# phymhan/pc-gan

Measured on AMD Instinct MI355X. Metric: images/sec (G+D step) 128x128 bs32 per GPU, higher is better.
Workload: dtype f32; 1 GPU; wsgan_emb UTKFace-shaped 128x128 bs32/GPU fp32: 9-block ResnetGenerator + 3-layer PatchGAN + ResNet-18 Elo encoder@224 + AlexNet IP@224, full optimize_parameters(); global_batch=32, parallelism=dp1

## Files before the change

### include/pcgan_hip.h

```cpp
#ifndef PCGAN_HIP_H
#define PCGAN_HIP_H

#include <stddef.h>
#include <stdint.h>

#ifdef __cplusplus
extern "C" {
#endif

typedef void* pcgan_stream_t;

const char* pcgan_last_error(void);
int pcgan_version(void);
int pcgan_device_info(int* cu_count, char* arch, int arch_len);

typedef struct {
    int N, C, H, W;
    int K, R, S;
    int stride, pad, pad_mode;
    int P, Q;
    int dtype;
} pcgan_conv_desc;

enum { PCGAN_ACT_NONE = 0, PCGAN_ACT_RELU = 1, PCGAN_ACT_LRELU = 2, PCGAN_ACT_TANH = 3, PCGAN_ACT_SIGMOID = 4 };
// ... 182 lines not shown
                       const float* const* b1, const void* const* pk2, const float* const* b2, float* const* rm1, float* const* rv1,
                       float* const* rm2, float* const* rv2, void* y1, void* h, void* y2, void* out, float* stats, float* amax,
                       pcgan_stream_t s);
int pcgan_restrunk_bwd(const pcgan_resblock_desc* d, int nblocks, const void* dout, const void* x, const float* x_amax, int n_xamax,
                       const void* y1, const void* h, const void* y2, const void* out, const float* stats, const float* amax,
                       const void* const* pk1b, const void* const* pk2b, float* const* dw1, float* const* db1, float* const* dw2,
                       float* const* db2, void* dy2, void* dh, void* dy1, void* dxs, void* dx, float* scratch, void* wgrad_ws,
                       size_t wgrad_ws_bytes, pcgan_stream_t s, pcgan_stream_t side, pcgan_event_t fork_event);

int pcgan_conv2d_wgrad_direct_supported(const pcgan_conv_desc* d);
int pcgan_conv2d_wgrad_rowring_supported(const pcgan_conv_desc* d);
size_t pcgan_conv2d_wgrad_rowring_workspace_bytes(const pcgan_conv_desc* d);
int pcgan_conv2d_bwd_weight_rowring(const pcgan_conv_desc* d, const void* x, const float* x_amax, int n_xamax, const void* dy, const float* dy_amax,
                                    int n_dyamax, float* dw, int accumulate, void* ws, size_t ws_bytes, pcgan_stream_t s);
size_t pcgan_conv2d_wgrad_direct_workspace_bytes(const pcgan_conv_desc* d);
int pcgan_conv2d_bwd_weight_direct(const pcgan_conv_desc* d, const void* x, const float* x_amax, int n_xamax, const void* dy,
                                   const float* dy_amax, int n_dyamax, float* dw, int accumulate, void* ws, size_t ws_bytes, pcgan_stream_t s);

typedef struct {
    int N, C, H, W;
    int K, R, S;
    int stride, pad_h, pad_w;
    int P, Q;
    int k_off, K_total;
    int dtype;
} pcgan_iconv_desc;
int pcgan_iconv_supported(const pcgan_iconv_desc* d);
size_t pcgan_iconv_packed_bytes(const pcgan_iconv_desc* d);
int pcgan_iconv_pack(const pcgan_iconv_desc* d, int pool_expand, const float* w, const float* gamma, const float* beta, const float* mean,
                     const float* var, float eps, void* packed, pcgan_stream_t s);
int pcgan_iconv_fwd(const pcgan_iconv_desc* d, const void* x, const void* packed, void* y, int relu, pcgan_stream_t s);
int pcgan_maxpool_slice_fwd(const void* x, void* y, int N, int C, int H, int W, int k, int stride, int P, int Q, int k_off, int K_total,
                            int dtype, pcgan_stream_t s);
int pcgan_inception_prep(const void* x, void* y, int N, int C, int H, int W, int OH, int OW, const float* scale, const float* shift,
                         int dtype, pcgan_stream_t s);

int pcgan_linear_softmax_fwd(const void* x, const float* w, const float* b, void* logits, void* probs, int N, int C, int K, int dtype,
                             pcgan_stream_t s);

size_t pcgan_linear_ce_workspace_bytes(int N);
int pcgan_linear_ce_fwd(const void* x, const float* w, const float* b, const int64_t* labels, const float* class_weight, void* logits,
                        void* dlogits, float* loss, int64_t* pred, int32_t* correct, void* workspace, size_t workspace_bytes, int N,
                        int C, int K, int dtype, pcgan_stream_t s);
int pcgan_linear_bwd(const void* dlogits, const void* x, const float* w, void* dx, float* dw, float* db, int N, int C, int K,
                     int accumulate, int dtype, pcgan_stream_t s);

size_t pcgan_pool_mse_workspace_bytes(int NF);
int pcgan_pool_mse_fwd(const void* x, const float* target, float* pred, int32_t* argmax, void* dx, float* loss, int32_t* hits, void* ws,
                       size_t ws_bytes, int N, int F, int HW, int is_max, float delta, float gscale, int dtype, pcgan_stream_t s);

int pcgan_proj_head_fwd(const void* p, const float* y, const float* psi_w, const float* psi_b, const float* ly_w, const float* ly_b,
                        void* out, float* h, int B, int C, int HW, int nz, int By, int sigmoid, int dtype, pcgan_stream_t s);
size_t pcgan_proj_head_bwd_workspace_bytes(int B, int nz);
int pcgan_proj_head_bwd(const void* g, const float* h, const float* y, const float* psi_w, const float* psi_b, const float* ly_w,
                        const float* ly_b, void* dp, float* dpsi_w, float* dpsi_b, float* dly_w, float* dly_b, float* dy, void* workspace,
                        size_t workspace_bytes, int B, int C, int HW, int nz, int By, int sigmoid, int accumulate, int dtype,
                        pcgan_stream_t s);

int pcgan_skip_join_fwd(const void* a, const void* b, void* out, int N, int Ca, int Cb, int HW, int act_a, int act_b, int dtype,
                        pcgan_stream_t s);
int pcgan_skip_join_bwd(const void* dout, const void* a, const void* b, void* da, void* db, int N, int Ca, int Cb, int HW, int act_a,
                        int act_b, int dtype, pcgan_stream_t s);

int pcgan_set_nonfinite_counter(unsigned int* dev_word);
int pcgan_set_option(const char* key, int value);
int pcgan_get_option(const char* key, int* value);
int pcgan_timer_enable(int capacity);
int pcgan_timer_read(int kind, float* ms, int cap);
#define PCGAN_IGEMM_LAUNCH_INFO 7
#define PCGAN_IGEMM_HGEMM_F16X2 1
#define PCGAN_IGEMM_HGEMM_BF16 2
#define PCGAN_IGEMM_IGEMM2_CG16 3
#define PCGAN_IGEMM_IGEMM2_CG4 4
#define PCGAN_IGEMM_GENERIC 5
#define PCGAN_IGEMM_SMALLM 6
int pcgan_igemm_last_launch(int* info, int n);
#define PCGAN_WGRAD_LAUNCH_INFO 9
#define PCGAN_WGRAD_TILE2 1
#define PCGAN_WGRAD_TILE 2
#define PCGAN_WGRAD_SMALLM 3
#define PCGAN_WGRAD_STRIP 4
int pcgan_wgrad_last_launch(int* info, int n);

#ifdef __cplusplus
}
#endif
#endif
```

### pc-gan_amd/csrc/amax.hip

```cpp
#include "common.h"

namespace pcgan {

template <typename TA>
__global__ void __launch_bounds__(256) absmax_kernel(const TA* __restrict__ x, size_t n, float* __restrict__ out) {
    float m = 0.f;
    size_t head = ((16 - (reinterpret_cast<uintptr_t>(x) & 15)) & 15) / sizeof(TA);
    head = head < n ? head : n;
    const TA* xb = x + head;
    const size_t nb = n - head, n4 = nb / 4, stride = (size_t)gridDim.x * blockDim.x;
    size_t i = blockIdx.x * (size_t)blockDim.x + threadIdx.x;
    for (; i + 3 * stride < n4; i += 4 * stride) {
        const float4 a = ld4(xb + 4 * i), b = ld4(xb + 4 * (i + stride)), c = ld4(xb + 4 * (i + 2 * stride)), d = ld4(xb + 4 * (i + 3 * stride));
        m = fmaxf(m, fmaxf(fmaxf(fmaxf(fabsf(a.x), fabsf(a.y)), fmaxf(fabsf(a.z), fabsf(a.w))), fmaxf(fmaxf(fabsf(b.x), fabsf(b.y)), fmaxf(fabsf(b.z), fabsf(b.w)))));
        m = fmaxf(m, fmaxf(fmaxf(fmaxf(fabsf(c.x), fabsf(c.y)), fmaxf(fabsf(c.z), fabsf(c.w))), fmaxf(fmaxf(fabsf(d.x), fabsf(d.y)), fmaxf(fabsf(d.z), fabsf(d.w)))));
    }
    for (; i < n4; i += stride) {
        const float4 v = ld4(xb + 4 * i);
        m = fmaxf(fmaxf(m, fmaxf(fabsf(v.x), fabsf(v.y))), fmaxf(fabsf(v.z), fabsf(v.w)));
    }
    if (blockIdx.x == 0) {
        if (threadIdx.x < head) m = fmaxf(m, fabsf(ld1(x + threadIdx.x)));
        if (threadIdx.x < (nb & 3)) m = fmaxf(m, fabsf(ld1(xb + 4 * n4 + threadIdx.x)));
    }
    __shared__ float red[16];
    m = block_max(m, red);
    if (threadIdx.x == 0) out[blockIdx.x] = m;
}

__global__ void __launch_bounds__(256) amax_audit_kernel(const float* __restrict__ claimed, int nc, const float* __restrict__ fresh, int nf,
                                                         unsigned* __restrict__ counts) {
    __shared__ float red[16];
    float c = 0.f, f = 0.f;
    for (int i = threadIdx.x; i < nc; i += 256) c = fmaxf(c, claimed[i]);
    for (int i = threadIdx.x; i < nf; i += 256) f = fmaxf(f, fresh[i]);
    c = block_max(c, red);
    __syncthreads();
    f = block_max(f, red);
    if (threadIdx.x == 0 && f != c) {
        if (!(f <= c)) atomicAdd(counts + 0, 1u);
        else if (f < c * 0.00390625f) atomicAdd(counts + 1, 1u);
        else atomicAdd(counts + 2, 1u);
    }
}

__global__ void __launch_bounds__(256) weight_row_absmax_kernel(const float* __restrict__ w, int K, int C, int T, int by_c, float* __restrict__ out) {
    const int row = blockIdx.x;
    float m = 0.f;
    if (!by_c) {
        const float* p = w + (size_t)row * C * T;
        for (int i = threadIdx.x; i < C * T; i += 256) m = fmaxf(m, fabsf(p[i]));
    } else {
        for (int i = threadIdx.x; i < K * T; i += 256) {
            const int k = i / T, t = i - k * T;
            m = fmaxf(m, fabsf(w[((size_t)k * C + row) * T + t]));
        }
    }
    __shared__ float red[16];
    m = block_max(m, red);
    if (threadIdx.x == 0) out[row] = m;
}

int launch_weight_row_absmax(const float* w, int K, int C, int T, int by_c, float* out, hipStream_t st) {
    hipLaunchKernelGGL(weight_row_absmax_kernel, dim3((unsigned)(by_c ? C : K)), dim3(256), 0, st, w, K, C, T, by_c, out);
    PCGAN_LAUNCH_CHECK();
    return 0;
}

}

extern "C" int pcgan_absmax_slots(size_t n) {
    const size_t want = (n / 4 + 1023) / 1024;
    return (int)(want < 1 ? 1 : (want > 1024 ? 1024 : want));
}

extern "C" int pcgan_absmax(const void* x, size_t n, int dtype, float* out, int slots, pcgan_stream_t s) {
    PCGAN_CHECK(x && out && n > 0 && slots > 0 && slots <= 1024, "absmax: null pointer, empty tensor or bad slot count");
    PCGAN_CHECK(dtype == PCGAN_F32 || dtype == PCGAN_BF16, "absmax: dtype %d", dtype);
    hipStream_t st = (hipStream_t)s;
    const dim3 grid((unsigned)slots);
    if (dtype == PCGAN_BF16) hipLaunchKernelGGL(pcgan::absmax_kernel<pcgan::bf16>, grid, dim3(256), 0, st, (const pcgan::bf16*)x, n, out);
    else hipLaunchKernelGGL(pcgan::absmax_kernel<float>, grid, dim3(256), 0, st, (const float*)x, n, out);
    PCGAN_LAUNCH_CHECK();
    return 0;
}

extern "C" int pcgan_amax_audit(const float* claimed, int n_claimed, const float* fresh, int n_fresh, unsigned int* counts, pcgan_stream_t s) {
    PCGAN_CHECK(claimed && fresh && counts && n_claimed > 0 && n_fresh > 0, "amax_audit: null pointer or empty maxima");
    hipLaunchKernelGGL(pcgan::amax_audit_kernel, dim3(1), dim3(256), 0, (hipStream_t)s, claimed, n_claimed, fresh, n_fresh, counts);
    PCGAN_LAUNCH_CHECK();
    return 0;
}
```

### pc-gan_amd/csrc/bsplit.h

```cpp
#pragma once
#include "common.h"

namespace pcgan {

typedef float f32x16 __attribute__((ext_vector_type(16)));
typedef __bf16 bf16x8 __attribute__((ext_vector_type(8)));
typedef _Float16 f16x8 __attribute__((ext_vector_type(8)));
typedef unsigned int u32x4 __attribute__((ext_vector_type(4)));
static constexpr unsigned BS_OOB = 0x80000000u;
static constexpr int BS_MAXTAP = 25;

__device__ __forceinline__ void split3(float x, __bf16& h, __bf16& m, __bf16& l) {
    h = (__bf16)x;
    const float r1 = x - (float)h;
    m = (__bf16)r1;
    l = (__bf16)(r1 - (float)m);
}

struct BsplitArgs {
    const void* X;
    const void* A;
    const float* bias;
    void* Y;
    int N, C, H, W, M, R, S, pad, reflect, P, Q;
    int nMt, nst, act;
    float slope;
    unsigned x_bytes, a_bytes;
    int tstart[4];
    unsigned phase_bytes;
    int nst_split;
};

enum { BS_FWD_ZERO = 0, BS_FWD_REFLECT = 1, BS_DGRAD_REFLECT = 2, BS_WGRAD = 3 };

__device__ __forceinline__ void pack_store8(__bf16* __restrict__ A, size_t e, size_t per_piece, int np, float wscale, const float (&v)[8]) {
    if (np == 2) {
        f16x8 h, l;
#pragma unroll
        for (int j = 0; j < 8; ++j) {
            _Float16 x, y;
            split2h(v[j] * wscale, x, y);
            h[j] = x;
            l[j] = y;
        }
        *reinterpret_cast<f16x8*>(reinterpret_cast<_Float16*>(A) + 8 * e) = h;
        *reinterpret_cast<f16x8*>(reinterpret_cast<_Float16*>(A) + per_piece + 8 * e) = l;
        return;
    }
    bf16x8 h, mm, l;
#pragma unroll
    for (int j = 0; j < 8; ++j) {
        __bf16 x, y, z;
        split3(v[j], x, y, z);
        h[j] = x;
        mm[j] = y;
        l[j] = z;
    }
    *reinterpret_cast<bf16x8*>(A + 8 * e) = h;
    if (np == 3) {
        *reinterpret_cast<bf16x8*>(A + per_piece + 8 * e) = mm;
        *reinterpret_cast<bf16x8*>(A + 2 * per_piece + 8 * e) = l;
    }
}

enum { BH_FWD = 0, BH_DGRAD = 1 };

struct HaloArgs {
    const void* X;
    const void* A;
    const float* bias;
    void* Y;
    int N, C, H, M, nMt, nch, act;
    float slope;
    unsigned x_bytes, a_bytes;
    const float* x_amax;
    const float* w_amax;
    int x_namax;
    unsigned* ovf;
    const void* R;
};

enum { PK_BF16X3 = 0,
       PK_BF16 = 1,
       PK_F16X2 = 2 };

struct HWgradArgs {
    const void* XP;
    const void* DY;
    float* part;
    int N, C, K, P, Q, Hp, Wp, R, S, nst, nst_split;
    unsigned xp_bytes, dy_bytes;
    const float* x_amax;
    const float* dy_amax;
    int x_namax, dy_namax;
    int ntile, nwg;
    unsigned* ovf;
    int reflect_inline;
    int splits, nmt;
    int Qs, pad;
};

static inline int np_of(const pcgan_conv_desc* d) { return d->dtype == PCGAN_BF16 ? 1 : 3; }
static inline size_t es_of(const pcgan_conv_desc* d) { return d->dtype == PCGAN_BF16 ? 2 : 4; }

int launch_pad(const void* x, void* xpad, int planes, int H, int W, int pad, int reflect, bool half, hipStream_t st);
int launch_bsplit_pack(const float* w, void* packed, int M, int C, int T, int nMt, int nst, int bm, int np, const float* rowmax, hipStream_t st);
int launch_bsplit_pack_dgrad(const float* w, void* packed, int K, int C, int nMt, int nst, int bm, int np, const float* rowmax, int nphase,
                             hipStream_t st);
int launch_pack_dy(const void* dy, void* packed, int K, int HW, int nst, int bm, int np, bool half, hipStream_t st);
int launch_wgrad_reduce(const float* part, float* dw, int splits, size_t total, int accumulate, hipStream_t st);
int launch_bsplit(int mode, int dtype, int bm, dim3 grid, const BsplitArgs& a, hipStream_t st);
int launch_halo(int mode, int pk, int W, const HaloArgs& a, hipStream_t st);
int launch_hsplit_wgrad(const HWgradArgs& a, int bm, int stride, int cw, bool gen, bool half, dim3 grid, hipStream_t st);

}
```

### pc-gan_amd/csrc/bsplit_pack.hip

```cpp
#include "bsplit.h"

namespace pcgan {

__global__ void bsplit_pack_kernel(const float* __restrict__ w, __bf16* __restrict__ A, int M, int C, int T, int nMt, int nst,
                                   int bm_shift, int np, const float* __restrict__ rowmax = nullptr) {
    const int BM = 128 << bm_shift;
    const size_t per_piece = (size_t)nMt * nst * 16 * BM;
    for (size_t e = blockIdx.x * (size_t)blockDim.x + threadIdx.x; e < per_piece / 8; e += (size_t)gridDim.x * blockDim.x) {
        const int row = (int)(e & (BM - 1)), half = (int)((e >> (7 + bm_shift)) & 1);
        const size_t q = e >> (8 + bm_shift);
        const int st = (int)(q % nst), mt = (int)(q / nst);
        const int m = mt * BM + row, c0 = (st / T) * 16 + half * 8, tap = st % T;
        float v[8];
#pragma unroll
        for (int j = 0; j < 8; ++j) v[j] = m < M ? w[((size_t)m * C + c0 + j) * T + tap] : 0.f;
        const float wscale = (np == 2 && m < M) ? pow2_scale(rowmax[m]) : 1.f;
        pack_store8(A, e, per_piece, np, wscale, v);
    }
}

int launch_bsplit_pack(const float* w, void* packed, int M, int C, int T, int nMt, int nst, int bm, int np, const float* rowmax, hipStream_t st) {
    const size_t per_piece = (size_t)nMt * nst * 16 * bm;
    hipLaunchKernelGGL(bsplit_pack_kernel, dim3(capped_blocks(per_piece / 8, 256, 4096)), dim3(256), 0, st, w, (__bf16*)packed, M, C, T, nMt, nst,
                       bm == 256 ? 1 : 0, np, rowmax);
    PCGAN_LAUNCH_CHECK();
    return 0;
}

__global__ void bsplit_pack_dgrad_kernel(const float* __restrict__ w, __bf16* __restrict__ A, int K, int C, int nMt, int nst, int bm_shift,
                                         int np, const float* __restrict__ rowmax = nullptr, int nphase = 3) {
    const int BM = 128 << bm_shift;
    const size_t per_piece = (size_t)nMt * nst * 16 * BM, per_phase = (size_t)np * per_piece;
    const size_t per_phase8 = per_piece / 8;
    for (size_t i = blockIdx.x * (size_t)blockDim.x + threadIdx.x; i < (size_t)nphase * per_phase8; i += (size_t)gridDim.x * blockDim.x) {
        const int phase = (int)(i / per_phase8);
        const size_t e = i - (size_t)phase * per_phase8;
        const int row = (int)(e & (BM - 1)), half = (int)((e >> (7 + bm_shift)) & 1);
        const size_t q = e >> (8 + bm_shift);
        const int st = (int)(q % nst), mt = (int)(q / nst);
        const int c = mt * BM + row, k0 = (st / 9) * 16 + half * 8, tap = st % 9;
        const int rp = tap / 3, sp = tap - rp * 3;
        const bool fold = (phase == 1 && rp == 0) || (phase == 2 && rp == 2);
        float v[8];
#pragma unroll
        for (int j = 0; j < 8; ++j) {
            v[j] = 0.f;
            if (c < C) {
                const float* wk = w + ((size_t)(k0 + j) * C + c) * 9;
                v[j] = wk[(2 - rp) * 3 + (2 - sp)];
                if (fold) v[j] += wk[rp * 3 + (2 - sp)];
            }
        }
        const float wscale = (np == 2 && c < C) ? pow2_scale(rowmax[c]) : 1.f;
        pack_store8(A + (size_t)phase * per_phase, e, per_piece, np, wscale, v);
    }
}

int launch_bsplit_pack_dgrad(const float* w, void* packed, int K, int C, int nMt, int nst, int bm, int np, const float* rowmax, int nphase,
                             hipStream_t st) {
    const size_t total = (size_t)nphase * nMt * nst * 2 * bm;
    hipLaunchKernelGGL(bsplit_pack_dgrad_kernel, dim3(capped_blocks(total, 256, 4096)), dim3(256), 0, st, w, (__bf16*)packed, K, C, nMt, nst,
                       bm == 256 ? 1 : 0, np, rowmax, nphase);
    PCGAN_LAUNCH_CHECK();
    return 0;
}

template <typename TA>
__global__ void bsplit_pad_reflect_kernel(const TA* __restrict__ x, TA* __restrict__ xp, int H, int W, int pad, int reflect = 1) {
    const int Hp = H + 2 * pad, Wp = W + 2 * pad;
    const TA* src = x + (size_t)blockIdx.y * H * W;
    TA* dst = xp + (size_t)blockIdx.y * Hp * Wp;
    for (int i = blockIdx.x * blockDim.x + threadIdx.x; i < Hp * Wp; i += gridDim.x * blockDim.x) {
        int y = i / Wp - pad, xx = i % Wp - pad;
        if (!reflect) {
            const bool in = (unsigned)y < (unsigned)H && (unsigned)xx < (unsigned)W;
            TA v;
            st1(&v, 0.f);
            dst[i] = in ? src[y * W + xx] : v;
            continue;
        }
        y = y < 0 ? -y : (y >= H ? 2 * (H - 1) - y : y);
        xx = xx < 0 ? -xx : (xx >= W ? 2 * (W - 1) - xx : xx);
        dst[i] = src[y * W + xx];
    }
}

template <typename TA>
__global__ void __launch_bounds__(256) bsplit_pad_wave_kernel(const TA* __restrict__ x, TA* __restrict__ xp, int planes, int H, int W, int pad, int reflect) {
    const int lane = threadIdx.x & 63;
    const int plane = blockIdx.x * 4 + (threadIdx.x >> 6);
    if (plane >= planes) return;
    const int Hp = H + 2 * pad, Wp = W + 2 * pad, half = Wp >> 1;
    const TA* src = x + (size_t)plane * H * W;
    TA* dst = xp + (size_t)plane * Hp * Wp;
    int row = lane / half, cp = lane - row * half;
    const int drow = 64 / half, dcp = 64 - drow * half;
    typedef TA pair_t __attribute__((ext_vector_type(2)));
    while (row < Hp) {
        int y = row - pad, x0 = 2 * cp - pad, x1 = x0 + 1;
        bool in0 = (unsigned)y < (unsigned)H, in1 = in0;
        if (reflect) {
            y = y < 0 ? -y : (y >= H ? 2 * (H - 1) - y : y);
            x0 = x0 < 0 ? -x0 : (x0 >= W ? 2 * (W - 1) - x0 : x0);
            x1 = x1 < 0 ? -x1 : (x1 >= W ? 2 * (W - 1) - x1 : x1);
            in0 = in1 = true;
        } else {
            in0 = in0 && (unsigned)x0 < (unsigned)W;
            in1 = in1 && (unsigned)x1 < (unsigned)W;
        }
        TA zero;
        st1(&zero, 0.f);
        pair_t v;
        v.x = in0 ? src[y * W + x0] : zero;
        v.y = in1 ? src[y * W + x1] : zero;
        *reinterpret_cast<pair_t*>(dst + row * Wp + 2 * cp) = v;
        cp += dcp;
        row += drow;
        if (cp >= half) {
            cp -= half;
            ++row;
        }
    }
}

int launch_pad(const void* x, void* xpad, int planes, int H, int W, int pad, int reflect, bool half, hipStream_t st) {
    const int Hp = H + 2 * pad, Wp = W + 2 * pad;
    if (Wp % 2 == 0 && Wp <= 128 && Hp * Wp <= 8192 && planes >= 1024) {
        const dim3 grid((planes + 3) / 4);
        if (half) hipLaunchKernelGGL(bsplit_pad_wave_kernel<bf16>, grid, dim3(256), 0, st, (const bf16*)x, (bf16*)xpad, planes, H, W, pad, reflect);
        else hipLaunchKernelGGL(bsplit_pad_wave_kernel<float>, grid, dim3(256), 0, st, (const float*)x, (float*)xpad, planes, H, W, pad, reflect);
        PCGAN_LAUNCH_CHECK();
        return 0;
    }
    const dim3 pgrid((Hp * Wp + 255) / 256, planes);
    if (half) hipLaunchKernelGGL(bsplit_pad_reflect_kernel<bf16>, pgrid, dim3(256), 0, st, (const bf16*)x, (bf16*)xpad, H, W, pad, reflect);
    else hipLaunchKernelGGL(bsplit_pad_reflect_kernel<float>, pgrid, dim3(256), 0, st, (const float*)x, (float*)xpad, H, W, pad, reflect);
    PCGAN_LAUNCH_CHECK();
    return 0;
}

template <typename TA>
__global__ void bsplit_pack_dy_kernel(const TA* __restrict__ dy, __bf16* __restrict__ A, int K, int HW, int nst, int bm_shift, int np) {
    const int BM = 128 << bm_shift;
    const size_t per_piece = (size_t)nst * 16 * BM;
    for (size_t i = blockIdx.x * (size_t)blockDim.x + threadIdx.x; i < per_piece; i += (size_t)gridDim.x * blockDim.x) {
// ... 46 lines not shown
```

### pc-gan_amd/csrc/hgemm.hip

```cpp
#include "igemm.h"

namespace pcgan {

typedef _Float16 f16x8 __attribute__((ext_vector_type(8)));
typedef _Float16 f16x4 __attribute__((ext_vector_type(4)));

typedef __bf16 bf16x8v __attribute__((ext_vector_type(8)));
typedef __bf16 bf16x4v __attribute__((ext_vector_type(4)));

template <int MODE, int BM, int BP, typename TA>
__global__ void __launch_bounds__(256) hgemm_kernel(IgemmArgs a) {
    static_assert(MODE == MODE_FWD_ZERO || MODE == MODE_FWD_REFLECT || MODE == MODE_BWD, "forward and plain data gradient");
    constexpr bool HALF = sizeof(TA) == 2;
    constexpr int NP = HALF ? 1 : 2;
    constexpr unsigned ES = sizeof(TA);
    constexpr int WM = (BM == 128 || (BM == 64 && BP == 64)) ? 2 : 1;
    constexpr int WP = 4 / WM;
    constexpr int WMT = BM / WM, WPT = BP / WP;
    constexpr int MI = WMT / 32, PJ = WPT / 32;
    constexpr int KPT = BP / 16;
    constexpr int ACH = BM * 4 / 256;
    constexpr int TROWS = NTAP_FWD + 1;
    constexpr int AH = BM + 8;
    __shared__ __attribute__((aligned(16))) f16x8 As[2][NP][2 * AH];
    __shared__ __attribute__((aligned(16))) f16x8 Bs[2][NP][2 * BP];
    __shared__ unsigned offT[TROWS][BP];
    __shared__ __attribute__((aligned(16))) float biasS[BM];
    __shared__ __attribute__((aligned(16))) float iswS[BM];

    const int nMt = (a.M + BM - 1) / BM;
    const int mt = blockIdx.x % nMt;
    int pt = blockIdx.x / nMt;
    int phase = 0;
    while (phase + 1 < a.nphase && pt >= a.tstart[phase + 1]) ++phase;
    pt -= a.tstart[phase];
    const PhaseArgs& P = a.ph[phase];
    const int tid = threadIdx.x;
    const int lane = tid & 63, lo = lane & 31, hi = lane >> 5;
    const int wave = __builtin_amdgcn_readfirstlane(tid >> 6);
    const int wm = wave / WP, wp = wave % WP;
    const int Ptot = P.Ptot, Kp = P.Kp;
    const int m0 = mt * BM, p0 = pt * BP;
    const int ph_nS = P.nS;
    const int T = P.nR * ph_nS;
    const int HgWg4 = a.Hg * a.Wg * (int)ES;
    const __amdgpu_buffer_rsrc_t rX = make_rsrc(a.X, a.x_bytes);
    const __amdgpu_buffer_rsrc_t rA = make_rsrc(P.A, (unsigned)a.M * (unsigned)Kp * 4u);

    float sx = 1.f;
    const int pl = tid % BP;
    {
        const int pg = p0 + pl;
        const bool pvalid = pg < Ptot;
        int gn = 0, py = 0, px = 0;
        if (pvalid) pix_coord(a, P, pg, gn, py, px);
        const unsigned vbase = (unsigned)gn * (unsigned)a.Cg * (unsigned)(a.Hg * a.Wg);
        for (int t = tid / BP; t <= T; t += 256 / BP) {
            const int ri = t / ph_nS, sj = t - ri * ph_nS;
            const int r = P.r0 + ri * a.tstep, sxx = P.s0 + sj * a.tstep;
            const bool live = pvalid && t < T;
            const unsigned y = axis_entry<MODE>(py, py + a.pad, true, r, a.Hg, a.sl, a.pad);
            const unsigned x = axis_entry<MODE>(px, px + a.pad, true, sxx, a.Wg, a.sl, a.pad);
            offT[t][pl] = (live && y != 0xffffffffu && x != 0xffffffffu) ? (vbase + y * (unsigned)a.Wg + x) * ES : OOB;
        }
    }
    const int ksub = __builtin_amdgcn_readfirstlane(tid / BP);
    __syncthreads();

    const int nst_all = Kp >> 4;
    const int nst_per = a.ksplit > 1 ? (nst_all + a.ksplit - 1) / a.ksplit : nst_all;
    const int st_begin = a.ksplit > 1 ? (int)blockIdx.z * nst_per : 0;
    const int st_end = st_begin + nst_per < nst_all ? st_begin + nst_per : nst_all;
    const int nst_here = st_end > st_begin ? st_end - st_begin : 0;

    int it_tap, it_c, it_k0, it_left = nst_here;
    {
        const int cc0 = st_begin / T;
        it_tap = st_begin - cc0 * T;
        it_c = cc0 * 16;
        it_k0 = st_begin * 16;
    }
    unsigned a_base[ACH];
#pragma unroll
    for (int j = 0; j < ACH; ++j) {
        const int q = tid + 256 * j;
        const int row = q >> 2, kc = (q & 3) * 4;
        a_base[j] = (m0 + row < a.M) ? (unsigned)((m0 + row) * Kp + kc) * 4u : OOB;
    }
// ... 147 lines not shown
        fetch(op[0], 0);
        stash(rg[1], 1);
        __syncthreads();
        load(rg[1]);
        const int nst2 = (nst_here + 1) & ~1;
        for (int s = 0; s < nst2; s += 2) {
#pragma unroll
            for (int t = 0; t < 2; ++t) {
                fetch(op[t ^ 1], t ^ 1);
                mma(op[t]);
                stash(rg[t], t);
                load(rg[t]);
                interleave();
                __builtin_amdgcn_sched_barrier(0);
                __syncthreads();
                __builtin_amdgcn_sched_barrier(0);
            }
        }
    }

    const float isx = 1.f / sx;
    const int YhYw = a.Yh * a.Yw;
    bool bad = false;
    if constexpr (!HALF) {
#pragma unroll
        for (int j = 0; j < PJ; ++j)
#pragma unroll
            for (int i = 0; i < MI; ++i)
#pragma unroll
                for (int r = 0; r < 16; ++r) bad |= is_nonfinite(acc[i][j][r]);
        report_nonfinite(a.ovf, bad);
    }
#pragma unroll
    for (int j = 0; j < PJ; ++j) {
        const int pix = p0 + wp * WPT + j * 32 + lo;
        if (pix >= Ptot) continue;
        int n, oy, ox;
        pix_coord(a, P, pix, n, oy, ox);
        if (a.ksplit > 1) {
            float* Yp = a.Ypart + ((size_t)blockIdx.z * a.N + n) * a.M * YhYw + oy * a.Yw + ox;
#pragma unroll
            for (int i = 0; i < MI; ++i)
#pragma unroll
                for (int r = 0; r < 16; ++r) {
                    const int ml = wm * WMT + i * 32 + (r & 3) + 8 * (r >> 2) + 4 * hi;
                    const int m = m0 + ml;
                    if (m < a.M) Yp[(size_t)m * YhYw] = (acc[i][j][r] * isx) * (HALF ? 1.f : iswS[ml]);
                }
            continue;
        }
        TA* Yp = (TA*)a.Y + (size_t)n * a.M * YhYw + oy * a.Yw + ox;
#pragma unroll
        for (int i = 0; i < MI; ++i)
#pragma unroll
            for (int r = 0; r < 16; ++r) {
                const int ml = wm * WMT + i * 32 + (r & 3) + 8 * (r >> 2) + 4 * hi;
                if (m0 + ml < a.M) st1(Yp + (size_t)(m0 + ml) * YhYw, act_apply((acc[i][j][r] * isx) * (HALF ? 1.f : iswS[ml]) + biasS[ml], a.act, a.slope));
            }
    }
}

template <int MODE>
static void launch_mode(const IgemmArgs& a, int bm, int bp, dim3 grid2, hipStream_t st) {
    if (bm == 128 && bp == 128) LAUNCH_TA(a.dtype, hgemm_kernel, grid2, a, MODE, 128, 128);
    else if (bm == 128) LAUNCH_TA(a.dtype, hgemm_kernel, grid2, a, MODE, 128, 64);
    else if (bp == 128) LAUNCH_TA(a.dtype, hgemm_kernel, grid2, a, MODE, 64, 128);
    else LAUNCH_TA(a.dtype, hgemm_kernel, grid2, a, MODE, 64, 64);
}
int launch_hgemm(int mode, const IgemmArgs& a, int bm, int bp, dim3 grid2, hipStream_t st) {
    switch (mode) {
        case MODE_FWD_ZERO: launch_mode<MODE_FWD_ZERO>(a, bm, bp, grid2, st); break;
        case MODE_FWD_REFLECT: launch_mode<MODE_FWD_REFLECT>(a, bm, bp, grid2, st); break;
        case MODE_BWD: launch_mode<MODE_BWD>(a, bm, bp, grid2, st); break;
        default: PCGAN_CHECK(false, "hgemm: no kernel for mode %d", mode);
    }
    PCGAN_LAUNCH_CHECK();
    return 0;
}

}

using namespace pcgan;

__global__ void __launch_bounds__(256) hgemm_presplit_kernel(float* __restrict__ A, int M, int Kp4, const float* __restrict__ rowmax) {
    const size_t n4 = (size_t)M * Kp4;
    for (size_t i = (size_t)blockIdx.x * 256 + threadIdx.x; i < n4; i += (size_t)gridDim.x * 256) {
        const float s = pow2_scale(rowmax[i / Kp4]);
        const float4 v = reinterpret_cast<const float4*>(A)[i];
        f16x4 h, l;
        _Float16 x, y;
        split2h(v.x * s, x, y); h[0] = x; l[0] = y;
        split2h(v.y * s, x, y); h[1] = x; l[1] = y;
        split2h(v.z * s, x, y); h[2] = x; l[2] = y;
        split2h(v.w * s, x, y); h[3] = x; l[3] = y;
        reinterpret_cast<f16x4*>(A)[2 * i] = h;
        reinterpret_cast<f16x4*>(A)[2 * i + 1] = l;
    }
}

int pcgan::launch_hgemm_presplit(float* A, int M, int Kp4, const float* rowmax, hipStream_t st) {
    hipLaunchKernelGGL(hgemm_presplit_kernel, dim3(capped_blocks((size_t)M * Kp4, 256, 2048)), dim3(256), 0, st, A, M, Kp4, rowmax);
    PCGAN_LAUNCH_CHECK();
    return 0;
}
```

### pc-gan_amd/csrc/igemm_conv.hip

```cpp
#include "igemm.h"
#include <stdlib.h>
#include <mutex>

namespace pcgan {

template <typename TA>
__global__ void splitk_reduce_kernel(const float* __restrict__ part, TA* __restrict__ y, const float* __restrict__ bias,
                                     int ks, size_t n, int M, int HW, int act, float slope) {
    const size_t n4 = (n & 3) ? 0 : (n >> 2);
    const size_t stride = (size_t)gridDim.x * blockDim.x;
    for (size_t i = blockIdx.x * (size_t)blockDim.x + threadIdx.x; i < n4; i += stride) {
        float4 acc = reinterpret_cast<const float4*>(part)[i];
        for (int s = 1; s < ks; ++s) {
            const float4 v = reinterpret_cast<const float4*>(part + (size_t)s * n)[i];
            acc.x += v.x; acc.y += v.y; acc.z += v.z; acc.w += v.w;
        }
        float o[4] = {acc.x, acc.y, acc.z, acc.w};
#pragma unroll
        for (int u = 0; u < 4; ++u) {
            const size_t e = i * 4 + u;
            if (bias) o[u] += bias[(e / HW) % M];
            o[u] = act_apply(o[u], act, slope);
        }
        st4(y + 4 * i, make_float4(o[0], o[1], o[2], o[3]));
    }
    for (size_t e = (n4 << 2) + blockIdx.x * (size_t)blockDim.x + threadIdx.x; e < n; e += stride) {
        float acc = 0.f;
        for (int s = 0; s < ks; ++s) acc += part[(size_t)s * n + e];
        if (bias) acc += bias[(e / HW) % M];
        st1(y + e, act_apply(acc, act, slope));
    }
}

__global__ void repack_fwd_kernel(const float* __restrict__ w, float* __restrict__ A, int K, int C, int Cgp,
                                  int RS, int chunked) {
    const int Kp = RS * Cgp;
    const size_t total = (size_t)K * Kp;
    for (size_t i = blockIdx.x * (size_t)blockDim.x + threadIdx.x; i < total; i += (size_t)gridDim.x * blockDim.x) {
        const int k = (int)(i / Kp);
        const int j = (int)(i - (size_t)k * Kp);
        int tap, c;
        if (chunked) {
            const int t2 = j >> 4;
            const int cc = t2 / RS;
            tap = t2 - cc * RS;
            c = cc * 16 + (j & 15);
        } else {
            tap = j / Cgp;
            c = j - tap * Cgp;
        }
        A[i] = (c < C) ? w[((size_t)k * C + c) * RS + tap] : 0.f;
    }
}
__global__ void repack_bwd_kernel(const float* __restrict__ w, float* __restrict__ A, int K, int C, int Kgp,
                                  int R, int S, int r0, int s0, int tstep, int nR, int nS, int chunked, int fold) {
    const int Kp = nR * nS * Kgp;
    const size_t total = (size_t)C * Kp;
    for (size_t i = blockIdx.x * (size_t)blockDim.x + threadIdx.x; i < total; i += (size_t)gridDim.x * blockDim.x) {
        const int c = (int)(i / Kp);
        const int j = (int)(i - (size_t)c * Kp);
        int t, k;
        if (chunked) {
            const int t2 = j >> 4;
            const int kc = t2 / (nR * nS);
            t = t2 - kc * (nR * nS);
            k = kc * 16 + (j & 15);
        } else {
            t = j / Kgp;
            k = j - t * Kgp;
        }
        const int ri = t / nS, sj = t - ri * nS;
        const int r = r0 + ri * tstep, s = s0 + sj * tstep;
        float v = (k < K) ? w[(((size_t)k * C + c) * R + r) * S + s] : 0.f;
        if (k < K && fold == 1 && r == R - 1) v += w[(((size_t)k * C + c) * R + 0) * S + s];
        if (k < K && fold == 2 && r == 0) v += w[(((size_t)k * C + c) * R + (R - 1)) * S + s];
        A[i] = v;
    }
}

struct PackBwdArgs {
    const float* w;
    int K, C, Kgp, R, S, tstep, chunked, n;
    struct Entry {
        float* A;
        int r0, s0, nR, nS, fold;
    } e[16];
};
__global__ void repack_bwd_multi_kernel(PackBwdArgs a) {
    const PackBwdArgs::Entry& E = a.e[blockIdx.y];
    const int RS = E.nR * E.nS;
    const int Kp = RS * a.Kgp;
    const size_t total = (size_t)a.C * Kp;
    for (size_t i = blockIdx.x * (size_t)blockDim.x + threadIdx.x; i < total; i += (size_t)gridDim.x * blockDim.x) {
        const int c = (int)(i / Kp);
        const int j = (int)(i - (size_t)c * Kp);
        int t, k;
        if (a.chunked) {
            const int t2 = j >> 4;
            const int kc = t2 / RS;
            t = t2 - kc * RS;
            k = kc * 16 + (j & 15);
        } else {
            t = j / a.Kgp;
            k = j - t * a.Kgp;
        }
        const int ri = t / E.nS, sj = t - ri * E.nS;
        const int r = E.r0 + ri * a.tstep, sx = E.s0 + sj * a.tstep;
        float v = 0.f;
        if (k < a.K) {
            const float* wk = a.w + ((size_t)k * a.C + c) * a.R * a.S;
            v = wk[r * a.S + sx];
            if (E.fold == 1 && r == a.R - 1) v += wk[sx];
            if (E.fold == 2 && r == 0) v += wk[(a.R - 1) * a.S + sx];
        }
        E.A[i] = v;
    }
}

template <typename TA>
__global__ void reflect_fold_kernel(const TA* __restrict__ t, TA* __restrict__ dx, int NC, int H, int W,
                                    int pad) {
    const int Hp = H + 2 * pad, Wp = W + 2 * pad;
    const int W4 = (W + 3) >> 2;
    const TA* tp = t + (size_t)blockIdx.y * Hp * Wp;
    TA* dp = dx + (size_t)blockIdx.y * H * W;
    for (int i = blockIdx.x * blockDim.x + threadIdx.x; i < H * W4; i += gridDim.x * blockDim.x) {
        const int y = i / W4, x0 = (i - y * W4) * 4;
        int ys[3], ny = 0;
        ys[ny++] = y + pad;
        if (y >= 1 && y <= pad) ys[ny++] = pad - y;
        if (y >= H - 1 - pad && y <= H - 2) ys[ny++] = pad + 2 * (H - 1) - y;
        float acc[4] = {0.f, 0.f, 0.f, 0.f};
        for (int a = 0; a < ny; ++a) {
            const TA* row = tp + ys[a] * Wp;
#pragma unroll
            for (int j = 0; j < 4; ++j) {
                const int x = x0 + j;
                if (x >= W) continue;
                float v = ld1(row + x + pad);
                if (x >= 1 && x <= pad) v += ld1(row + pad - x);
                if (x >= W - 1 - pad && x <= W - 2) v += ld1(row + pad + 2 * (W - 1) - x);
                acc[j] += v;
            }
        }
        if ((W & 3) == 0) {
            st4(dp + y * W + x0, make_float4(acc[0], acc[1], acc[2], acc[3]));
        } else {
            for (int j = 0; j < 4 && x0 + j < W; ++j) st1(dp + y * W + x0 + j, acc[j]);
        }
    }
}

int launch_splitk_reduce(int dtype, hipStream_t st, const float* part, void* y, const float* bias, int ks, size_t out_elems, int M,
                         int HW, int act, float slope) {
    const dim3 b(capped_blocks(out_elems / 4, 256, 4096));
    if (dtype == PCGAN_BF16)
        hipLaunchKernelGGL(splitk_reduce_kernel<bf16>, b, dim3(256), 0, st, part, (bf16*)y, bias, ks, out_elems, M, HW, act, slope);
    else
        hipLaunchKernelGGL(splitk_reduce_kernel<float>, b, dim3(256), 0, st, part, (float*)y, bias, ks, out_elems, M, HW, act, slope);
    PCGAN_LAUNCH_CHECK();
    return 0;
}

static int check_desc(const pcgan_conv_desc* d) {
    PCGAN_CHECK(d != nullptr, "conv: null descriptor");
    PCGAN_CHECK(d->N > 0 && d->C > 0 && d->H > 0 && d->W > 0 && d->K > 0 && d->R > 0 && d->S > 0,
                "conv: non-positive dimension");
    PCGAN_CHECK(ilog2_exact(d->stride) >= 0 && d->stride <= 4, "conv: stride %d unsupported (1,2,4)", d->stride);
    PCGAN_CHECK(d->pad_mode == 0 || d->pad_mode == 1, "conv: pad_mode %d", d->pad_mode);
    PCGAN_CHECK(d->dtype == PCGAN_F32 || d->dtype == PCGAN_BF16, "conv: dtype %d (PCGAN_F32 / PCGAN_BF16)", d->dtype);
    const int P = (d->H + 2 * d->pad - d->R) / d->stride + 1, Q = (d->W + 2 * d->pad - d->S) / d->stride + 1;
    PCGAN_CHECK(P == d->P && Q == d->Q, "conv: output dims %dx%d do not match geometry %dx%d", d->P, d->Q, P, Q);
    if (d->pad_mode == 1)
        PCGAN_CHECK(d->pad < d->H && d->pad < d->W, "conv: reflection pad %d >= input size", d->pad);
    const size_t xin = (size_t)d->N * d->C * (d->H + 2 * d->pad) * (d->W + 2 * d->pad) * 4;
    const size_t yout = (size_t)d->N * d->K * d->P * d->Q * 4;
    PCGAN_CHECK(xin < (1ull << 31) && yout < (1ull << 31),
                "conv: tensor of %zu bytes exceeds the 2 GiB addressing limit of one launch (split the batch)",
                xin > yout ? xin : yout);
    PCGAN_CHECK((size_t)d->K * round4(d->C) * d->R * d->S * 4 < (1ull << 31) &&
                    (size_t)d->C * round4(d->K) * d->R * d->S * 4 < (1ull << 31), "conv: weight tensor too large");
    PCGAN_CHECK(d->R * d->S <= 512, "conv: filter too large");
    return 0;
}

static inline bool chunked_k(int Cg, int M, int R, int S) { return (Cg % 16) == 0 && M > 4 && R * S <= NTAP_FWD; }
static inline bool cg4_k(int Cg, int M, int R, int S) { return round4(Cg) == 4 && M > 4 && R * S <= NTAP_CG4; }
static inline long tile_blocks(int M, int ptot_max, int nphase, int mm, int pp) {
    return (long)((M + mm - 1) / mm) * ((ptot_max + pp - 1) / pp) * nphase;
}
static inline long split_below() { return 192; }
static inline bool may_split(int M, int ptot_max, int nphase) {
    if (option(OPT_HGEMM_KS) > 1) return M > 4;
    const int m = M > 64 ? 128 : (M > 32 ? 64 : 32);
    return M > 4 && tile_blocks(M, ptot_max, nphase, m, 128) < split_below();
}
static void choose_tile(int M, int ptot_max, int nphase, int nst, bool allow_split, int* bm, int* bp, int* ks) {
    int m = M > 64 ? 128 : (M > 32 ? 64 : 32);
    int p = 128;
// ... 52 lines not shown
    int nst_min = 1 << 30;
    for (int i = 0; i < a.nphase; ++i) nst_min = (a.ph[i].Kp + 15) / 16 < nst_min ? (a.ph[i].Kp + 15) / 16 : nst_min;
    const size_t out_elems = (size_t)a.N * a.M * a.Yh * a.Yw;
    choose_tile(a.M, pmax, a.nphase, nst_min, part_ws != nullptr, &bm, &bp, &ks);
    if (ks > 1 && (size_t)ks * out_elems * 4 > part_bytes) ks = 1;
    a.ksplit = ks;
    a.Ypart = part_ws;
    const dim3 grid((unsigned)(((a.M + bm - 1) / bm) * ((pmax + bp - 1) / bp)), (unsigned)a.nphase, (unsigned)ks);
    a.tstart[0] = 0;
    for (int i = 0; i < a.nphase; ++i) a.tstart[i + 1] = a.tstart[i] + (a.ph[i].Ptot + bp - 1) / bp;
    const dim3 grid2((unsigned)(((a.M + bm - 1) / bm) * a.tstart[a.nphase]), 1u, (unsigned)ks);
    const bool cg16 = a.chunked == 1, cg4 = a.chunked == 2;
    PCGAN_CHECK(cg16 || mode != MODE_BWD_REFLECT, "igemm: fused reflect data-gradient needs K %% 16 == 0");
    if (cg4) {
        PCGAN_CHECK(a.Cgp == 4, "igemm: 4-channel stages need a 3-/4-channel tensor");
        for (int i = 0; i < a.nphase; ++i)
            PCGAN_CHECK(a.ph[i].nR * a.ph[i].nS <= NTAP_CG4, "igemm: 4-channel stages: more than %d taps", NTAP_CG4);
    }
    if (cg16) {
        PCGAN_CHECK((a.Cg % 16) == 0, "igemm: chunked K order needs a multiple of 16 channels");
        for (int i = 0; i < a.nphase; ++i)
            PCGAN_CHECK(a.ph[i].nR * a.ph[i].nS <= (mode == MODE_BWD_REFLECT ? NTAP_MIR : NTAP_FWD) && (a.ph[i].Kp % 16) == 0,
                        "igemm: chunked K order: bad phase");
    }
    const bool half = a.dtype == PCGAN_BF16 && option(OPT_HGEMM_BF16) != 0;
    if ((half || (a.hsplit && a.dtype == PCGAN_F32)) && cg16 && mode != MODE_BWD_REFLECT && bm >= 64) {
        record_launch(half ? PCGAN_IGEMM_HGEMM_BF16 : PCGAN_IGEMM_HGEMM_F16X2, mode, bm, bp, ks, a.nphase);
        if (int e = launch_hgemm(mode, a, bm, bp, grid2, st)) return e;
    } else {
        record_launch(cg16 ? PCGAN_IGEMM_IGEMM2_CG16 : (cg4 ? PCGAN_IGEMM_IGEMM2_CG4 : PCGAN_IGEMM_GENERIC), mode, bm, bp, ks, a.nphase);
        if (int e = launch_igemm_f32(mode, a, bm, bp, grid, grid2, st)) return e;
    }
    if (ks > 1 && launch_splitk_reduce(a.dtype, st, part_ws, a.Y, a.bias, ks, out_elems, a.M, a.Yh * a.Yw, a.act, a.slope)) return 2;
    return 0;
}

}

using namespace pcgan;

static size_t fwd_part_bytes(const pcgan_conv_desc* d) {
    const int ptot = d->N * d->P * d->Q;
    if (d->K <= 4) return (ptot <= 65536 && d->C >= 64) ? align_up((size_t)8 * d->K * ptot * 4, 256) : 0;
    return may_split(d->K, ptot, 1) ? align_up((size_t)8 * d->N * d->K * d->P * d->Q * 4, 256) : 0;
}
static size_t bwd_part_bytes(const pcgan_conv_desc* d) {
    const int s = d->stride;
    const int pmax = d->N * ((d->H + s - 1) / s) * ((d->W + s - 1) / s);
    return may_split(d->C, pmax, s * s) ? align_up((size_t)8 * d->N * d->C * d->H * d->W * 4, 256) : 0;
}
static size_t fwd_base_bytes(const pcgan_conv_desc* d) {
    return align_up((size_t)d->K * d->R * d->S * round4(d->C) * 4 + (size_t)d->R * d->S * round4(d->C) * 16 +
                    (d->K <= 4 ? (size_t)d->S * d->C * 128 : 0), 256);
}
static bool bwd_fused_reflect(const pcgan_conv_desc* d) {
    return d->pad_mode == 1 && chunked_k(d->K, d->C, d->R, d->S) && d->R * d->S <= NTAP_MIR && d->H >= 2 * d->pad + 2 &&
           d->W >= 2 * d->pad + 2;
}
static bool bwd_rowfold(const pcgan_conv_desc* d) { return bwd_fused_reflect(d) && d->pad == 1 && d->R == 3 && d->stride == 1; }
static size_t bwd_base_bytes(const pcgan_conv_desc* d) {
    const size_t a = (size_t)d->C * d->R * d->S * round4(d->K) * 4;
    return align_up((bwd_rowfold(d) ? 3 * a : a) + (size_t)d->R * d->S * round4(d->K) * 16 +
                    (d->C <= 4 ? (size_t)d->stride * d->S * d->K * 128 : 0), 256);
}

extern "C" size_t pcgan_conv2d_workspace_bytes(const pcgan_conv_desc* d, int pass) {
    if (!d) return 0;
    const size_t RS = (size_t)d->R * d->S;
    if (pass == PCGAN_PASS_FWD) return fwd_base_bytes(d) + fwd_part_bytes(d);
    if (pass == PCGAN_PASS_BWD_DATA) {
        size_t b = bwd_base_bytes(d) + bwd_part_bytes(d);
        if (d->pad_mode == 1)
            b += align_up((size_t)d->N * d->C * (d->H + 2 * d->pad) * (d->W + 2 * d->pad) * 4, 256);
        return b;
    }
    int cps;
    const int splits = wgrad_splits(d, &cps);
    return align_up((size_t)splits * d->K * RS * round4(d->C) * 4, 256);
}

static int pack_fwd(const pcgan_conv_desc* d, const float* w, float* A, hipStream_t st) {
    const int Cgp = round4(d->C), RS = d->R * d->S;
    const size_t total = (size_t)d->K * RS * Cgp;
    hipLaunchKernelGGL(repack_fwd_kernel, dim3(capped_blocks(total, 256, 4096)), dim3(256), 0, st, w, A, d->K, d->C, Cgp, RS,
                       (int)chunked_k(d->C, d->K, d->R, d->S));
    PCGAN_LAUNCH_CHECK();
    if (d->K <= 4) {
        if (int e = launch_transpose4(A, A + total, d->K, RS * Cgp, st)) return e;
        if (int e = launch_pack_strip(A, A + total + (size_t)RS * Cgp * 4, d->K, d->C, Cgp, d->R, d->S, st)) return e;
    }
    return 0;
}

struct HsplitOpt {
    const float* x_amax;
    int n_amax;
    const float* w_amax;
};
static void apply_hsplit(IgemmArgs& a, const HsplitOpt* hs) {
    if (!hs) return;
    a.hsplit = 1; a.x_amax = hs->x_amax; a.x_namax = hs->n_amax; a.w_amax = hs->w_amax;
    a.ovf = pcgan::nonfinite_counter();
}

static int conv2d_fwd_impl(const pcgan_conv_desc* d, const void* x, const float* w, const float* packed,
                           const float* bias, void* y, int act, float slope, void* ws, size_t ws_bytes,
                           pcgan_stream_t s, const HsplitOpt* hs = nullptr) {
    if (check_desc(d)) return 1;
    PCGAN_CHECK(x && (w || packed) && y, "conv2d_fwd: null pointer");
    PCGAN_CHECK(ws && ws_bytes >= pcgan_conv2d_workspace_bytes(d, PCGAN_PASS_FWD),
                "conv2d_fwd: workspace too small (%zu)", ws_bytes);
    hipStream_t st = (hipStream_t)s;
    const int Cgp = round4(d->C), RS = d->R * d->S;
    float* A = packed ? const_cast<float*>(packed) : (float*)ws;
    if (!packed && pack_fwd(d, w, A, st)) return 2;
    IgemmArgs a;
    memset(&a, 0, sizeof(a));
    a.X = x; a.Y = y; a.bias = bias; a.dtype = d->dtype;
    a.M = d->K; a.N = d->N; a.Cg = d->C; a.Cgp = Cgp; a.Hg = d->H; a.Wg = d->W;
    a.Yh = d->P; a.Yw = d->Q;
    a.ostep = 1; a.sl = ilog2_exact(d->stride); a.pad = d->pad; a.tstep = 1;
    a.act = act; a.slope = slope;
    a.x_bytes = (unsigned)((size_t)d->N * d->C * d->H * d->W * esz(d));
    a.nphase = 1;
    a.chunked = chunked_k(d->C, d->K, d->R, d->S) ? 1 : (cg4_k(d->C, d->K, d->R, d->S) ? 2 : 0);
    apply_hsplit(a, hs);
    PhaseArgs& p = a.ph[0];
    p.A = A; p.Kp = RS * Cgp; p.Hs = d->P; p.Ws = d->Q; p.fy = 0; p.fx = 0;
    if (d->K <= 4) {
        p.A = A + (size_t)d->K * RS * Cgp;
        p.As = p.A + (size_t)RS * Cgp * 4;
    }
    p.r0 = 0; p.s0 = 0; p.nR = d->R; p.nS = d->S; p.Ptot = d->N * d->P * d->Q;
    float* part = fwd_part_bytes(d) ? (float*)((char*)ws + fwd_base_bytes(d)) : nullptr;
    return launch_igemm(d->pad_mode == 1 ? MODE_FWD_REFLECT : MODE_FWD_ZERO, a, st, part, fwd_part_bytes(d));
}

extern "C" int pcgan_conv2d_fwd(const pcgan_conv_desc* d, const void* x, const float* w, const float* bias,
                                void* y, int act, float slope, void* ws, size_t ws_bytes, pcgan_stream_t s) {
    if (check_desc(d)) return 1;
    PCGAN_CHECK(w, "conv2d_fwd: null weight pointer");
    return conv2d_fwd_impl(d, x, w, nullptr, bias, y, act, slope, ws, ws_bytes, s);
}
extern "C" int pcgan_conv2d_fwd_packed(const pcgan_conv_desc* d, const void* x, const float* packed,
                                       const float* bias, void* y, int act, float slope, void* ws, size_t ws_bytes,
                                       pcgan_stream_t s) {
    if (check_desc(d)) return 1;
    PCGAN_CHECK(packed, "conv2d_fwd_packed: null packed-weight pointer");
    pcgan::TimerScope timer(pcgan::timer_kind_res(d, pcgan::TIMER_RES_FWD), (hipStream_t)s);
    return conv2d_fwd_impl(d, x, nullptr, packed, bias, y, act, slope, ws, ws_bytes, s);
}

namespace pcgan {
int launch_reflect_fold(const void* padded, void* dx, int NC, int H, int W, int pad, int dtype, hipStream_t st) {
    PCGAN_CHECK(NC <= 65535, "conv2d_bwd_data: more than 65535 planes in the reflect fold");
    const dim3 grid((H * ((W + 3) / 4) + 255) / 256, NC);
    if (dtype == PCGAN_BF16)
        hipLaunchKernelGGL(reflect_fold_kernel<bf16>, grid, dim3(256), 0, st, (const bf16*)padded, (bf16*)dx, NC, H, W, pad);
    else
        hipLaunchKernelGGL(reflect_fold_kernel<float>, grid, dim3(256), 0, st, (const float*)padded, (float*)dx, NC, H, W, pad);
    PCGAN_LAUNCH_CHECK();
    return 0;
}
}

struct BwdPhase {
    int fy, fx, r0, s0, nR, nS, Hs, Ws;
    int fold;
    size_t a_off, at_off, as_off;
};
struct BwdPlan {
    bool fused, rowfold, padded;
    int H, W, pad;
    bool need_zero;
    int n;
    BwdPhase ph[16];
};
static void bwd_plan(const pcgan_conv_desc* d, BwdPlan& pl) {
    memset(&pl, 0, sizeof(pl));
    pl.fused = bwd_fused_reflect(d);
    pl.rowfold = bwd_rowfold(d);
    pl.padded = d->pad_mode == 1 && !pl.fused;
    const int H = pl.H = pl.padded ? d->H + 2 * d->pad : d->H;
    const int W = pl.W = pl.padded ? d->W + 2 * d->pad : d->W;
    const int pad = pl.pad = pl.padded ? 0 : d->pad;
    const int stv = d->stride, Kgp = round4(d->K), RS = d->R * d->S;
    if (pl.rowfold) {
        for (int f = 0; f < 3; ++f) {
            BwdPhase& p = pl.ph[pl.n++];
            p.nR = d->R; p.nS = d->S; p.Ws = W; p.fold = f;
            p.Hs = f == 0 ? H - 2 : 1;
            p.fy = f == 0 ? 0 : (f == 1 ? 1 : H - 2);
            p.a_off = (size_t)f * d->C * RS * Kgp;
        }
        return;
    }
    size_t a_off = 0;
    size_t at_off = (size_t)d->C * RS * Kgp;
    size_t as_off = at_off + (size_t)RS * Kgp * 4;
    for (int fy = 0; fy < stv; ++fy) {
        for (int fx = 0; fx < stv; ++fx) {
            const int r0 = (fy + pad) % stv, s0 = (fx + pad) % stv;
            const int nR = r0 < d->R ? (d->R - r0 + stv - 1) / stv : 0;
            const int nS = s0 < d->S ? (d->S - s0 + stv - 1) / stv : 0;
            const int Hs = fy < H ? (H - fy + stv - 1) / stv : 0;
            const int Ws = fx < W ? (W - fx + stv - 1) / stv : 0;
            if (Hs * Ws == 0) continue;
            if (nR * nS == 0) {
                pl.need_zero = true;
                continue;
            }
            const BwdPhase p = {fy, fx, r0, s0, nR, nS, Hs, Ws, 0, a_off, at_off, as_off};
            pl.ph[pl.n++] = p;
            a_off += (size_t)d->C * nR * nS * Kgp;
            at_off += (size_t)nR * nS * Kgp * 4;
            as_off += (size_t)d->K * nS * 32;
        }
    }
}

static int pack_bwd(const pcgan_conv_desc* d, const BwdPlan& pl, const float* w, float* packed, hipStream_t st) {
    const int Kgp = round4(d->K);
    const int chunked = (int)chunked_k(d->K, d->C, d->R, d->S);
    if (d->C <= 4) {
        for (int i = 0; i < pl.n; ++i) {
            const BwdPhase& p = pl.ph[i];
            float* A = packed + p.a_off;
            const size_t total = (size_t)d->C * p.nR * p.nS * Kgp;
            hipLaunchKernelGGL(repack_bwd_kernel, dim3(capped_blocks(total, 256, 4096)), dim3(256), 0, st, w, A, d->K, d->C, Kgp, d->R,
                               d->S, p.r0, p.s0, d->stride, p.nR, p.nS, chunked, 0);
            PCGAN_LAUNCH_CHECK();
            if (int e = launch_transpose4(A, packed + p.at_off, d->C, p.nR * p.nS * Kgp, st)) return e;
            if (int e = launch_pack_strip(A, packed + p.as_off, d->C, d->K, Kgp, p.nR, p.nS, st)) return e;
        }
        return 0;
    }
    if (pl.n == 0) return 0;
    size_t max_total = 0;
    PackBwdArgs pk;
    memset(&pk, 0, sizeof(pk));
    pk.w = w; pk.K = d->K; pk.C = d->C; pk.Kgp = Kgp; pk.R = d->R; pk.S = d->S; pk.tstep = d->stride; pk.chunked = chunked; pk.n = pl.n;
    for (int i = 0; i < pl.n; ++i) {
        const BwdPhase& p = pl.ph[i];
        const size_t total = (size_t)d->C * p.nR * p.nS * Kgp;
        max_total = total > max_total ? total : max_total;
        PackBwdArgs::Entry& pe = pk.e[i];
        pe.A = packed + p.a_off; pe.r0 = p.r0; pe.s0 = p.s0; pe.nR = p.nR; pe.nS = p.nS; pe.fold = p.fold;
    }
    hipLaunchKernelGGL(repack_bwd_multi_kernel, dim3(capped_blocks(max_total, 256, 2048), pk.n), dim3(256), 0, st, pk);
    PCGAN_LAUNCH_CHECK();
    return 0;
}

static int conv2d_bwd_data_impl(const pcgan_conv_desc* d, const void* dy, const float* w, const float* packed,
                                const float* bias, void* dx, void* ws, size_t ws_bytes, pcgan_stream_t s, const HsplitOpt* hs = nullptr) {
    if (check_desc(d)) return 1;
    PCGAN_CHECK(dy && (w || packed), "conv2d_bwd_data: null pointer");
    PCGAN_CHECK(ws && ws_bytes >= pcgan_conv2d_workspace_bytes(d, PCGAN_PASS_BWD_DATA),
                "conv2d_bwd_data: workspace too small (%zu)", ws_bytes);
    PCGAN_CHECK(d->pad_mode == 0 || d->stride == 1, "conv2d_bwd_data: reflection padding needs stride 1");
    hipStream_t st = (hipStream_t)s;
    const int Kgp = round4(d->K), stv = d->stride;
    BwdPlan pl;
    bwd_plan(d, pl);
    float* Abase = packed ? const_cast<float*>(packed) : (float*)ws;
    if (!packed && pack_bwd(d, pl, w, Abase, st)) return 2;
    const size_t a_bytes = bwd_base_bytes(d);
    const int H = pl.H, W = pl.W;
    void* out = pl.padded ? (void*)((char*)ws + a_bytes) : dx;

    IgemmArgs a;
    memset(&a, 0, sizeof(a));
    a.X = dy; a.Y = out; a.bias = bias; a.dtype = d->dtype;
    a.M = d->C; a.N = d->N; a.Cg = d->K; a.Cgp = Kgp; a.Hg = d->P; a.Wg = d->Q;
    a.Yh = H; a.Yw = W;
    a.ostep = stv; a.sl = ilog2_exact(stv); a.pad = pl.pad; a.tstep = stv;
    a.act = PCGAN_ACT_NONE; a.slope = 0.f;
    a.chunked = chunked_k(d->K, d->C, d->R, d->S) ? 1 : (cg4_k(d->K, d->C, d->R, d->S) ? 2 : 0);
    a.rowfold = pl.rowfold;
    apply_hsplit(a, hs);
    a.x_bytes = (unsigned)((size_t)d->N * d->K * d->P * d->Q * esz(d));
    a.nphase = pl.n;
    for (int i = 0; i < pl.n; ++i) {
        const BwdPhase& q = pl.ph[i];
        PhaseArgs& p = a.ph[i];
        p.A = Abase + q.a_off; p.Kp = q.nR * q.nS * Kgp; p.Hs = q.Hs; p.Ws = q.Ws; p.fy = q.fy; p.fx = q.fx;
        if (d->C <= 4) {
            p.A = Abase + q.at_off;
            p.As = Abase + q.as_off;
        }
        p.r0 = q.r0; p.s0 = q.s0; p.nR = q.nR; p.nS = q.nS; p.Ptot = d->N * q.Hs * q.Ws;
        p.ymap = pl.rowfold && q.fold == 0;
    }
    if (pl.rowfold) return launch_igemm(MODE_BWD_REFLECT, a, st, nullptr, 0);
    if (pl.need_zero) {
        PCGAN_CHECK(!bias, "conv2d_bwd_data: bias with uncovered phases is unsupported");
        hipError_t e = hipMemsetAsync(out, 0, (size_t)d->N * d->C * H * W * esz(d), st);
        PCGAN_CHECK(e == hipSuccess, "memset failed: %s", hipGetErrorString(e));
    }
    float* part = (bwd_part_bytes(d) && !pl.padded && !pl.need_zero) ? (float*)((char*)ws + a_bytes) : nullptr;
    if (launch_igemm(pl.fused ? MODE_BWD_REFLECT : MODE_BWD, a, st, part, bwd_part_bytes(d))) return 2;
    if (pl.padded) return pcgan::launch_reflect_fold(out, dx, d->N * d->C, d->H, d->W, d->pad, d->dtype, st);
    return 0;
}

extern "C" int pcgan_conv2d_bwd_data(const pcgan_conv_desc* d, const void* dy, const float* w,
                                     const float* bias, void* dx, void* ws, size_t ws_bytes,
                                     pcgan_stream_t s) {
    if (check_desc(d)) return 1;
    PCGAN_CHECK(w && dx, "conv2d_bwd_data: null pointer");
    return conv2d_bwd_data_impl(d, dy, w, nullptr, bias, dx, ws, ws_bytes, s);
}
extern "C" int pcgan_conv2d_bwd_data_packed(const pcgan_conv_desc* d, const void* dy, const float* packed,
                                            const float* bias, void* dx, void* ws, size_t ws_bytes,
                                            pcgan_stream_t s) {
    if (check_desc(d)) return 1;
    PCGAN_CHECK(packed && dx, "conv2d_bwd_data_packed: null pointer");
    pcgan::TimerScope timer(pcgan::timer_kind_res(d, pcgan::TIMER_RES_DGRAD), (hipStream_t)s);
    return conv2d_bwd_data_impl(d, dy, nullptr, packed, bias, dx, ws, ws_bytes, s);
}

extern "C" int pcgan_conv2d_hgemm_supported(const pcgan_conv_desc* d, int pass) {
    if (!d || d->dtype != PCGAN_F32) return 0;
    if (pass == PCGAN_PASS_FWD) return chunked_k(d->C, d->K, d->R, d->S) && d->K > 32;
    if (pass == PCGAN_PASS_BWD_DATA) return d->pad_mode == 0 && chunked_k(d->K, d->C, d->R, d->S) && d->C > 32;
    return 0;
}
extern "C" int pcgan_conv2d_fwd_packed_hsplit(const pcgan_conv_desc* d, const void* x, const float* x_amax, int n_amax, const float* packed,
                                              const float* w_amax, const float* bias, void* y, int act, float slope, void* ws,
                                              size_t ws_bytes, pcgan_stream_t s) {
    if (check_desc(d)) return 1;
    PCGAN_CHECK(pcgan_conv2d_hgemm_supported(d, PCGAN_PASS_FWD), "conv2d_fwd_packed_hsplit: unsupported shape");
    PCGAN_CHECK(packed && x_amax && n_amax > 0 && w_amax, "conv2d_fwd_packed_hsplit: null pointer");
    const HsplitOpt hs = {x_amax, n_amax, w_amax};
// ... 78 lines not shown
```

### pc-gan_amd/csrc/smallm_conv.hip

```cpp
#include "igemm.h"

namespace pcgan {

__global__ void transpose4_kernel(const float* __restrict__ A, float* __restrict__ At, int M, int Kp) {
    const int total = Kp * 4;
    for (int i = blockIdx.x * blockDim.x + threadIdx.x; i < total; i += gridDim.x * blockDim.x) {
        const int k = i >> 2, m = i & 3;
        At[i] = m < M ? A[(size_t)m * Kp + k] : 0.f;
    }
}

__global__ void pack_strip_kernel(const float* __restrict__ A, float* __restrict__ Ws, int M, int Cg, int Cgp, int nR, int nS) {
    const int total = Cg * nS * 32;
    const int Kp = nR * nS * Cgp;
    for (int i = blockIdx.x * blockDim.x + threadIdx.x; i < total; i += gridDim.x * blockDim.x) {
        const int m = i & 3, ri = (i >> 2) & 7, cs = i >> 5;
        const int c = cs / nS, sj = cs - c * nS;
        Ws[i] = (m < M && ri < nR) ? A[(size_t)m * Kp + (ri * nS + sj) * Cgp + c] : 0.f;
    }
}

template <int MODE, typename TA>
__global__ void __launch_bounds__(256) smallm_conv_kernel(IgemmArgs a) {
    constexpr unsigned ES = sizeof(TA);
    __shared__ unsigned rowoff[12][64], coloff[12][64];
    __shared__ float red[3][4][64];
    const PhaseArgs& P = a.ph[blockIdx.y];
    const int Ptot = P.Ptot;
    const int p0 = blockIdx.x * 64;
    if (p0 >= Ptot) return;
    const int tid = threadIdx.x;
    const int pl = tid & 63;
    const int wave = __builtin_amdgcn_readfirstlane(tid >> 6);
    const int pg = p0 + pl;
    const bool pvalid = pg < Ptot;
    const int HsWs = P.Hs * P.Ws, HgWg = a.Hg * a.Wg;
    int n = 0, py = 0, px = 0;
    if (pvalid) {
        n = pg / HsWs;
        const int rem = pg - n * HsWs;
        const int sy = rem / P.Ws;
        py = sy * a.ostep + P.fy;
        px = (rem - sy * P.Ws) * a.ostep + P.fx;
    }
    for (int i = wave; i < P.nR; i += 4) {
        const int r = P.r0 + i * a.tstep;
        int iy;
        bool ok = true;
        if (MODE == MODE_BWD) {
            const int ty = py + a.pad - r;
            iy = ty >> a.sl;
            ok = ty >= 0 && iy < a.Hg;
        } else {
            iy = (py << a.sl) - a.pad + r;
            if (MODE == MODE_FWD_REFLECT) {
                iy = iy < 0 ? -iy : iy;
                iy = iy >= a.Hg ? 2 * (a.Hg - 1) - iy : iy;
            } else {
                ok = (unsigned)iy < (unsigned)a.Hg;
            }
        }
        rowoff[i][pl] = ok ? (unsigned)(iy * a.Wg) * ES : SM_INV;
    }
    for (int j = wave; j < P.nS; j += 4) {
        const int s = P.s0 + j * a.tstep;
        int ix;
        bool ok = true;
        if (MODE == MODE_BWD) {
            const int tx = px + a.pad - s;
            ix = tx >> a.sl;
            ok = tx >= 0 && ix < a.Wg;
        } else {
            ix = (px << a.sl) - a.pad + s;
            if (MODE == MODE_FWD_REFLECT) {
                ix = ix < 0 ? -ix : ix;
                ix = ix >= a.Wg ? 2 * (a.Wg - 1) - ix : ix;
            } else {
                ok = (unsigned)ix < (unsigned)a.Wg;
            }
        }
        coloff[j][pl] = ok ? (unsigned)ix * ES : SM_INV;
    }
    __syncthreads();
    const unsigned vbase = pvalid ? (unsigned)(n * a.Cg * HgWg) * ES : SM_INV;
    const __amdgpu_buffer_rsrc_t rX = make_rsrc(a.X, a.x_bytes);
    const float4* __restrict__ At = reinterpret_cast<const float4*>(P.A);
    const int cpw = (a.Cg + 3) >> 2;
    const int c_lo = wave * cpw;
    const int c_hi = (c_lo + cpw < a.Cg) ? c_lo + cpw : a.Cg;
    float acc0 = 0.f, acc1 = 0.f, acc2 = 0.f, acc3 = 0.f;
    for (int c = c_lo; c < c_hi; ++c) {
        const unsigned soff = (unsigned)(c * HgWg) * ES;
        for (int ri = 0; ri < P.nR; ++ri) {
            const unsigned ro = vbase + rowoff[ri][pl];
            const float4* __restrict__ wrow = At + (ri * P.nS) * a.Cgp + c;
#pragma unroll 4
            for (int sj = 0; sj < P.nS; ++sj) {
                const float x = ldx<TA>(rX, ro + coloff[sj][pl], soff);
                const float4 w = wrow[sj * a.Cgp];
                acc0 += x * w.x; acc1 += x * w.y; acc2 += x * w.z; acc3 += x * w.w;
            }
        }
    }
// ... 150 lines not shown
    if (wave > 0 || !svalid) return;
    const int YhYw = a.Yh * a.Yw;
#pragma unroll
    for (int j = 0; j < PX; ++j) {
        if (sy0 + j >= P.Hs) break;
        const int py = (sy0 + j) * a.ostep + P.fy;
        const size_t yo = (size_t)n * a.M * YhYw + py * a.Yw + px;
#pragma unroll
        for (int m = 0; m < MO; ++m) {
            if (m < a.M) {
                float v = acc[m][j] + (red[0][m * PX + j][pl] + red[1][m * PX + j][pl]) + red[2][m * PX + j][pl];
                if (a.ksplit > 1) {
                    a.Ypart[(size_t)blockIdx.z * a.N * a.M * YhYw + yo + (size_t)m * YhYw] = v;
                    continue;
                }
                if (a.bias) v += a.bias[m];
                st1((TA*)a.Y + yo + (size_t)m * YhYw, act_apply(v, a.act, a.slope));
            }
        }
    }
}

template <int MODE, typename TA>
__global__ void __launch_bounds__(256) smallm_conv_fewtaps_kernel(IgemmArgs a) {
    constexpr unsigned ES = sizeof(TA);
    const PhaseArgs& P = a.ph[blockIdx.y];
    const int Ptot = P.Ptot;
    if ((int)(blockIdx.x * 256) >= Ptot) return;
    const int pg = blockIdx.x * 256 + threadIdx.x;
    const bool pvalid = pg < Ptot;
    const Geom g{a.Hg, a.Wg, a.sl, a.pad};
    const int HsWs = P.Hs * P.Ws, HgWg = a.Hg * a.Wg;
    int n = 0, py = 0, px = 0;
    if (pvalid) {
        n = pg / HsWs;
        const int rem = pg - n * HsWs;
        const int sy = rem / P.Ws;
        py = sy * a.ostep + P.fy;
        px = (rem - sy * P.Ws) * a.ostep + P.fx;
    }
    const int vbase = n * a.Cg * HgWg;
    const __amdgpu_buffer_rsrc_t rX = make_rsrc(a.X, a.x_bytes);
    const float4* __restrict__ At = reinterpret_cast<const float4*>(P.A);
    float acc0 = 0.f, acc1 = 0.f, acc2 = 0.f, acc3 = 0.f;
    for (int ri = 0; ri < P.nR; ++ri) {
        for (int sj = 0; sj < P.nS; ++sj) {
            int off;
            const bool ok = tap_offset<MODE>(g, py, px, P.r0 + ri * a.tstep, P.s0 + sj * a.tstep, off) && pvalid;
            const unsigned voff = ok ? (unsigned)(vbase + off) * ES : OOB;
            const int kbase = (ri * P.nS + sj) * a.Cgp;
            int c = 0;
            for (; c + 8 <= a.Cg; c += 8) {
                float x[8];
#pragma unroll
                for (int u = 0; u < 8; ++u) x[u] = ldx<TA>(rX, voff, (unsigned)((c + u) * HgWg) * ES);
#pragma unroll
                for (int u = 0; u < 8; ++u) {
                    const float4 w = At[kbase + c + u];
                    acc0 += x[u] * w.x; acc1 += x[u] * w.y; acc2 += x[u] * w.z; acc3 += x[u] * w.w;
                }
            }
            for (; c < a.Cg; ++c) {
                const float x = ldx<TA>(rX, voff, (unsigned)(c * HgWg) * ES);
                const float4 w = At[kbase + c];
                acc0 += x * w.x; acc1 += x * w.y; acc2 += x * w.z; acc3 += x * w.w;
            }
        }
    }
    if (!pvalid) return;
    const int YhYw = a.Yh * a.Yw;
    TA* Yp = (TA*)a.Y + (size_t)n * a.M * YhYw + py * a.Yw + px;
    const float out[4] = {acc0, acc1, acc2, acc3};
#pragma unroll
    for (int m = 0; m < 4; ++m) {
        if (m < a.M) {
            float v = out[m];
            if (a.bias) v += a.bias[m];
            st1(Yp + (size_t)m * YhYw, act_apply(v, a.act, a.slope));
        }
    }
}

int launch_transpose4(const float* A, float* At, int M, int Kp, hipStream_t st) {
    hipLaunchKernelGGL(transpose4_kernel, dim3((Kp * 4 + 255) / 256), dim3(256), 0, st, A, At, M, Kp);
    PCGAN_LAUNCH_CHECK();
    return 0;
}
int launch_pack_strip(const float* A, float* Ws, int M, int Cg, int Cgp, int nR, int nS, hipStream_t st) {
    hipLaunchKernelGGL(pack_strip_kernel, dim3((Cg * nS * 32 + 255) / 256), dim3(256), 0, st, A, Ws, M, Cg, Cgp, nR, nS);
    PCGAN_LAUNCH_CHECK();
    return 0;
}

enum { SM_STRIP, SM_FEWTAPS, SM_GENERIC };
template <int MODE>
static void launch_mode(int kernel, const IgemmArgs& a, dim3 grid, int maxR, hipStream_t st) {
    if (kernel == SM_FEWTAPS) LAUNCH_TA(a.dtype, smallm_conv_fewtaps_kernel, grid, a, MODE);
    else if (kernel == SM_GENERIC) LAUNCH_TA(a.dtype, smallm_conv_kernel, grid, a, MODE);
    else if (maxR <= 4 && a.M <= 3) LAUNCH_TA(a.dtype, smallm_strip_kernel, grid, a, MODE, 4, 3);
    else if (maxR <= 4) LAUNCH_TA(a.dtype, smallm_strip_kernel, grid, a, MODE, 4, 4);
    else if (a.M <= 3) LAUNCH_TA(a.dtype, smallm_strip_kernel, grid, a, MODE, 7, 3);
    else LAUNCH_TA(a.dtype, smallm_strip_kernel, grid, a, MODE, 7, 4);
}
static int launch_kernel(int mode, int kernel, const IgemmArgs& a, dim3 grid, int maxR, hipStream_t st) {
    switch (mode == MODE_BWD_REFLECT ? MODE_BWD : mode) {
        case MODE_FWD_ZERO: launch_mode<MODE_FWD_ZERO>(kernel, a, grid, maxR, st); break;
        case MODE_FWD_REFLECT: launch_mode<MODE_FWD_REFLECT>(kernel, a, grid, maxR, st); break;
        default: launch_mode<MODE_BWD>(kernel, a, grid, maxR, st); break;
    }
    PCGAN_LAUNCH_CHECK();
    return 0;
}

int launch_smallm(int mode, IgemmArgs& a, int pmax, hipStream_t st, float* part_ws, size_t part_bytes) {
    PCGAN_CHECK(a.x_bytes < SM_INV, "small-M conv: gathered tensor must be < 1 GiB");
    for (int i = 0; i < a.nphase; ++i)
        PCGAN_CHECK(a.ph[i].nR <= 12 && a.ph[i].nS <= 12, "small-M conv: more than 12 taps per axis");
    int maxR = 0, minH = 1 << 30, maxstrips = 0, maxtaps = 0;
    for (int i = 0; i < a.nphase; ++i) {
        maxR = a.ph[i].nR > maxR ? a.ph[i].nR : maxR;
        minH = a.ph[i].Hs < minH ? a.ph[i].Hs : minH;
        const int ns = a.N * ((a.ph[i].Hs + 7) / 8) * a.ph[i].Ws;
        maxstrips = ns > maxstrips ? ns : maxstrips;
        maxtaps = a.ph[i].nR * a.ph[i].nS > maxtaps ? a.ph[i].nR * a.ph[i].nS : maxtaps;
    }
    const bool unit = mode == MODE_BWD || mode == MODE_BWD_REFLECT || (a.sl == 0 && a.ostep == 1);
    if (unit && maxR >= 3 && maxR <= 7 && minH >= 8) {
        const int wgs = ((maxstrips + 63) / 64) * a.nphase;
        int ks = 1;
        const size_t out_elems = (size_t)a.N * a.M * a.Yh * a.Yw;
        if (part_ws != nullptr && a.nphase == 1 && wgs < 128 && a.Cg >= 64) {
            ks = 256 / wgs;
            if (ks > 8) ks = 8;
            if (ks > a.Cg / 16) ks = a.Cg / 16;
            if ((size_t)ks * out_elems * 4 > part_bytes) ks = 1;
        }
        a.ksplit = ks;
        a.Ypart = part_ws;
        record_launch(PCGAN_IGEMM_SMALLM, mode, 0, 0, ks, a.nphase);
        const dim3 gs((unsigned)((maxstrips + 63) / 64), (unsigned)a.nphase, (unsigned)ks);
        if (int e = launch_kernel(mode, SM_STRIP, a, gs, maxR, st)) return e;
        if (ks > 1 && launch_splitk_reduce(a.dtype, st, part_ws, a.Y, a.bias, ks, out_elems, a.M, a.Yh * a.Yw, a.act, a.slope)) return 2;
        return 0;
    }
    record_launch(PCGAN_IGEMM_SMALLM, mode, 0, 0, 1, a.nphase);
    if (maxtaps <= 9) return launch_kernel(mode, SM_FEWTAPS, a, dim3((unsigned)((pmax + 255) / 256), (unsigned)a.nphase), maxR, st);
    return launch_kernel(mode, SM_GENERIC, a, dim3((unsigned)((pmax + 63) / 64), (unsigned)a.nphase), maxR, st);
}

}
```

### pc-gan_amd/csrc/thin_conv.hip

```cpp
#include "common.h"

namespace pcgan {
namespace {

typedef _Float16 f16x8 __attribute__((ext_vector_type(8)));
typedef _Float16 f16x4 __attribute__((ext_vector_type(4)));
typedef float f32x16 __attribute__((ext_vector_type(16)));
typedef unsigned u32x4 __attribute__((ext_vector_type(4)));
typedef unsigned u32x2 __attribute__((ext_vector_type(2)));

constexpr unsigned THIN_OOB = 0x80000000u;

struct ThinArgs {
    const float* X;
    float* Y;
    const u32x4* A;
    const float* rowmax;
    const float* bias;
    const float* x_amax;
    int x_namax;
    int N, Cin, H, W, M, P, Q, pad, reflect, tilesX, tilesY, act;
    float slope;
    unsigned x_bytes;
    unsigned* ovf;
};

__device__ __forceinline__ constexpr int tap_off(int t, int T, int S, int WC) { return t < T ? (t / S) * WC + (t % S) : 0; }

template <int R, int S, int ST>
__global__ void __launch_bounds__(256) thin_conv_kernel(ThinArgs a) {
    constexpr int TH = 8, TW = 32, T = R * S;
    constexpr int WR = (TH - 1) * ST + R, WC = (TW - 1) * ST + S, NPOS = WR * WC;
    constexpr int NST = (T * 4 + 15) / 16;
    constexpr int PER = (NPOS + 255) / 256;
    __shared__ __attribute__((aligned(16))) u32x2 Wh[NPOS], Wl[NPOS];
    __shared__ float isw[64];
    __shared__ float red[8];
    const int tid = threadIdx.x, lane = tid & 63, lo = lane & 31, hi = lane >> 5;
    const int wave = __builtin_amdgcn_readfirstlane(tid >> 6);
    const int wm = wave & 1, ph = wave >> 1;
    const int bid = blockIdx.x, mt = blockIdx.y;
    const int tx = bid % a.tilesX, ty = (bid / a.tilesX) % a.tilesY, n = bid / (a.tilesX * a.tilesY);
    const int oy0 = ty * TH, ox0 = tx * TW;

#ifndef THIN_AHEAD
#define THIN_AHEAD 2
#endif
    constexpr int AHEAD = THIN_AHEAD < NST ? THIN_AHEAD : NST, NH = AHEAD;
    f16x8 Ah[NST], Al[NST];
    const u32x4* Ap = a.A + ((size_t)(mt * 2 + wm) * NST * 2) * 64 + lane;
#pragma unroll
    for (int st = 0; st < NH; ++st) {
        Ah[st] = __builtin_bit_cast(f16x8, Ap[(st * 2 + 0) * 64]);
        Al[st] = __builtin_bit_cast(f16x8, Ap[(st * 2 + 1) * 64]);
    }

    const __amdgpu_buffer_rsrc_t rX = __builtin_amdgcn_make_buffer_rsrc(const_cast<float*>(a.X), 0, (int)a.x_bytes, 0x00020000);
    const int HW = a.H * a.W;
    float xv[PER][4];
#pragma unroll
    for (int i = 0; i < PER; ++i) {
        const int p = tid + i * 256;
        const int wy = p / WC, wx = p - wy * WC;
        int iy = oy0 * ST - a.pad + wy, ix = ox0 * ST - a.pad + wx;
        bool ok = p < NPOS;
        if (a.reflect) {
            iy = iy < 0 ? -iy : (iy >= a.H ? 2 * a.H - 2 - iy : iy);
            ix = ix < 0 ? -ix : (ix >= a.W ? 2 * a.W - 2 - ix : ix);
            iy = min(max(iy, 0), a.H - 1);
            ix = min(max(ix, 0), a.W - 1);
        } else {
            ok = ok && iy >= 0 && iy < a.H && ix >= 0 && ix < a.W;
        }
        const unsigned vo = ok ? (unsigned)(iy * a.W + ix) * 4u : THIN_OOB;
#pragma unroll
        for (int c = 0; c < 4; ++c)
            xv[i][c] = c < a.Cin ? __uint_as_float(__builtin_amdgcn_raw_buffer_load_b32(rX, vo, (unsigned)((n * a.Cin + c) * HW) * 4u, 0)) : 0.f;
    }

    const float sx = pow2_scale(block_max(thread_max_of_partials(a.x_amax, a.x_namax, tid, 256), red));
    if (tid < 64) isw[tid] = 1.f / (pow2_scale(a.rowmax[mt * 64 + tid]) * sx);

#pragma unroll
    for (int i = 0; i < PER; ++i) {
        const int p = tid + i * 256;
        f16x4 h, l;
#pragma unroll
        for (int c = 0; c < 4; ++c) {
            _Float16 x, y;
            split2h(xv[i][c] * sx, x, y);
            h[c] = x;
            l[c] = y;
        }
        if (p < NPOS) {
            Wh[p] = __builtin_bit_cast(u32x2, h);
            Wl[p] = __builtin_bit_cast(u32x2, l);
        }
    }
    __syncthreads();

    f32x16 acc[4];
#pragma unroll
    for (int j = 0; j < 4; ++j)
#pragma unroll
        for (int r = 0; r < 16; ++r) acc[j][r] = 0.f;
    const int base = (ph * 4 * ST) * WC + lo * ST;
#pragma unroll
    for (int st = 0; st < NST; ++st) {
        if (st + AHEAD < NST) {
            Ah[st + AHEAD] = __builtin_bit_cast(f16x8, Ap[((st + AHEAD) * 2 + 0) * 64]);
            Al[st + AHEAD] = __builtin_bit_cast(f16x8, Ap[((st + AHEAD) * 2 + 1) * 64]);
            __builtin_amdgcn_sched_barrier(0);
        }
        const int o0 = hi ? tap_off(st * 4 + 2, T, S, WC) : tap_off(st * 4 + 0, T, S, WC);
        const int o1 = hi ? tap_off(st * 4 + 3, T, S, WC) : tap_off(st * 4 + 1, T, S, WC);
#pragma unroll
        for (int j = 0; j < 4; ++j) {
            const int q = base + j * ST * WC;
            u32x4 bh, bl;
            const u32x2 h0 = Wh[q + o0], h1 = Wh[q + o1], l0 = Wl[q + o0], l1 = Wl[q + o1];
            bh.x = h0.x; bh.y = h0.y; bh.z = h1.x; bh.w = h1.y;
            bl.x = l0.x; bl.y = l0.y; bl.z = l1.x; bl.w = l1.y;
            const f16x8 Bh = __builtin_bit_cast(f16x8, bh), Bl = __builtin_bit_cast(f16x8, bl);
            acc[j] = __builtin_amdgcn_mfma_f32_32x32x16_f16(Al[st], Bh, acc[j], 0, 0, 0);
            acc[j] = __builtin_amdgcn_mfma_f32_32x32x16_f16(Ah[st], Bl, acc[j], 0, 0, 0);
            acc[j] = __builtin_amdgcn_mfma_f32_32x32x16_f16(Ah[st], Bh, acc[j], 0, 0, 0);
        }
    }

    bool bad = false;
    const int ox = ox0 + lo;
    const size_t PQ = (size_t)a.P * a.Q;
#pragma unroll
    for (int j = 0; j < 4; ++j) {
        const int oy = oy0 + ph * 4 + j;
        if (oy >= a.P || ox >= a.Q) continue;
#pragma unroll
        for (int r = 0; r < 16; ++r) {
            const int ml = wm * 32 + (r >> 2) * 8 + hi * 4 + (r & 3), m = mt * 64 + ml;
            const float av = acc[j][r] * isw[ml];
            bad |= is_nonfinite(av);
            a.Y[((size_t)n * a.M + m) * PQ + (size_t)oy * a.Q + ox] = act_apply(av + (a.bias ? a.bias[m] : 0.f), a.act, a.slope);
        }
    }
    report_nonfinite(a.ovf, bad);
}

__global__ void thin_pack_kernel(const float* __restrict__ w, const float* __restrict__ rowmax, u32x4* __restrict__ out, int M, int G, int T,
                                 int nst, int transposed, int Kout, int Cin, int total) {
    const int e = blockIdx.x * blockDim.x + threadIdx.x;
    if (e >= total) return;
    const int ln = e & 63, piece = (e >> 6) & 1, st = (e >> 7) % nst, mb = (e >> 7) / nst;
    const int lo = ln & 31, hi = ln >> 5, m = mb * 32 + lo;
    const float s = m < M ? pow2_scale(rowmax[m]) : 1.f;
    f16x8 v;
#pragma unroll
    for (int i = 0; i < 8; ++i) {
        const int k = st * 16 + hi * 8 + i, tap = k >> 2, g = k & 3;
        float x = 0.f;
        if (m < M && tap < T && g < G) x = transposed ? w[((size_t)g * Cin + m) * T + (T - 1 - tap)] : w[((size_t)m * Cin + g) * T + tap];
        _Float16 h, l;
        split2h(x * s, h, l);
        v[i] = piece ? l : h;
    }
    (void)Kout;
    out[e] = __builtin_bit_cast(u32x4, v);
}

struct Geo {
    int G, M, Hin, Win, Hout, Wout, pad, reflect, R, S, ST, nst, transposed;
    bool fold;
};

bool thin_geometry(const pcgan_conv_desc* d, int pass, Geo* g) {
    if (!d || d->dtype != PCGAN_F32) return false;
    const bool k77 = d->R == 7 && d->S == 7, k44 = d->R == 4 && d->S == 4;
    if (pass == PCGAN_PASS_FWD) {
        if (d->C > 4 || d->K % 64 != 0 || d->K > 256) return false;
        if (!((k77 && (d->stride == 1 || d->stride == 2)) || (k44 && d->stride == 2))) return false;
        if (d->pad_mode == 1 && (d->stride != 1 || d->pad >= d->H || d->pad >= d->W)) return false;
        *g = Geo{d->C, d->K, d->H, d->W, d->P, d->Q, d->pad, d->pad_mode == 1, d->R, d->S, d->stride, (d->R * d->S * 4 + 15) / 16, 0, false};
        return true;
    }
    if (pass == PCGAN_PASS_BWD_DATA) {
        if (d->K > 4 || d->C % 64 != 0 || d->C > 256 || !k77 || d->stride != 1) return false;
        const bool refl = d->pad_mode == 1;
        const int pad = refl ? d->R - 1 : d->R - 1 - d->pad;
        if (pad < 0) return false;
        *g = Geo{d->K, d->C, d->P, d->Q, refl ? d->H + 2 * d->pad : d->H, refl ? d->W + 2 * d->pad : d->W, pad, false, d->R, d->S, 1,
                 (d->R * d->S * 4 + 15) / 16, 1, refl};
        return true;
    }
    return false;
}

size_t thin_body_bytes(const Geo& g) { return (size_t)(g.M / 32) * g.nst * 2 * 64 * 16; }

template <int R, int S, int ST>
int launch_thin(const ThinArgs& a, int mtiles, hipStream_t st) {
    hipLaunchKernelGGL((thin_conv_kernel<R, S, ST>), dim3((unsigned)(a.N * a.tilesX * a.tilesY), (unsigned)mtiles), dim3(256), 0, st, a);
    PCGAN_LAUNCH_CHECK();
    return 0;
}

int run_thin(const Geo& g, int N, const void* x, const float* x_amax, int n_amax, const void* packed, const float* bias, void* y, int act,
             float slope, hipStream_t st) {
    ThinArgs a;
    memset(&a, 0, sizeof(a));
    a.X = (const float*)x; a.Y = (float*)y; a.A = (const u32x4*)packed;
    a.rowmax = (const float*)((const char*)packed + thin_body_bytes(g));
    a.bias = bias; a.x_amax = x_amax; a.x_namax = n_amax;
    a.N = N; a.Cin = g.G; a.H = g.Hin; a.W = g.Win; a.M = g.M; a.P = g.Hout; a.Q = g.Wout; a.pad = g.pad; a.reflect = g.reflect;
    a.tilesX = (g.Wout + 31) / 32; a.tilesY = (g.Hout + 7) / 8; a.act = act; a.slope = slope;
    const size_t xb = (size_t)N * g.G * g.Hin * g.Win * 4;
    PCGAN_CHECK(xb < 0x7fffffffull, "conv2d thin: input of %zu bytes exceeds the 31-bit buffer range", xb);
    PCGAN_CHECK((size_t)N * a.tilesX * a.tilesY < 0x7fffffffull, "conv2d thin: too many tiles");
    a.x_bytes = (unsigned)xb;
    a.ovf = nonfinite_counter();
    const int mt = g.M / 64;
    if (g.R == 7 && g.ST == 1) return launch_thin<7, 7, 1>(a, mt, st);
    if (g.R == 7 && g.ST == 2) return launch_thin<7, 7, 2>(a, mt, st);
    if (g.R == 4 && g.ST == 2) return launch_thin<4, 4, 2>(a, mt, st);
    set_error("conv2d thin: no kernel for %dx%d stride %d", g.R, g.S, g.ST);
    return 1;
}

}
}

using namespace pcgan;

extern "C" int pcgan_conv2d_thin_supported(const pcgan_conv_desc* d, int pass) {
    Geo g;
    return thin_geometry(d, pass, &g) ? 1 : 0;
}

extern "C" size_t pcgan_conv2d_thin_packed_bytes(const pcgan_conv_desc* d, int pass) {
    Geo g;
    if (!thin_geometry(d, pass, &g)) return 0;
    return thin_body_bytes(g) + (size_t)g.M * sizeof(float);
}

extern "C" size_t pcgan_conv2d_thin_workspace_bytes(const pcgan_conv_desc* d, int pass) {
    Geo g;
    if (!thin_geometry(d, pass, &g) || !g.fold) return 0;
    return (size_t)d->N * g.M * g.Hout * g.Wout * sizeof(float);
}

extern "C" int pcgan_conv2d_thin_pack(const pcgan_conv_desc* d, int pass, const float* w, void* packed, pcgan_stream_t s) {
    Geo g;
    PCGAN_CHECK(thin_geometry(d, pass, &g), "conv2d_thin_pack: unsupported shape (pcgan_conv2d_thin_supported)");
    PCGAN_CHECK(w && packed, "conv2d_thin_pack: null pointer");
    hipStream_t st = (hipStream_t)s;
    float* rowmax = (float*)((char*)packed + thin_body_bytes(g));
    if (launch_weight_row_absmax(w, d->K, d->C, d->R * d->S, g.transposed, rowmax, st)) return 2;
    const int total = (g.M / 32) * g.nst * 2 * 64;
    hipLaunchKernelGGL(thin_pack_kernel, dim3((unsigned)((total + 255) / 256)), dim3(256), 0, st, w, (const float*)rowmax, (u32x4*)packed, g.M,
                       g.G, g.R * g.S, g.nst, g.transposed, d->K, d->C, total);
    PCGAN_LAUNCH_CHECK();
    return 0;
}

extern "C" int pcgan_conv2d_fwd_thin(const pcgan_conv_desc* d, const void* x, const float* x_amax, int n_amax, const void* packed,
                                     const float* bias, void* y, int act, float slope, pcgan_stream_t s) {
    Geo g;
    PCGAN_CHECK(thin_geometry(d, PCGAN_PASS_FWD, &g), "conv2d_fwd_thin: unsupported shape (pcgan_conv2d_thin_supported)");
    PCGAN_CHECK(x && x_amax && n_amax > 0 && packed && y, "conv2d_fwd_thin: null pointer");
    return run_thin(g, d->N, x, x_amax, n_amax, packed, bias, y, act, slope, (hipStream_t)s);
}

extern "C" int pcgan_conv2d_bwd_data_thin(const pcgan_conv_desc* d, const void* dy, const float* dy_amax, int n_amax, const void* packed,
                                          void* dx, void* ws, size_t ws_bytes, pcgan_stream_t s) {
    Geo g;
    PCGAN_CHECK(thin_geometry(d, PCGAN_PASS_BWD_DATA, &g), "conv2d_bwd_data_thin: unsupported shape (pcgan_conv2d_thin_supported)");
    PCGAN_CHECK(dy && dy_amax && n_amax > 0 && packed && dx, "conv2d_bwd_data_thin: null pointer");
    if (!g.fold) return run_thin(g, d->N, dy, dy_amax, n_amax, packed, nullptr, dx, PCGAN_ACT_NONE, 0.f, (hipStream_t)s);
    PCGAN_CHECK(ws && ws_bytes >= pcgan_conv2d_thin_workspace_bytes(d, PCGAN_PASS_BWD_DATA), "conv2d_bwd_data_thin: workspace too small (%zu)",
                ws_bytes);
    if (int e = run_thin(g, d->N, dy, dy_amax, n_amax, packed, nullptr, ws, PCGAN_ACT_NONE, 0.f, (hipStream_t)s)) return e;
    return launch_reflect_fold(ws, dx, d->N * d->C, d->H, d->W, d->pad, PCGAN_F32, (hipStream_t)s);
}
```

### pc-gan_amd/hip/lib.py

```python
import ctypes
import os

_HERE = os.path.dirname(os.path.abspath(__file__))
LIB_PATH = os.environ.get('PCGAN_LIB') or os.path.join(os.path.dirname(_HERE), 'lib', 'libpcgan_hip.so')

ACT_NONE, ACT_RELU, ACT_LRELU, ACT_TANH, ACT_SIGMOID = 0, 1, 2, 3, 4
PASS_FWD, PASS_BWD_DATA, PASS_BWD_WEIGHT = 0, 1, 2
F32, BF16 = 0, 1


class ImageDesc(ctypes.Structure):
    _fields_ = [(n, ctypes.c_int) for n in ('H', 'W', 'RH', 'RW', 'FH', 'FW', 'ksize_h', 'ksize_v', 'out_channels')]


class ResBlockDesc(ctypes.Structure):
    _fields_ = [('N', ctypes.c_int), ('C', ctypes.c_int), ('H', ctypes.c_int), ('W', ctypes.c_int), ('eps', ctypes.c_float),
                ('momentum', ctypes.c_float), ('dtype', ctypes.c_int)]


class ConvDesc(ctypes.Structure):
    _fields_ = [(n, ctypes.c_int) for n in
                ('N', 'C', 'H', 'W', 'K', 'R', 'S', 'stride', 'pad', 'pad_mode', 'P', 'Q', 'dtype')]


class IconvDesc(ctypes.Structure):
    _fields_ = [(n, ctypes.c_int) for n in
                ('N', 'C', 'H', 'W', 'K', 'R', 'S', 'stride', 'pad_h', 'pad_w', 'P', 'Q', 'k_off', 'K_total', 'dtype')]


_vp, _i, _f, _sz = ctypes.c_void_p, ctypes.c_int, ctypes.c_float, ctypes.c_size_t
_dp = ctypes.POINTER(ConvDesc)
_icp = ctypes.POINTER(IconvDesc)
_ip = ctypes.POINTER(ImageDesc)
_rp = ctypes.POINTER(ResBlockDesc)

SIGNATURES = {
    'pcgan_last_error': (ctypes.c_char_p, []),
    'pcgan_version': (_i, []),
    'pcgan_device_info': (_i, [ctypes.POINTER(_i), ctypes.c_char_p, _i]),
    'pcgan_conv2d_workspace_bytes': (_sz, [_dp, _i]),
    'pcgan_conv2d_fwd': (_i, [_dp, _vp, _vp, _vp, _vp, _i, _f, _vp, _sz, _vp]),
    'pcgan_conv2d_bwd_data': (_i, [_dp, _vp, _vp, _vp, _vp, _vp, _sz, _vp]),
    'pcgan_conv2d_packed_bytes': (_sz, [_dp, _i]),
    'pcgan_conv2d_pack_weights': (_i, [_dp, _i, _vp, _vp, _vp]),
    'pcgan_conv2d_fwd_packed': (_i, [_dp, _vp, _vp, _vp, _vp, _i, _f, _vp, _sz, _vp]),
    'pcgan_conv2d_bwd_data_packed': (_i, [_dp, _vp, _vp, _vp, _vp, _vp, _sz, _vp]),
    'pcgan_conv2d_bwd_weight': (_i, [_dp, _vp, _vp, _vp, _i, _vp, _sz, _vp]),
    'pcgan_channel_sum': (_i, [_vp, _vp, _vp, _i, _i, _i, _i, _i, _vp]),
    'pcgan_act_bwd': (_i, [_vp, _vp, _vp, _sz, _i, _f, _i, _vp]),
    'pcgan_act_fwd': (_i, [_vp, _vp, _sz, _i, _f, _i, _vp]),
    'pcgan_concat_z': (_i, [_vp, _vp, _vp, _i, _i, _i, _i, _i, _i, _vp]),
    'pcgan_add': (_i, [_vp, _vp, _vp, _sz, _i, _vp]),
    'pcgan_scale': (_i, [_vp, _vp, _f, _vp, _sz, _i, _vp]),
    'pcgan_cast': (_i, [_vp, _i, _vp, _i, _sz, _vp]),
    'pcgan_channel_scale': (_i, [_vp, _vp, _vp, _i, _i, _f, _i, _vp]),
    'pcgan_plane_stats': (_i, [_vp, _vp, _vp, _i, _i, _i, _vp]),
    'pcgan_bn_merge': (_i, [_vp, _vp, _vp, _vp, _vp, _vp, _i, _i, _i, _f, _vp]),
    'pcgan_in_running_update': (_i, [_vp, _vp, _vp, _vp, _i, _i, _i, _f, _vp]),
    'pcgan_norm_act_fwd': (_i, [_vp, _vp, _vp, _vp, _vp, _vp, _vp, _vp, _i, _i, _i, _i, _f, _i, _f, _i, _vp]),
    'pcgan_norm_bwd_stats': (_i, [_vp, _vp, _vp, _vp, _vp, _vp, _vp, _i, _i, _i, _i, _f, _i, _f, _i, _vp]),
    'pcgan_norm_bwd_apply': (_i, [_vp, _vp, _vp, _vp, _vp, _vp, _vp, _vp, _vp, _vp, _vp, _i, _i, _i, _i, _f, _i, _f, _i, _vp]),
    'pcgan_bn_bwd_reduce': (_i, [_vp, _vp, _vp, _vp, _i, _i, _vp]),
    'pcgan_bn_stats_merged': (_i, [_vp, _vp, _vp, _vp, _vp, _vp, _vp, _vp, _vp, _i, _i, _i, _f, _i, _vp]),
    'pcgan_bn_bwd_stats_reduced': (_i, [_vp, _vp, _vp, _vp, _vp, _vp, _vp, _vp, _vp, _vp, _i, _i, _i, _f, _i, _f, _i, _vp]),
    'pcgan_bn_fwd_fused': (_i, [_vp, _vp, _vp, _vp, _vp, _vp, _vp, _vp, _vp, _vp, _vp, _i, _i, _i, _f, _f, _i, _f, _i, _vp]),
    'pcgan_bn_bwd_fused': (_i, [_vp, _vp, _vp, _vp, _vp, _vp, _vp, _vp, _vp, _vp, _vp, _i, _i, _i, _f, _i, _f, _i, _vp]),
    'pcgan_instnorm_fwd': (_i, [_vp, _vp, _vp, _vp, _vp, _vp, _i, _i, _i, _f, _i, _f, _i, _vp]),
    'pcgan_instnorm_bwd': (_i, [_vp, _vp, _vp, _vp, _vp, _vp, _vp, _vp, _vp, _i, _i, _i, _f, _i, _f, _i, _vp]),
    'pcgan_instnorm_fused': (_i, [_i]),
    'pcgan_sum_planes': (_i, [_vp, _vp, _i, _i, _i, _vp]),
    'pcgan_maxpool_fwd': (_i, [_vp, _vp, _vp, _i, _i, _i, _i, _i, _i, _i, _i, _i, _vp]),
    'pcgan_maxpool_bwd': (_i, [_vp, _vp, _vp, _i, _i, _i, _i, _i, _i, _i, _i, _i, _vp]),
    'pcgan_global_pool_fwd': (_i, [_vp, _vp, _vp, _i, _i, _i, _i, _vp]),
    'pcgan_global_pool_bwd': (_i, [_vp, _vp, _vp, _i, _i, _i, _i, _vp]),
    'pcgan_bilinear_fwd': (_i, [_vp, _vp, _i, _i, _i, _i, _i, _i, _vp]),
    'pcgan_bilinear_bwd': (_i, [_vp, _vp, _i, _i, _i, _i, _i, _i, _vp]),
    'pcgan_bce_loss': (_i, [_vp, _vp, _vp, _vp, _i, _i, _f, _vp, _sz, _i, _vp]),
    'pcgan_l1_loss': (_i, [_vp, _vp, _vp, _vp, _sz, _f, _vp, _sz, _i, _vp]),
    'pcgan_mse_loss': (_i, [_vp, _vp, _vp, _vp, _sz, _f, _vp, _sz, _i, _vp]),
    'pcgan_loss_workspace_bytes': (_sz, [_sz]),
    'pcgan_adam_step': (_i, [_vp, _vp, _vp, _vp, _sz, _f, _f, _f, _f, _i, _vp]),
    'pcgan_adam_step_dev': (_i, [_vp, _vp, _vp, _vp, _sz, _vp, _vp, _f, _f, _f, _vp]),
    'pcgan_conv2d_bsplit_supported': (_i, [_dp]),
    'pcgan_conv2d_bsplit_packed_bytes': (_sz, [_dp]),
    'pcgan_conv2d_bsplit_pack': (_i, [_dp, _vp, _vp, _vp]),
    'pcgan_conv2d_fwd_bsplit': (_i, [_dp, _vp, _vp, _vp, _vp, _i, _f, _vp]),
    'pcgan_conv2d_bsplit_dgrad_supported': (_i, [_dp]),
    'pcgan_conv2d_bsplit_dgrad_packed_bytes': (_sz, [_dp]),
    'pcgan_conv2d_bsplit_dgrad_pack': (_i, [_dp, _vp, _vp, _vp]),
    'pcgan_conv2d_bwd_data_bsplit': (_i, [_dp, _vp, _vp, _vp, _vp]),
    'pcgan_conv2d_bsplit_wgrad_supported': (_i, [_dp]),
    'pcgan_conv2d_bsplit_wgrad_workspace_bytes': (_sz, [_dp]),
    'pcgan_conv2d_bwd_weight_bsplit': (_i, [_dp, _vp, _vp, _vp, _i, _vp, _sz, _vp]),
    'pcgan_absmax_slots': (_i, [_sz]),
    'pcgan_absmax': (_i, [_vp, _sz, _i, _vp, _i, _vp]),
    'pcgan_amax_audit': (_i, [_vp, _i, _vp, _i, _vp, _vp]),
    'pcgan_conv2d_hsplit_supported': (_i, [_dp, _i]),
    'pcgan_conv2d_hsplit_packed_bytes': (_sz, [_dp, _i]),
    'pcgan_conv2d_hsplit_pack': (_i, [_dp, _i, _vp, _vp, _vp]),
    'pcgan_conv2d_fwd_hsplit': (_i, [_dp, _vp, _vp, _i, _vp, _vp, _vp, _i, _f, _vp]),
    'pcgan_conv2d_bwd_data_hsplit': (_i, [_dp, _vp, _vp, _i, _vp, _vp, _vp]),
    'pcgan_conv2d_bwd_data_hsplit_add': (_i, [_dp, _vp, _vp, _i, _vp, _vp, _vp, _vp]),
    'pcgan_event_create': (_i, [ctypes.POINTER(_vp)]),
    'pcgan_event_destroy': (_i, [_vp]),
    'pcgan_resblock_supported': (_i, [_rp]),
    'pcgan_resblock_wgrad_workspace_bytes': (_sz, [_rp]),
    'pcgan_resblock_fwd': (_i, [_rp, _vp, _vp, _i, _vp, _vp, _vp, _vp, _vp, _vp, _vp, _vp, _vp, _vp, _vp, _vp, _vp, _vp, _vp]),
    'pcgan_resblock_bwd': (_i, [_rp, _vp, _vp, _vp, _i, _vp, _vp, _vp, _vp, _vp, _vp, _vp, _vp, _vp, _vp, _vp, _vp, _vp, _vp, _vp, _vp,
                                _vp, _sz, _vp, _vp, _vp]),
    'pcgan_set_nonfinite_counter': (_i, [_vp]),
    'pcgan_set_option': (_i, [ctypes.c_char_p, _i]),
    'pcgan_get_option': (_i, [ctypes.c_char_p, _vp]),
    'pcgan_timer_enable': (_i, [_i]),
    'pcgan_timer_read': (_i, [_i, _vp, _i]),
    'pcgan_igemm_last_launch': (_i, [ctypes.POINTER(_i), _i]),
    'pcgan_wgrad_last_launch': (_i, [ctypes.POINTER(_i), _i]),
    'pcgan_conv2d_hgemm_supported': (_i, [_dp, _i]),
    'pcgan_conv2d_hgemm_pack': (_i, [_dp, _i, _vp, _vp, _vp, _vp]),
    'pcgan_conv2d_fwd_packed_hsplit': (_i, [_dp, _vp, _vp, _i, _vp, _vp, _vp, _vp, _i, _f, _vp, _sz, _vp]),
    'pcgan_conv2d_bwd_data_packed_hsplit': (_i, [_dp, _vp, _vp, _i, _vp, _vp, _vp, _vp, _vp, _sz, _vp]),
    'pcgan_conv2d_thin_supported': (_i, [_dp, _i]),
    'pcgan_conv2d_thin_packed_bytes': (_sz, [_dp, _i]),
    'pcgan_conv2d_thin_workspace_bytes': (_sz, [_dp, _i]),
    'pcgan_conv2d_thin_pack': (_i, [_dp, _i, _vp, _vp, _vp]),
    'pcgan_conv2d_fwd_thin': (_i, [_dp, _vp, _vp, _i, _vp, _vp, _vp, _i, _f, _vp]),
    'pcgan_conv2d_bwd_data_thin': (_i, [_dp, _vp, _vp, _i, _vp, _vp, _vp, _sz, _vp]),
    'pcgan_conv2d_hsplit_wgrad_supported': (_i, [_dp]),
    'pcgan_conv2d_hsplit_wgrad_inline': (_i, [_dp]),
    'pcgan_conv2d_hsplit_wgrad_workspace_bytes': (_sz, [_dp]),
    'pcgan_conv2d_bwd_weight_hsplit': (_i, [_dp, _vp, _vp, _i, _vp, _vp, _i, _vp, _i, _vp, _sz, _vp]),
    'pcgan_restrunk_fwd': (_i, [_rp, _i, _vp, _vp, _i] + [_vp] * 8 + [_vp] * 6 + [_vp]),
    'pcgan_restrunk_bwd': (_i, [_rp, _i, _vp, _vp, _vp, _i] + [_vp] * 6 + [_vp] * 6 + [_vp] * 6 + [_vp, _sz, _vp, _vp, _vp]),
    'pcgan_conv2d_wgrad_direct_supported': (_i, [_dp]),
    'pcgan_conv2d_wgrad_rowring_supported': (_i, [_dp]),
    'pcgan_conv2d_wgrad_rowring_workspace_bytes': (_sz, [_dp]),
    'pcgan_conv2d_bwd_weight_rowring': (_i, [_dp, _vp, _vp, _i, _vp, _vp, _i, _vp, _i, _vp, _sz, _vp]),
    'pcgan_conv2d_wgrad_direct_workspace_bytes': (_sz, [_dp]),
    'pcgan_conv2d_bwd_weight_direct': (_i, [_dp, _vp, _vp, _i, _vp, _vp, _i, _vp, _i, _vp, _sz, _vp]),
    'pcgan_image_transform_band': (_i, [_ip, _vp, ctypes.POINTER(_i), ctypes.POINTER(_i)]),
    'pcgan_image_transform': (_i, [_ip, _vp, _vp, _vp, _vp, _vp, _vp, _vp, _i, _i, _i, _vp]),
    'pcgan_image_resize_u8': (_i, [_ip, _vp, _vp, _vp, _vp, _vp, _vp, _i, _i, _i, _vp]),
    'pcgan_image_affine': (_i, [_ip, _vp, _vp, _vp, _vp, _i, _vp]),
    'pcgan_iconv_supported': (_i, [_icp]),
    'pcgan_iconv_packed_bytes': (_sz, [_icp]),
    'pcgan_iconv_pack': (_i, [_icp, _i, _vp, _vp, _vp, _vp, _vp, _f, _vp, _vp]),
    'pcgan_iconv_fwd': (_i, [_icp, _vp, _vp, _vp, _i, _vp]),
    'pcgan_maxpool_slice_fwd': (_i, [_vp, _vp, _i, _i, _i, _i, _i, _i, _i, _i, _i, _i, _i, _vp]),
    'pcgan_inception_prep': (_i, [_vp, _vp, _i, _i, _i, _i, _i, _i, _vp, _vp, _i, _vp]),
    'pcgan_linear_softmax_fwd': (_i, [_vp, _vp, _vp, _vp, _vp, _i, _i, _i, _i, _vp]),
    'pcgan_linear_ce_workspace_bytes': (_sz, [_i]),
    'pcgan_linear_ce_fwd': (_i, [_vp, _vp, _vp, _vp, _vp, _vp, _vp, _vp, _vp, _vp, _vp, _sz, _i, _i, _i, _i, _vp]),
    'pcgan_linear_bwd': (_i, [_vp, _vp, _vp, _vp, _vp, _vp, _i, _i, _i, _i, _i, _vp]),
    'pcgan_proj_head_fwd': (_i, [_vp] * 8 + [_i] * 7 + [_vp]),
    'pcgan_proj_head_bwd_workspace_bytes': (_sz, [_i, _i]),
    'pcgan_proj_head_bwd': (_i, [_vp] * 14 + [_sz] + [_i] * 8 + [_vp]),
    'pcgan_pool_mse_workspace_bytes': (_sz, [_i]),
    'pcgan_pool_mse_fwd': (_i, [_vp] * 8 + [_sz] + [_i] * 4 + [_f, _f, _i, _vp]),
    'pcgan_skip_join_fwd': (_i, [_vp] * 3 + [_i] * 7 + [_vp]),
    'pcgan_skip_join_bwd': (_i, [_vp] * 5 + [_i] * 7 + [_vp]),
}

_lib = None


def load():
    global _lib
    if _lib is not None:
        return _lib
    if not os.path.exists(LIB_PATH):
        raise RuntimeError(
            'pcgan_amd: %s not found -- build it with `python -c "import __graft_entry__ as g; g.build()"` '
            '(or `make -C pc-gan_amd/csrc`). There is no fallback path.' % LIB_PATH)
    import torch
    bundled = os.path.join(os.path.dirname(torch.__file__), 'lib', 'libamdhip64.so')
    if os.path.exists(bundled):
        ctypes.CDLL(bundled, mode=ctypes.RTLD_GLOBAL)
    lib = ctypes.CDLL(LIB_PATH)
    for name, (res, args) in SIGNATURES.items():
        fn = getattr(lib, name)
        fn.restype = res
        fn.argtypes = args
    _lib = lib
    _options_from_environment(lib)
    return lib


_ENV_OPTIONS = (('PCGAN_BSPLIT_HALO', 'bsplit_halo', int), ('PCGAN_WGRAD_GEN', 'wgrad_gen', int), ('PCGAN_WGRAD_PADCOPY', 'wgrad_padcopy', int),
                ('PCGAN_WGRAD_CW', 'wgrad_cw', int), ('PCGAN_HGEMM', 'hgemm_bf16', int), ('PCGAN_WGRAD_DIRECT', 'wgrad_direct', int),
                ('PCGAN_WGD_LOOK', 'wgd_look', int), ('PCGAN_WGRAD_ROWRING', 'wgrad_rowring', int))


def _options_from_environment(lib):
    for env, key, conv in _ENV_OPTIONS:
        v = os.environ.get(env)
        if v not in (None, ''):
            set_option(key, conv(v), lib)


def set_option(key, value, lib=None):
    lib = lib or load()
    if lib.pcgan_set_option(key.encode(), int(value)) != 0:
        msg = lib.pcgan_last_error()
        raise RuntimeError('pcgan_hip set_option failed: %s' % (msg.decode() if msg else '?'))


def get_option(key):
    v = ctypes.c_int(0)
    if load().pcgan_get_option(key.encode(), ctypes.byref(v)) != 0:
        raise RuntimeError('pcgan_hip get_option: unknown option %r' % key)
    return v.value


def check(status, what):
    if status != 0:
        msg = load().pcgan_last_error()
        raise RuntimeError('pcgan_hip %s failed (status %d): %s' % (what, status, msg.decode() if msg else '?'))
```

### pc-gan_amd/hip/ops.py

```python
import collections
import ctypes
import os

import torch

from . import lib as _L
from .lib import ConvDesc, ResBlockDesc, ACT_NONE, F32, BF16

_vp = ctypes.c_void_p


def _p(t):
    return _vp(t.data_ptr()) if t is not None else _vp(0)


_DEVICE_INDEX = []


def _raw_stream():
    if not _DEVICE_INDEX:
        _DEVICE_INDEX.append(torch.cuda.current_device())
    return torch._C._cuda_getCurrentRawStream(_DEVICE_INDEX[0])


# ... 237 lines not shown
THIN = os.environ.get('PCGAN_THIN', '1') == '1'
THIN_WGRAD = os.environ.get('PCGAN_THIN_WGRAD', '1') == '1'
WGRAD_INLINE_BIG = os.environ.get('PCGAN_WGRAD_INLINE_BIG', '1') != '0'
THIN_MASK = int(os.environ.get('PCGAN_THIN_MASK', '7'))


AMAX_STATS = {'attached': 0, 'computed': 0}
ROUTE_STATS = {}


def _count_route(pass_, route, n=1):
    k = (pass_, route)
    ROUTE_STATS[k] = ROUTE_STATS.get(k, 0) + n


def _want_maxima(dt, C):
    return HSPLIT and dt == F32 and C % 16 == 0


def _attach_amax(t, pmax, event=None):
    t._pcgan_amax = (t._version, pmax, _raw_stream(), event)


def amax_of(x):
    ent = x.__dict__.get('_pcgan_amax')
    if ent is not None and ent[0] == x._version:
        AMAX_STATS['attached'] += 1
        if ent[2] != _raw_stream():
            cur = torch.cuda.current_stream()
            if len(ent) > 3 and ent[3] is not None:
                cur.wait_event(ent[3])
            ent[1].record_stream(cur)
        if AMAX_AUDIT_EVERY and AMAX_STATS['attached'] % AMAX_AUDIT_EVERY == 0:
            _audit_amax(x, ent[1])
        return ent[1]
    AMAX_STATS['computed'] += 1
    lib = _L.load()
    slots = int(lib.pcgan_absmax_slots(x.numel()))
    out = torch.empty(slots, dtype=torch.float32, device=x.device)
    _L.check(lib.pcgan_absmax(_p(x), x.numel(), _DTYPES[x.dtype], _p(out), slots, _stream()), 'absmax')
    ev = torch.cuda.Event()
    ev.record(torch.cuda.current_stream())
    _attach_amax(x, out, ev)
    return out


AMAX_AUDIT_EVERY = int(os.environ.get('PCGAN_AMAX_AUDIT', '64') or 0)
AMAX_STATS['audited'] = 0


def _audit_amax(x, claimed):
    _sentinel()
    cnt = _SENTINEL.get('audit')
    if cnt is None or x.dtype != torch.float32:
        return
    lib = _L.load()
    slots = int(lib.pcgan_absmax_slots(x.numel()))
    fresh = torch.empty(slots, dtype=torch.float32, device=x.device)
    _L.check(lib.pcgan_absmax(_p(x), x.numel(), F32, _p(fresh), slots, _stream()), 'absmax')
    _L.check(lib.pcgan_amax_audit(_p(claimed), claimed.numel(), _p(fresh), slots, _vp(cnt.data_ptr()), _stream()), 'amax_audit')
    AMAX_STATS['audited'] += 1


_PackForm = collections.namedtuple('_PackForm', 'query pack lib_pass rows')
_PACK_FORMS = {
    _L.PASS_FWD: _PackForm('pcgan_conv2d_packed_bytes', 'pcgan_conv2d_pack_weights', _L.PASS_FWD, None),
    _L.PASS_BWD_DATA: _PackForm('pcgan_conv2d_packed_bytes', 'pcgan_conv2d_pack_weights', _L.PASS_BWD_DATA, None),
    PASS_FWD_BSPLIT: _PackForm('pcgan_conv2d_bsplit_packed_bytes', 'pcgan_conv2d_bsplit_pack', None, None),
    PASS_BWD_BSPLIT: _PackForm('pcgan_conv2d_bsplit_dgrad_packed_bytes', 'pcgan_conv2d_bsplit_dgrad_pack', None, None),
    PASS_FWD_HSPLIT: _PackForm('pcgan_conv2d_hsplit_packed_bytes', 'pcgan_conv2d_hsplit_pack', _L.PASS_FWD, None),
    PASS_BWD_HSPLIT: _PackForm('pcgan_conv2d_hsplit_packed_bytes', 'pcgan_conv2d_hsplit_pack', _L.PASS_BWD_DATA, None),
    PASS_FWD_HGEMM: _PackForm('pcgan_conv2d_packed_bytes', 'pcgan_conv2d_hgemm_pack', _L.PASS_FWD, 'K'),
    PASS_BWD_HGEMM: _PackForm('pcgan_conv2d_packed_bytes', 'pcgan_conv2d_hgemm_pack', _L.PASS_BWD_DATA, 'C'),
    PASS_FWD_THIN: _PackForm('pcgan_conv2d_thin_packed_bytes', 'pcgan_conv2d_thin_pack', _L.PASS_FWD, None),
    PASS_BWD_THIN: _PackForm('pcgan_conv2d_thin_packed_bytes', 'pcgan_conv2d_thin_pack', _L.PASS_BWD_DATA, None),
}


def _packed_weights(lib, d, pass_, w, cache, want_rowmax=False):
    key = (pass_, d.stride, d.pad, d.pad_mode, d.dtype)
    stamp = _weight_stamp(w)
    ent = cache.get(key)
    if ent is not None and ent[0] == stamp:
        if ent[3] != _raw_stream():
            torch.cuda.current_stream().wait_event(ent[2])
        return (ent[1], ent[4]) if want_rowmax else ent[1]
    cur = torch.cuda.current_stream()
    form = _PACK_FORMS[pass_]
    head = (ctypes.byref(d),) if form.lib_pass is None else (ctypes.byref(d), form.lib_pass)
    nb = max(int(getattr(lib, form.query)(*head)), 256)
    if ent is not None and ent[1].numel() == nb and ent[1].device == w.device:
        buf = ent[1]
        if ent[3] != cur.cuda_stream:
            for st in list(_side.values()) + list(_branch.values()):
                cur.wait_stream(st)
    else:
        buf = _ws(nb, w.device)
    rowmax = None
    if form.rows is not None:
        rows = getattr(d, form.rows)
        rowmax = ent[4] if (ent is not None and len(ent) > 4 and ent[4] is not None and ent[4].numel() == rows and buf is ent[1]) else \
            torch.empty(rows, dtype=torch.float32, device=w.device)
    out = (_p(buf),) if rowmax is None else (_p(rowmax), _p(buf))
    _L.check(getattr(lib, form.pack)(*head, _p(w), *out, _stream()), form.pack[len('pcgan_'):])
    ev = torch.cuda.Event()
    ev.record(cur)
    cache[key] = (stamp, buf, ev, cur.cuda_stream, rowmax)
    return (buf, rowmax) if want_rowmax else buf


_PLANS = {}


def clear_plans():
    _PLANS.clear()
    _RB_PLANS.clear()


class _Plan(object):
    __slots__ = ('d', 'dref', 'P', 'Q', 'ws_bytes', 'route', 'pack_pass', 'amax', 'launch')


NONFINITE_CHECK = os.environ.get('PCGAN_NONFINITE_CHECK', '1') != '0'
_SENTINEL = {}


def _sentinel():
    if not NONFINITE_CHECK or 'word' in _SENTINEL or not torch.cuda.is_available():
        return
    _SENTINEL['word'] = torch.zeros(1, dtype=torch.int32, device='cuda')
    _SENTINEL['audit'] = torch.zeros(3, dtype=torch.int32, device='cuda')
    _L.check(_L.load().pcgan_set_nonfinite_counter(_vp(_SENTINEL['word'].data_ptr())), 'set_nonfinite_counter')


def nonfinite_count(reset=True):
    w = _SENTINEL.get('word')
    if w is None:
        return 0
    n = int(w.item())
    if n and reset:
        w.zero_()
    return n


def stale_maxima_count(reset=True):
    a = _SENTINEL.get('audit')
    if a is None:
        return (0, 0, 0)
    v = tuple(int(t) for t in a.tolist())
    if any(v) and reset:
        a.zero_()
    return v


def check_nonfinite(where=''):
    small, large, other = stale_maxima_count()
    if small or large or other:
        raise RuntimeError('pcgan_amd: stale operand maxima%s: %d audited tensor(s) held MORE than the maximum attached to them (fp16 overflow), '
                           '%d held less than 2^-8 of it (the fp16 route silently loses >= 8 bits of every product), %d differed otherwise -- '
                           'a tensor was rewritten through .data / a raw pointer after a kernel attached its maxima; rewrite it through an '
                           'op, or drop `_pcgan_amax`' % ((' (' + where + ')') if where else '', small, large, other))
    n = nonfinite_count()
    if n:
        raise RuntimeError('pcgan_amd: %d wave(s) of the fp16-route convolutions produced inf / NaN%s -- an operand exceeded the maximum its '
                           'scale was derived from (a tensor rewritten through .data / a raw pointer after its maxima were attached?) or the '
                           'inputs were already non-finite' % (n, (' (' + where + ')') if where else ''))


_Route = collections.namedtuple('_Route', 'name pack_pass cond ws_bytes amax launch')


def _n(t):
    return t.numel() if t is not None else 0


def _fwd_hsplit(lib, d, x, xmax, pk, wmax, bias, y, act, slope, ws):
    _L.check(lib.pcgan_conv2d_fwd_hsplit(d, _p(x), _p(xmax), _n(xmax), _p(pk), _p(bias), _p(y), act, slope, _stream()), 'conv2d_fwd_hsplit')


def _fwd_hgemm(lib, d, x, xmax, pk, wmax, bias, y, act, slope, ws):
    _L.check(lib.pcgan_conv2d_fwd_packed_hsplit(d, _p(x), _p(xmax), _n(xmax), _p(pk), _p(wmax), _p(bias), _p(y), act, slope, _p(ws), ws.numel(),
                                                _stream()), 'conv2d_fwd_packed_hsplit')


def _fwd_bsplit(lib, d, x, xmax, pk, wmax, bias, y, act, slope, ws):
    _L.check(lib.pcgan_conv2d_fwd_bsplit(d, _p(x), _p(pk), _p(bias), _p(y), act, slope, _stream()), 'conv2d_fwd_bsplit')


def _fwd_thin(lib, d, x, xmax, pk, wmax, bias, y, act, slope, ws):
    _L.check(lib.pcgan_conv2d_fwd_thin(d, _p(x), _p(xmax), _n(xmax), _p(pk), _p(bias), _p(y), act, slope, _stream()), 'conv2d_fwd_thin')


def _fwd_packed(lib, d, x, xmax, pk, wmax, bias, y, act, slope, ws):
    _L.check(lib.pcgan_conv2d_fwd_packed(d, _p(x), _p(pk), _p(bias), _p(y), act, slope, _p(ws), ws.numel(), _stream()), 'conv2d_fwd_packed')


def _dgrad_hsplit(lib, d, dy, dmax, pk, wmax, bias, dx, ws):
    _L.check(lib.pcgan_conv2d_bwd_data_hsplit(d, _p(dy), _p(dmax), _n(dmax), _p(pk), _p(dx), _stream()), 'conv2d_bwd_data_hsplit')

# ... 955 lines not shown
```

### pc-gan_amd/hip/optim.py

```python
import torch

from . import ops

_ALIGN = 64


class FusedAdam(torch.optim.Optimizer):
    def __init__(self, params, lr=1e-3, betas=(0.9, 0.999), eps=1e-8):
        params = list(params)
        if not params:
            raise ValueError('FusedAdam: empty parameter list')
        super().__init__(params, dict(lr=lr, betas=betas, eps=eps))
        ps = self.param_groups[0]['params']
        dev = ps[0].device
        for p in ps:
            if p.dtype != torch.float32 or p.device != dev:
                raise RuntimeError('FusedAdam: all parameters must be fp32 on one device')
        offs, total = [], 0
        for p in ps:
            offs.append(total)
            total += (p.numel() + _ALIGN - 1) // _ALIGN * _ALIGN
        self.flat = torch.zeros(total, dtype=torch.float32, device=dev)
        self.gflat = torch.zeros(total, dtype=torch.float32, device=dev)
        self.exp_avg = torch.zeros(total, dtype=torch.float32, device=dev)
        self.exp_avg_sq = torch.zeros(total, dtype=torch.float32, device=dev)
        self._views = []
        with torch.no_grad():
            for p, o in zip(ps, offs):
                n = p.numel()
                self.flat[o:o + n].copy_(p.data.reshape(-1))
                p.data = self.flat[o:o + n].view(p.shape)
                gv = self.gflat[o:o + n].view(p.shape)
                p.grad = gv
                p._pcgan_fused_grad = True
                self._views.append((p, gv))
        self.numel = sum(p.numel() for p in ps)
        self.step_dev = torch.zeros(1, dtype=torch.int32, device=dev)
        self.lr_dev = torch.full((1,), float(lr), dtype=torch.float32, device=dev)
        self._lr_host = float(lr)
        self._step_host = 0
        self.updated = None

    def zero_grad(self, set_to_none=False):
        if self.updated is not None and self.gflat.is_cuda:
            torch.cuda.current_stream(self.gflat.device).wait_event(self.updated)
        else:
            ops.join_side_stream()
        self.gflat.zero_()
        for p, gv in self._views:
            if p.grad is None or p.grad.data_ptr() != gv.data_ptr():
                p.grad = gv

    def rebind(self):
        with torch.no_grad():
            o = 0
            for p, gv in self._views:
                n = p.numel()
                view = self.flat[o:o + n].view(p.shape)
                if p.data.data_ptr() != view.data_ptr():
                    view.copy_(p.data)
                    p.data = view
                o += (n + _ALIGN - 1) // _ALIGN * _ALIGN

    def step_on_grad_stream(self, before=None):
        cur = torch.cuda.current_stream(self.flat.device)
        side = ops.side_stream_for(cur)
        side.wait_stream(cur)
        with torch.cuda.stream(side):
            if before is not None:
                before()
            self.step(_joined=True)
            ev = torch.cuda.Event()
            ev.record(side)
        self.updated = ev
        ops._side_state['dirty'] = True
        return ev

    @torch.no_grad()
    def step(self, closure=None, _joined=False):
        if not _joined:
            ops.join_side_stream(force=True)
            self.updated = None
        g = self.param_groups[0]
        lr = float(g['lr'])
        if lr != self._lr_host:
            self.lr_dev.fill_(lr)
            self._lr_host = lr
        for p, gv in self._views:
            if p.grad is not None and p.grad.data_ptr() != gv.data_ptr():
                gv.copy_(p.grad)
                p.grad = gv
        if self.flat.is_cuda:
            ops.adam_step_dev(self.flat, self.gflat, self.exp_avg, self.exp_avg_sq, self.lr_dev, self.step_dev,
                              g['betas'][0], g['betas'][1], g['eps'], params=[p for p, _ in self._views])
        else:
            raise RuntimeError('FusedAdam: parameters are on %s; the HIP path needs a GPU (no CPU fallback)'
                               % self.flat.device)
        self._step_host += 1
```

Baseline: 1199 images/sec.

## Batch all weight repacks into one recorded pack plan run after Adam step

```diff
diff --git a/include/pcgan_hip.h b/include/pcgan_hip.h
--- a/include/pcgan_hip.h
+++ b/include/pcgan_hip.h
@@ -288,6 +288,25 @@
 #define PCGAN_WGRAD_STRIP 4
 int pcgan_wgrad_last_launch(int* info, int n);
 
+#define PCGAN_PACK_WEIGHTS 0
+#define PCGAN_PACK_HGEMM 1
+#define PCGAN_PACK_BSPLIT 2
+#define PCGAN_PACK_BSPLIT_DGRAD 3
+#define PCGAN_PACK_HSPLIT 4
+#define PCGAN_PACK_THIN 5
+typedef struct {
+    pcgan_conv_desc desc;
+    int form, pass;
+    const float* w;
+    float* rowmax;
+    void* packed;
+} pcgan_pack_item;
+int pcgan_pack_plan_create(const pcgan_pack_item* items, int n, void** plan);
+int pcgan_pack_plan_run(void* plan, pcgan_stream_t s);
+int pcgan_pack_plan_launches(void* plan);
+int pcgan_pack_plan_jobs(void* plan, int level);
+int pcgan_pack_plan_destroy(void* plan);
+
 #ifdef __cplusplus
 }
 #endif
diff --git a/pc-gan_amd/csrc/amax.hip b/pc-gan_amd/csrc/amax.hip
--- a/pc-gan_amd/csrc/amax.hip
+++ b/pc-gan_amd/csrc/amax.hip
@@ -1,4 +1,5 @@
-#include "common.h"
+#include "pack_kernels.h"
+#include "pack_plan.h"
 
 namespace pcgan {
 
@@ -44,25 +45,13 @@
     }
 }
 
-__global__ void __launch_bounds__(256) weight_row_absmax_kernel(const float* __restrict__ w, int K, int C, int T, int by_c, float* __restrict__ out) {
-    const int row = blockIdx.x;
-    float m = 0.f;
-    if (!by_c) {
-        const float* p = w + (size_t)row * C * T;
-        for (int i = threadIdx.x; i < C * T; i += 256) m = fmaxf(m, fabsf(p[i]));
-    } else {
-        for (int i = threadIdx.x; i < K * T; i += 256) {
-            const int k = i / T, t = i - k * T;
-            m = fmaxf(m, fabsf(w[((size_t)k * C + row) * T + t]));
-        }
-    }
-    __shared__ float red[16];
-    m = block_max(m, red);
-    if (threadIdx.x == 0) out[row] = m;
-}
+__global__ void __launch_bounds__(256) weight_row_absmax_kernel(RowAbsmaxArgs a) { weight_row_absmax_body(a, blockIdx.x, gridDim.x); }
 
 int launch_weight_row_absmax(const float* w, int K, int C, int T, int by_c, float* out, hipStream_t st) {
-    hipLaunchKernelGGL(weight_row_absmax_kernel, dim3((unsigned)(by_c ? C : K)), dim3(256), 0, st, w, K, C, T, by_c, out);
+    const RowAbsmaxArgs a = {w, out, K, C, T, by_c};
+    const unsigned blocks = (unsigned)(by_c ? C : K);
+    if (pack_recording()) return pack_record(PK_ROW_ABSMAX, blocks, false, &a, sizeof(a));
+    hipLaunchKernelGGL(weight_row_absmax_kernel, dim3(blocks), dim3(256), 0, st, a);
     PCGAN_LAUNCH_CHECK();
     return 0;
 }
diff --git a/pc-gan_amd/csrc/bsplit.h b/pc-gan_amd/csrc/bsplit.h
--- a/pc-gan_amd/csrc/bsplit.h
+++ b/pc-gan_amd/csrc/bsplit.h
@@ -1,21 +1,11 @@
 #pragma once
-#include "common.h"
+#include "pack_kernels.h"
 
 namespace pcgan {
 
 typedef float f32x16 __attribute__((ext_vector_type(16)));
-typedef __bf16 bf16x8 __attribute__((ext_vector_type(8)));
-typedef _Float16 f16x8 __attribute__((ext_vector_type(8)));
-typedef unsigned int u32x4 __attribute__((ext_vector_type(4)));
 static constexpr unsigned BS_OOB = 0x80000000u;
 static constexpr int BS_MAXTAP = 25;
-
-__device__ __forceinline__ void split3(float x, __bf16& h, __bf16& m, __bf16& l) {
-    h = (__bf16)x;
-    const float r1 = x - (float)h;
-    m = (__bf16)r1;
-    l = (__bf16)(r1 - (float)m);
-}
 
 struct BsplitArgs {
     const void* X;
@@ -33,35 +23,6 @@
 
 enum { BS_FWD_ZERO = 0, BS_FWD_REFLECT = 1, BS_DGRAD_REFLECT = 2, BS_WGRAD = 3 };
 
-__device__ __forceinline__ void pack_store8(__bf16* __restrict__ A, size_t e, size_t per_piece, int np, float wscale, const float (&v)[8]) {
-    if (np == 2) {
-        f16x8 h, l;
-#pragma unroll
-        for (int j = 0; j < 8; ++j) {
-            _Float16 x, y;
-            split2h(v[j] * wscale, x, y);
-            h[j] = x;
-            l[j] = y;
-        }
-        *reinterpret_cast<f16x8*>(reinterpret_cast<_Float16*>(A) + 8 * e) = h;
-        *reinterpret_cast<f16x8*>(reinterpret_cast<_Float16*>(A) + per_piece + 8 * e) = l;
-        return;
-    }
-    bf16x8 h, mm, l;
-#pragma unroll
-    for (int j = 0; j < 8; ++j) {
-        __bf16 x, y, z;
-        split3(v[j], x, y, z);
-        h[j] = x;
-        mm[j] = y;
-        l[j] = z;
-    }
-    *reinterpret_cast<bf16x8*>(A + 8 * e) = h;
-    if (np == 3) {
-        *reinterpret_cast<bf16x8*>(A + per_piece + 8 * e) = mm;
-        *reinterpret_cast<bf16x8*>(A + 2 * per_piece + 8 * e) = l;
-    }
-}
 
 enum { BH_FWD = 0, BH_DGRAD = 1 };
 
diff --git a/pc-gan_amd/csrc/bsplit_pack.hip b/pc-gan_amd/csrc/bsplit_pack.hip
--- a/pc-gan_amd/csrc/bsplit_pack.hip
+++ b/pc-gan_amd/csrc/bsplit_pack.hip
@@ -1,66 +1,28 @@
 #include "bsplit.h"
+#include "pack_plan.h"
 
 namespace pcgan {
 
-__global__ void bsplit_pack_kernel(const float* __restrict__ w, __bf16* __restrict__ A, int M, int C, int T, int nMt, int nst,
-                                   int bm_shift, int np, const float* __restrict__ rowmax = nullptr) {
-    const int BM = 128 << bm_shift;
-    const size_t per_piece = (size_t)nMt * nst * 16 * BM;
-    for (size_t e = blockIdx.x * (size_t)blockDim.x + threadIdx.x; e < per_piece / 8; e += (size_t)gridDim.x * blockDim.x) {
-        const int row = (int)(e & (BM - 1)), half = (int)((e >> (7 + bm_shift)) & 1);
-        const size_t q = e >> (8 + bm_shift);
-        const int st = (int)(q % nst), mt = (int)(q / nst);
-        const int m = mt * BM + row, c0 = (st / T) * 16 + half * 8, tap = st % T;
-        float v[8];
-#pragma unroll
-        for (int j = 0; j < 8; ++j) v[j] = m < M ? w[((size_t)m * C + c0 + j) * T + tap] : 0.f;
-        const float wscale = (np == 2 && m < M) ? pow2_scale(rowmax[m]) : 1.f;
-        pack_store8(A, e, per_piece, np, wscale, v);
-    }
-}
+__global__ void bsplit_pack_kernel(BsplitPackArgs a) { bsplit_pack_body(a, blockIdx.x, gridDim.x); }
+__global__ void bsplit_pack_dgrad_kernel(BsplitPackDgradArgs a) { bsplit_pack_dgrad_body(a, blockIdx.x, gridDim.x); }
 
 int launch_bsplit_pack(const float* w, void* packed, int M, int C, int T, int nMt, int nst, int bm, int np, const float* rowmax, hipStream_t st) {
     const size_t per_piece = (size_t)nMt * nst * 16 * bm;
-    hipLaunchKernelGGL(bsplit_pack_kernel, dim3(capped_blocks(per_piece / 8, 256, 4096)), dim3(256), 0, st, w, (__bf16*)packed, M, C, T, nMt, nst,
-                       bm == 256 ? 1 : 0, np, rowmax);
+    const BsplitPackArgs a = {w, (__bf16*)packed, rowmax, M, C, T, nMt, nst, bm == 256 ? 1 : 0, np};
+    const unsigned blocks = capped_blocks(per_piece / 8, 256, 4096);
+    if (pack_recording()) return pack_record(PK_BSPLIT, blocks, rowmax != nullptr, &a, sizeof(a));
+    hipLaunchKernelGGL(bsplit_pack_kernel, dim3(blocks), dim3(256), 0, st, a);
     PCGAN_LAUNCH_CHECK();
     return 0;
-}
-
-__global__ void bsplit_pack_dgrad_kernel(const float* __restrict__ w, __bf16* __restrict__ A, int K, int C, int nMt, int nst, int bm_shift,
-                                         int np, const float* __restrict__ rowmax = nullptr, int nphase = 3) {
-    const int BM = 128 << bm_shift;
-    const size_t per_piece = (size_t)nMt * nst * 16 * BM, per_phase = (size_t)np * per_piece;
-    const size_t per_phase8 = per_piece / 8;
-    for (size_t i = blockIdx.x * (size_t)blockDim.x + threadIdx.x; i < (size_t)nphase * per_phase8; i += (size_t)gridDim.x * blockDim.x) {
-        const int phase = (int)(i / per_phase8);
-        const size_t e = i - (size_t)phase * per_phase8;
-        const int row = (int)(e & (BM - 1)), half = (int)((e >> (7 + bm_shift)) & 1);
-        const size_t q = e >> (8 + bm_shift);
-        const int st = (int)(q % nst), mt = (int)(q / nst);
-        const int c = mt * BM + row, k0 = (st / 9) * 16 + half * 8, tap = st % 9;
-        const int rp = tap / 3, sp = tap - rp * 3;
-        const bool fold = (phase == 1 && rp == 0) || (phase == 2 && rp == 2);
-        float v[8];
-#pragma unroll
-        for (int j = 0; j < 8; ++j) {
-            v[j] = 0.f;
-            if (c < C) {
-                const float* wk = w + ((size_t)(k0 + j) * C + c) * 9;
-                v[j] = wk[(2 - rp) * 3 + (2 - sp)];
-                if (fold) v[j] += wk[rp * 3 + (2 - sp)];
-            }
-        }
-        const float wscale = (np == 2 && c < C) ? pow2_scale(rowmax[c]) : 1.f;
-        pack_store8(A + (size_t)phase * per_phase, e, per_piece, np, wscale, v);
-    }
 }
 
 int launch_bsplit_pack_dgrad(const float* w, void* packed, int K, int C, int nMt, int nst, int bm, int np, const float* rowmax, int nphase,
                              hipStream_t st) {
     const size_t total = (size_t)nphase * nMt * nst * 2 * bm;
-    hipLaunchKernelGGL(bsplit_pack_dgrad_kernel, dim3(capped_blocks(total, 256, 4096)), dim3(256), 0, st, w, (__bf16*)packed, K, C, nMt, nst,
-                       bm == 256 ? 1 : 0, np, rowmax, nphase);
+    const BsplitPackDgradArgs a = {w, (__bf16*)packed, rowmax, K, C, nMt, nst, bm == 256 ? 1 : 0, np, nphase};
+    const unsigned blocks = capped_blocks(total, 256, 4096);
+    if (pack_recording()) return pack_record(PK_BSPLIT_DGRAD, blocks, rowmax != nullptr, &a, sizeof(a));
+    hipLaunchKernelGGL(bsplit_pack_dgrad_kernel, dim3(blocks), dim3(256), 0, st, a);
     PCGAN_LAUNCH_CHECK();
     return 0;
 }
diff --git a/pc-gan_amd/csrc/hgemm.hip b/pc-gan_amd/csrc/hgemm.hip
--- a/pc-gan_amd/csrc/hgemm.hip
+++ b/pc-gan_amd/csrc/hgemm.hip
@@ -1,9 +1,8 @@
 #include "igemm.h"
+#include "pack_kernels.h"
+#include "pack_plan.h"
 
 namespace pcgan {
-
-typedef _Float16 f16x8 __attribute__((ext_vector_type(8)));
-typedef _Float16 f16x4 __attribute__((ext_vector_type(4)));
 
 typedef __bf16 bf16x8v __attribute__((ext_vector_type(8)));
 typedef __bf16 bf16x4v __attribute__((ext_vector_type(4)));
@@ -317,24 +316,13 @@
 
 using namespace pcgan;
 
-__global__ void __launch_bounds__(256) hgemm_presplit_kernel(float* __restrict__ A, int M, int Kp4, const float* __restrict__ rowmax) {
-    const size_t n4 = (size_t)M * Kp4;
-    for (size_t i = (size_t)blockIdx.x * 256 + threadIdx.x; i < n4; i += (size_t)gridDim.x * 256) {
-        const float s = pow2_scale(rowmax[i / Kp4]);
-        const float4 v = reinterpret_cast<const float4*>(A)[i];
-        f16x4 h, l;
-        _Float16 x, y;
-        split2h(v.x * s, x, y); h[0] = x; l[0] = y;
-        split2h(v.y * s, x, y); h[1] = x; l[1] = y;
-        split2h(v.z * s, x, y); h[2] = x; l[2] = y;
-        split2h(v.w * s, x, y); h[3] = x; l[3] = y;
-        reinterpret_cast<f16x4*>(A)[2 * i] = h;
-        reinterpret_cast<f16x4*>(A)[2 * i + 1] = l;
-    }
-}
+__global__ void __launch_bounds__(256) hgemm_presplit_kernel(PresplitArgs a) { hgemm_presplit_body(a, blockIdx.x, gridDim.x); }
 
 int pcgan::launch_hgemm_presplit(float* A, int M, int Kp4, const float* rowmax, hipStream_t st) {
-    hipLaunchKernelGGL(hgemm_presplit_kernel, dim3(capped_blocks((size_t)M * Kp4, 256, 2048)), dim3(256), 0, st, A, M, Kp4, rowmax);
+    const PresplitArgs a = {A, rowmax, M, Kp4};
+    const unsigned blocks = capped_blocks((size_t)M * Kp4, 256, 2048);
+    if (pack_recording()) return pack_record(PK_PRESPLIT, blocks, true, &a, sizeof(a));
+    hipLaunchKernelGGL(hgemm_presplit_kernel, dim3(blocks), dim3(256), 0, st, a);
     PCGAN_LAUNCH_CHECK();
     return 0;
 }
diff --git a/pc-gan_amd/csrc/igemm_conv.hip b/pc-gan_amd/csrc/igemm_conv.hip
--- a/pc-gan_amd/csrc/igemm_conv.hip
+++ b/pc-gan_amd/csrc/igemm_conv.hip
@@ -1,4 +1,6 @@
 #include "igemm.h"
+#include "pack_kernels.h"
+#include "pack_plan.h"
 #include <stdlib.h>
 #include <mutex>
 
@@ -32,89 +34,27 @@
     }
 }
 
-__global__ void repack_fwd_kernel(const float* __restrict__ w, float* __restrict__ A, int K, int C, int Cgp,
-                                  int RS, int chunked) {
-    const int Kp = RS * Cgp;
-    const size_t total = (size_t)K * Kp;
-    for (size_t i = blockIdx.x * (size_t)blockDim.x + threadIdx.x; i < total; i += (size_t)gridDim.x * blockDim.x) {
-        const int k = (int)(i / Kp);
-        const int j = (int)(i - (size_t)k * Kp);
-        int tap, c;
-        if (chunked) {
-            const int t2 = j >> 4;
-            const int cc = t2 / RS;
-            tap = t2 - cc * RS;
-            c = cc * 16 + (j & 15);
-        } else {
-            tap = j / Cgp;
-            c = j - tap * Cgp;
-        }
-        A[i] = (c < C) ? w[((size_t)k * C + c) * RS + tap] : 0.f;
-    }
-}
-__global__ void repack_bwd_kernel(const float* __restrict__ w, float* __restrict__ A, int K, int C, int Kgp,
-                                  int R, int S, int r0, int s0, int tstep, int nR, int nS, int chunked, int fold) {
-    const int Kp = nR * nS * Kgp;
-    const size_t total = (size_t)C * Kp;
-    for (size_t i = blockIdx.x * (size_t)blockDim.x + threadIdx.x; i < total; i += (size_t)gridDim.x * blockDim.x) {
-        const int c = (int)(i / Kp);
-        const int j = (int)(i - (size_t)c * Kp);
-        int t, k;
-        if (chunked) {
-            const int t2 = j >> 4;
-            const int kc = t2 / (nR * nS);
-            t = t2 - kc * (nR * nS);
-            k = kc * 16 + (j & 15);
-        } else {
-            t = j / Kgp;
-            k = j - t * Kgp;
-        }
-        const int ri = t / nS, sj = t - ri * nS;
-        const int r = r0 + ri * tstep, s = s0 + sj * tstep;
-        float v = (k < K) ? w[(((size_t)k * C + c) * R + r) * S + s] : 0.f;
-        if (k < K && fold == 1 && r == R - 1) v += w[(((size_t)k * C + c) * R + 0) * S + s];
-        if (k < K && fold == 2 && r == 0) v += w[(((size_t)k * C + c) * R + (R - 1)) * S + s];
-        A[i] = v;
-    }
-}
-
-struct PackBwdArgs {
-    const float* w;
-    int K, C, Kgp, R, S, tstep, chunked, n;
-    struct Entry {
-        float* A;
-        int r0, s0, nR, nS, fold;
-    } e[16];
-};
-__global__ void repack_bwd_multi_kernel(PackBwdArgs a) {
-    const PackBwdArgs::Entry& E = a.e[blockIdx.y];
-    const int RS = E.nR * E.nS;
-    const int Kp = RS * a.Kgp;
-    const size_t total = (size_t)a.C * Kp;
-    for (size_t i = blockIdx.x * (size_t)blockDim.x + threadIdx.x; i < total; i += (size_t)gridDim.x * blockDim.x) {
-        const int c = (int)(i / Kp);
-        const int j = (int)(i - (size_t)c * Kp);
-        int t, k;
-        if (a.chunked) {
-            const int t2 = j >> 4;
-            const int kc = t2 / RS;
-            t = t2 - kc * RS;
-            k = kc * 16 + (j & 15);
-        } else {
-            t = j / a.Kgp;
-            k = j - t * a.Kgp;
-        }
-        const int ri = t / E.nS, sj = t - ri * E.nS;
-        const int r = E.r0 + ri * a.tstep, sx = E.s0 + sj * a.tstep;
-        float v = 0.f;
-        if (k < a.K) {
-            const float* wk = a.w + ((size_t)k * a.C + c) * a.R * a.S;
-            v = wk[r * a.S + sx];
-            if (E.fold == 1 && r == a.R - 1) v += wk[sx];
-            if (E.fold == 2 && r == 0) v += wk[(a.R - 1) * a.S + sx];
-        }
-        E.A[i] = v;
-    }
+__global__ void repack_fwd_kernel(RepackFwdArgs a) { repack_fwd_body(a, blockIdx.x, gridDim.x); }
+__global__ void repack_bwd_kernel(RepackBwdArgs a) { repack_bwd_body(a, blockIdx.x, gridDim.x); }
+__global__ void repack_bwd_multi_kernel(PackBwdArgs a) { repack_bwd_multi_body(a, blockIdx.y * gridDim.x + blockIdx.x, gridDim.x * gridDim.y); }
+
+static int launch_repack_fwd(const RepackFwdArgs& a, unsigned blocks, hipStream_t st) {
+    if (pack_recording()) return pack_record(PK_REPACK_FWD, blocks, false, &a, sizeof(a));
+    hipLaunchKernelGGL(repack_fwd_kernel, dim3(blocks), dim3(256), 0, st, a);
+    PCGAN_LAUNCH_CHECK();
+    return 0;
+}
+static int launch_repack_bwd(const RepackBwdArgs& a, unsigned blocks, hipStream_t st) {
+    if (pack_recording()) return pack_record(PK_REPACK_BWD, blocks, false, &a, sizeof(a));
+    hipLaunchKernelGGL(repack_bwd_kernel, dim3(blocks), dim3(256), 0, st, a);
+    PCGAN_LAUNCH_CHECK();
+    return 0;
+}
+static int launch_repack_bwd_multi(const PackBwdArgs& a, unsigned blocks_per_entry, hipStream_t st) {
+    if (pack_recording()) return pack_record(PK_REPACK_BWD_MULTI, blocks_per_entry * (unsigned)a.n, false, &a, sizeof(a));
+    hipLaunchKernelGGL(repack_bwd_multi_kernel, dim3(blocks_per_entry, a.n), dim3(256), 0, st, a);
+    PCGAN_LAUNCH_CHECK();
+    return 0;
 }
 
 template <typename TA>
@@ -333,9 +273,8 @@
 static int pack_fwd(const pcgan_conv_desc* d, const float* w, float* A, hipStream_t st) {
     const int Cgp = round4(d->C), RS = d->R * d->S;
     const size_t total = (size_t)d->K * RS * Cgp;
-    hipLaunchKernelGGL(repack_fwd_kernel, dim3(capped_blocks(total, 256, 4096)), dim3(256), 0, st, w, A, d->K, d->C, Cgp, RS,
-                       (int)chunked_k(d->C, d->K, d->R, d->S));
-    PCGAN_LAUNCH_CHECK();
+    const RepackFwdArgs ra = {w, A, d->K, d->C, Cgp, RS, (int)chunked_k(d->C, d->K, d->R, d->S)};
+    if (int e = launch_repack_fwd(ra, capped_blocks(total, 256, 4096), st)) return e;
     if (d->K <= 4) {
         if (int e = launch_transpose4(A, A + total, d->K, RS * Cgp, st)) return e;
         if (int e = launch_pack_strip(A, A + total + (size_t)RS * Cgp * 4, d->K, d->C, Cgp, d->R, d->S, st)) return e;
@@ -478,9 +417,8 @@
             const BwdPhase& p = pl.ph[i];
             float* A = packed + p.a_off;
             const size_t total = (size_t)d->C * p.nR * p.nS * Kgp;
-            hipLaunchKernelGGL(repack_bwd_kernel, dim3(capped_blocks(total, 256, 4096)), dim3(256), 0, st, w, A, d->K, d->C, Kgp, d->R,
-                               d->S, p.r0, p.s0, d->stride, p.nR, p.nS, chunked, 0);
-            PCGAN_LAUNCH_CHECK();
+            const RepackBwdArgs ra = {w, A, d->K, d->C, Kgp, d->R, d->S, p.r0, p.s0, d->stride, p.nR, p.nS, chunked, 0};
+            if (int e = launch_repack_bwd(ra, capped_blocks(total, 256, 4096), st)) return e;
             if (int e = launch_transpose4(A, packed + p.at_off, d->C, p.nR * p.nS * Kgp, st)) return e;
             if (int e = launch_pack_strip(A, packed + p.as_off, d->C, d->K, Kgp, p.nR, p.nS, st)) return e;
         }
@@ -498,9 +436,7 @@
         PackBwdArgs::Entry& pe = pk.e[i];
         pe.A = packed + p.a_off; pe.r0 = p.r0; pe.s0 = p.s0; pe.nR = p.nR; pe.nS = p.nS; pe.fold = p.fold;
     }
-    hipLaunchKernelGGL(repack_bwd_multi_kernel, dim3(capped_blocks(max_total, 256, 2048), pk.n), dim3(256), 0, st, pk);
-    PCGAN_LAUNCH_CHECK();
-    return 0;
+    return launch_repack_bwd_multi(pk, capped_blocks(max_total, 256, 2048), st);
 }
 
 static int conv2d_bwd_data_impl(const pcgan_conv_desc* d, const void* dy, const float* w, const float* packed,
diff --git a/pc-gan_amd/csrc/pack_kernels.h b/pc-gan_amd/csrc/pack_kernels.h
--- /dev/null
+++ b/pc-gan_amd/csrc/pack_kernels.h
@@ -0,0 +1,325 @@
+#pragma once
+#include "common.h"
+
+namespace pcgan {
+
+typedef __bf16 bf16x8 __attribute__((ext_vector_type(8)));
+typedef _Float16 f16x8 __attribute__((ext_vector_type(8)));
+typedef _Float16 f16x4 __attribute__((ext_vector_type(4)));
+typedef unsigned int u32x4 __attribute__((ext_vector_type(4)));
+
+__device__ __forceinline__ void split3(float x, __bf16& h, __bf16& m, __bf16& l) {
+    h = (__bf16)x;
+    const float r1 = x - (float)h;
+    m = (__bf16)r1;
+    l = (__bf16)(r1 - (float)m);
+}
+
+__device__ __forceinline__ void pack_store8(__bf16* __restrict__ A, size_t e, size_t per_piece, int np, float wscale, const float (&v)[8]) {
+    if (np == 2) {
+        f16x8 h, l;
+#pragma unroll
+        for (int j = 0; j < 8; ++j) {
+            _Float16 x, y;
+            split2h(v[j] * wscale, x, y);
+            h[j] = x;
+            l[j] = y;
+        }
+        *reinterpret_cast<f16x8*>(reinterpret_cast<_Float16*>(A) + 8 * e) = h;
+        *reinterpret_cast<f16x8*>(reinterpret_cast<_Float16*>(A) + per_piece + 8 * e) = l;
+        return;
+    }
+    bf16x8 h, mm, l;
+#pragma unroll
+    for (int j = 0; j < 8; ++j) {
+        __bf16 x, y, z;
+        split3(v[j], x, y, z);
+        h[j] = x;
+        mm[j] = y;
+        l[j] = z;
+    }
+    *reinterpret_cast<bf16x8*>(A + 8 * e) = h;
+    if (np == 3) {
+        *reinterpret_cast<bf16x8*>(A + per_piece + 8 * e) = mm;
+        *reinterpret_cast<bf16x8*>(A + 2 * per_piece + 8 * e) = l;
+    }
+}
+
+struct RowAbsmaxArgs {
+    const float* w;
+    float* out;
+    int K, C, T, by_c;
+};
+__device__ __forceinline__ void weight_row_absmax_body(const RowAbsmaxArgs& a, unsigned vb, unsigned ) {
+    const float* __restrict__ w = a.w;
+    const int K = a.K, C = a.C, T = a.T;
+    const int row = (int)vb;
+    float m = 0.f;
+    if (!a.by_c) {
+        const float* p = w + (size_t)row * C * T;
+        for (int i = threadIdx.x; i < C * T; i += 256) m = fmaxf(m, fabsf(p[i]));
+    } else {
+        for (int i = threadIdx.x; i < K * T; i += 256) {
+            const int k = i / T, t = i - k * T;
+            m = fmaxf(m, fabsf(w[((size_t)k * C + row) * T + t]));
+        }
+    }
+    __shared__ float red[16];
+    m = block_max(m, red);
+    if (threadIdx.x == 0) a.out[row] = m;
+}
+
+struct RepackFwdArgs {
+    const float* w;
+    float* A;
+    int K, C, Cgp, RS, chunked;
+};
+__device__ __forceinline__ void repack_fwd_body(const RepackFwdArgs& a, unsigned vb, unsigned vgrid) {
+    const float* __restrict__ w = a.w;
+    float* __restrict__ A = a.A;
+    const int K = a.K, C = a.C, Cgp = a.Cgp, RS = a.RS, chunked = a.chunked;
+    const int Kp = RS * Cgp;
+    const size_t total = (size_t)K * Kp;
+    for (size_t i = vb * (size_t)256 + threadIdx.x; i < total; i += (size_t)vgrid * 256) {
+        const int k = (int)(i / Kp);
+        const int j = (int)(i - (size_t)k * Kp);
+        int tap, c;
+        if (chunked) {
+            const int t2 = j >> 4;
+            const int cc = t2 / RS;
+            tap = t2 - cc * RS;
+            c = cc * 16 + (j & 15);
+        } else {
+            tap = j / Cgp;
+            c = j - tap * Cgp;
+        }
+        A[i] = (c < C) ? w[((size_t)k * C + c) * RS + tap] : 0.f;
+    }
+}
+struct RepackBwdArgs {
+    const float* w;
+    float* A;
+    int K, C, Kgp, R, S, r0, s0, tstep, nR, nS, chunked, fold;
+};
+__device__ __forceinline__ void repack_bwd_body(const RepackBwdArgs& a, unsigned vb, unsigned vgrid) {
+    const float* __restrict__ w = a.w;
+    float* __restrict__ A = a.A;
+    const int K = a.K, C = a.C, Kgp = a.Kgp, R = a.R, S = a.S, r0 = a.r0, s0 = a.s0, tstep = a.tstep, nR = a.nR, nS = a.nS;
+    const int chunked = a.chunked, fold = a.fold;
+    const int Kp = nR * nS * Kgp;
+    const size_t total = (size_t)C * Kp;
+    for (size_t i = vb * (size_t)256 + threadIdx.x; i < total; i += (size_t)vgrid * 256) {
+        const int c = (int)(i / Kp);
+        const int j = (int)(i - (size_t)c * Kp);
+        int t, k;
+        if (chunked) {
+            const int t2 = j >> 4;
+            const int kc = t2 / (nR * nS);
+            t = t2 - kc * (nR * nS);
+            k = kc * 16 + (j & 15);
+        } else {
+            t = j / Kgp;
+            k = j - t * Kgp;
+        }
+        const int ri = t / nS, sj = t - ri * nS;
+        const int r = r0 + ri * tstep, s = s0 + sj * tstep;
+        float v = (k < K) ? w[(((size_t)k * C + c) * R + r) * S + s] : 0.f;
+        if (k < K && fold == 1 && r == R - 1) v += w[(((size_t)k * C + c) * R + 0) * S + s];
+        if (k < K && fold == 2 && r == 0) v += w[(((size_t)k * C + c) * R + (R - 1)) * S + s];
+        A[i] = v;
+    }
+}
+
+struct PackBwdArgs {
+    const float* w;
+    int K, C, Kgp, R, S, tstep, chunked, n;
+    struct Entry {
+        float* A;
+        int r0, s0, nR, nS, fold;
+    } e[16];
+};
+__device__ __forceinline__ void repack_bwd_multi_body(const PackBwdArgs& a, unsigned vb, unsigned vgrid) {
+    const unsigned gx = vgrid / (unsigned)a.n, by = vb / gx, bx = vb - by * gx;
+    const PackBwdArgs::Entry& E = a.e[by];
+    const int RS = E.nR * E.nS;
+    const int Kp = RS * a.Kgp;
+    const size_t total = (size_t)a.C * Kp;
+    for (size_t i = bx * (size_t)256 + threadIdx.x; i < total; i += (size_t)gx * 256) {
+        const int c = (int)(i / Kp);
+        const int j = (int)(i - (size_t)c * Kp);
+        int t, k;
+        if (a.chunked) {
+            const int t2 = j >> 4;
+            const int kc = t2 / RS;
+            t = t2 - kc * RS;
+            k = kc * 16 + (j & 15);
+        } else {
+            t = j / a.Kgp;
+            k = j - t * a.Kgp;
+        }
+        const int ri = t / E.nS, sj = t - ri * E.nS;
+        const int r = E.r0 + ri * a.tstep, sx = E.s0 + sj * a.tstep;
+        float v = 0.f;
+        if (k < a.K) {
+            const float* wk = a.w + ((size_t)k * a.C + c) * a.R * a.S;
+            v = wk[r * a.S + sx];
+            if (E.fold == 1 && r == a.R - 1) v += wk[sx];
+            if (E.fold == 2 && r == 0) v += wk[(a.R - 1) * a.S + sx];
+        }
+        E.A[i] = v;
+    }
+}
+
+struct Transpose4Args {
+    const float* A;
+    float* At;
+    int M, Kp;
+};
+__device__ __forceinline__ void transpose4_body(const Transpose4Args& a, unsigned vb, unsigned vgrid) {
+    const float* __restrict__ A = a.A;
+    float* __restrict__ At = a.At;
+    const int M = a.M, Kp = a.Kp;
+    const int total = Kp * 4;
+    for (int i = vb * 256 + threadIdx.x; i < total; i += vgrid * 256) {
+        const int k = i >> 2, m = i & 3;
+        At[i] = m < M ? A[(size_t)m * Kp + k] : 0.f;
+    }
+}
+struct PackStripArgs {
+    const float* A;
+    float* Ws;
+    int M, Cg, Cgp, nR, nS;
+};
+__device__ __forceinline__ void pack_strip_body(const PackStripArgs& a, unsigned vb, unsigned vgrid) {
+    const float* __restrict__ A = a.A;
+    float* __restrict__ Ws = a.Ws;
+    const int M = a.M, Cg = a.Cg, Cgp = a.Cgp, nR = a.nR, nS = a.nS;
+    const int total = Cg * nS * 32;
+    const int Kp = nR * nS * Cgp;
+    for (int i = vb * 256 + threadIdx.x; i < total; i += vgrid * 256) {
+        const int m = i & 3, ri = (i >> 2) & 7, cs = i >> 5;
+        const int c = cs / nS, sj = cs - c * nS;
+        Ws[i] = (m < M && ri < nR) ? A[(size_t)m * Kp + (ri * nS + sj) * Cgp + c] : 0.f;
+    }
+}
+
+struct PresplitArgs {
+    float* A;
+    const float* rowmax;
+    int M, Kp4;
+};
+__device__ __forceinline__ void hgemm_presplit_body(const PresplitArgs& a, unsigned vb, unsigned vgrid) {
+    float* __restrict__ A = a.A;
+    const float* __restrict__ rowmax = a.rowmax;
+    const int Kp4 = a.Kp4;
+    const size_t n4 = (size_t)a.M * Kp4;
+    for (size_t i = (size_t)vb * 256 + threadIdx.x; i < n4; i += (size_t)vgrid * 256) {
+        const float s = pow2_scale(rowmax[i / Kp4]);
+        const float4 v = reinterpret_cast<const float4*>(A)[i];
+        f16x4 h, l;
+        _Float16 x, y;
+        split2h(v.x * s, x, y); h[0] = x; l[0] = y;
+        split2h(v.y * s, x, y); h[1] = x; l[1] = y;
+        split2h(v.z * s, x, y); h[2] = x; l[2] = y;
+        split2h(v.w * s, x, y); h[3] = x; l[3] = y;
+        reinterpret_cast<f16x4*>(A)[2 * i] = h;
+        reinterpret_cast<f16x4*>(A)[2 * i + 1] = l;
+    }
+}
+
+struct BsplitPackArgs {
+    const float* w;
+    __bf16* A;
+    const float* rowmax;
+    int M, C, T, nMt, nst, bm_shift, np;
+};
+__device__ __forceinline__ void bsplit_pack_body(const BsplitPackArgs& a, unsigned vb, unsigned vgrid) {
+    const float* __restrict__ w = a.w;
+    __bf16* __restrict__ A = a.A;
+    const float* __restrict__ rowmax = a.rowmax;
+    const int M = a.M, C = a.C, T = a.T, nMt = a.nMt, nst = a.nst, bm_shift = a.bm_shift, np = a.np;
+    const int BM = 128 << bm_shift;
+    const size_t per_piece = (size_t)nMt * nst * 16 * BM;
+    for (size_t e = vb * (size_t)256 + threadIdx.x; e < per_piece / 8; e += (size_t)vgrid * 256) {
+        const int row = (int)(e & (BM - 1)), half = (int)((e >> (7 + bm_shift)) & 1);
+        const size_t q = e >> (8 + bm_shift);
+        const int st = (int)(q % nst), mt = (int)(q / nst);
+        const int m = mt * BM + row, c0 = (st / T) * 16 + half * 8, tap = st % T;
+        float v[8];
+#pragma unroll
+        for (int j = 0; j < 8; ++j) v[j] = m < M ? w[((size_t)m * C + c0 + j) * T + tap] : 0.f;
+        const float wscale = (np == 2 && m < M) ? pow2_scale(rowmax[m]) : 1.f;
+        pack_store8(A, e, per_piece, np, wscale, v);
+    }
+}
+
+struct BsplitPackDgradArgs {
+    const float* w;
+    __bf16* A;
+    const float* rowmax;
+    int K, C, nMt, nst, bm_shift, np, nphase;
+};
+__device__ __forceinline__ void bsplit_pack_dgrad_body(const BsplitPackDgradArgs& a, unsigned vb, unsigned vgrid) {
+    const float* __restrict__ w = a.w;
+    __bf16* __restrict__ A = a.A;
+    const float* __restrict__ rowmax = a.rowmax;
+    const int C = a.C, nMt = a.nMt, nst = a.nst, bm_shift = a.bm_shift, np = a.np, nphase = a.nphase;
+    const int BM = 128 << bm_shift;
+    const size_t per_piece = (size_t)nMt * nst * 16 * BM, per_phase = (size_t)np * per_piece;
+    const size_t per_phase8 = per_piece / 8;
+    for (size_t i = vb * (size_t)256 + threadIdx.x; i < (size_t)nphase * per_phase8; i += (size_t)vgrid * 256) {
+        const int phase = (int)(i / per_phase8);
+        const size_t e = i - (size_t)phase * per_phase8;
+        const int row = (int)(e & (BM - 1)), half = (int)((e >> (7 + bm_shift)) & 1);
+        const size_t q = e >> (8 + bm_shift);
+        const int st = (int)(q % nst), mt = (int)(q / nst);
+        const int c = mt * BM + row, k0 = (st / 9) * 16 + half * 8, tap = st % 9;
+        const int rp = tap / 3, sp = tap - rp * 3;
+        const bool fold = (phase == 1 && rp == 0) || (phase == 2 && rp == 2);
+        float v[8];
+#pragma unroll
+        for (int j = 0; j < 8; ++j) {
+            v[j] = 0.f;
+            if (c < C) {
+                const float* wk = w + ((size_t)(k0 + j) * C + c) * 9;
+                v[j] = wk[(2 - rp) * 3 + (2 - sp)];
+                if (fold) v[j] += wk[rp * 3 + (2 - sp)];
+            }
+        }
+        const float wscale = (np == 2 && c < C) ? pow2_scale(rowmax[c]) : 1.f;
+        pack_store8(A + (size_t)phase * per_phase, e, per_piece, np, wscale, v);
+    }
+}
+
+struct ThinPackArgs {
+    const float* w;
+    const float* rowmax;
+    u32x4* out;
+    int M, G, T, nst, transposed, Cin, total;
+};
+__device__ __forceinline__ void thin_pack_body(const ThinPackArgs& a, unsigned vb, unsigned ) {
+    const float* __restrict__ w = a.w;
+    const float* __restrict__ rowmax = a.rowmax;
+    const int M = a.M, G = a.G, T = a.T, nst = a.nst, transposed = a.transposed, Cin = a.Cin;
+    const int e = vb * 256 + threadIdx.x;
+    if (e >= a.total) return;
+    const int ln = e & 63, piece = (e >> 6) & 1, st = (e >> 7) % nst, mb = (e >> 7) / nst;
+    const int lo = ln & 31, hi = ln >> 5, m = mb * 32 + lo;
+    const float s = m < M ? pow2_scale(rowmax[m]) : 1.f;
+    f16x8 v;
+#pragma unroll
+    for (int i = 0; i < 8; ++i) {
+        const int k = st * 16 + hi * 8 + i, tap = k >> 2, g = k & 3;
+        float x = 0.f;
+        if (m < M && tap < T && g < G) x = transposed ? w[((size_t)g * Cin + m) * T + (T - 1 - tap)] : w[((size_t)m * Cin + g) * T + tap];
+        _Float16 h, l;
+        split2h(x * s, h, l);
+        v[i] = piece ? l : h;
+    }
+    a.out[e] = __builtin_bit_cast(u32x4, v);
+}
+
+bool pack_recording();
+int pack_record(int kind, unsigned blocks, bool has_rowmax, const void* args, size_t nbytes);
+
+}
diff --git a/pc-gan_amd/csrc/pack_plan.h b/pc-gan_amd/csrc/pack_plan.h
--- /dev/null
+++ b/pc-gan_amd/csrc/pack_plan.h
@@ -0,0 +1,107 @@
+#pragma once
+#include <stddef.h>
+#include <stdint.h>
+#include <string.h>
+#include <vector>
+
+#if defined(__HIPCC__)
+#define PCGAN_HD __host__ __device__
+#else
+#define PCGAN_HD
+#endif
+
+namespace pcgan {
+
+enum PackKind {
+    PK_ROW_ABSMAX = 0, PK_REPACK_FWD, PK_REPACK_BWD, PK_REPACK_BWD_MULTI, PK_BSPLIT, PK_BSPLIT_DGRAD,
+    PK_PRESPLIT, PK_TRANSPOSE4, PK_PACK_STRIP, PK_THIN,
+    PK_KINDS
+};
+
+static inline int pack_level(int kind, bool has_rowmax) {
+    if (kind == PK_BSPLIT || kind == PK_BSPLIT_DGRAD) return has_rowmax ? 1 : 0;
+    return kind >= PK_PRESPLIT ? 1 : 0;
+}
+
+struct PackJobRef {
+    int kind;
+    unsigned arg_off;
+};
+
+PCGAN_HD inline int pack_find_job(const unsigned* prefix, int n, unsigned block) {
+    int lo = 0, hi = n;
+    while (hi - lo > 1) {
+        const int mid = (lo + hi) >> 1;
+        if (prefix[mid] <= block) lo = mid;
+        else hi = mid;
+    }
+    return lo;
+}
+
+struct PackLevelLayout {
+    int n;
+    unsigned blocks;
+    size_t prefix_off, jobs_off;
+};
+struct PackPlanLayout {
+    PackLevelLayout level[2];
+    size_t blob_off, bytes;
+};
+
+class PackPlanBuilder {
+public:
+    static constexpr size_t ALIGN = 16;
+    static constexpr unsigned MAX_BLOCKS = 0x7fffffffu;
+
+    bool add(int kind, unsigned blocks, bool has_rowmax, const void* args, size_t nbytes) {
+        if (kind < 0 || kind >= PK_KINDS || blocks == 0 || (nbytes && !args)) return false;
+        Level& L = lv_[pack_level(kind, has_rowmax)];
+        const unsigned before = L.prefix.back();
+        if (blocks > MAX_BLOCKS - before) return false;
+        const size_t off = (blob_.size() + ALIGN - 1) / ALIGN * ALIGN;
+        if (off + nbytes > 0xffffffffull) return false;
+        blob_.resize(off + nbytes, 0);
+        if (nbytes) memcpy(blob_.data() + off, args, nbytes);
+        L.jobs.push_back(PackJobRef{kind, (unsigned)off});
+        L.prefix.push_back(before + blocks);
+        return true;
+    }
+
+    int jobs(int level) const { return (int)lv_[level].jobs.size(); }
+    unsigned blocks(int level) const { return lv_[level].prefix.back(); }
+    const unsigned* prefix(int level) const { return lv_[level].prefix.data(); }
+    const PackJobRef* job_refs(int level) const { return lv_[level].jobs.data(); }
+
+    PackPlanLayout image(std::vector<unsigned char>& out) const {
+        PackPlanLayout lay;
+        size_t at = 0;
+        for (int l = 0; l < 2; ++l) {
+            lay.level[l].n = jobs(l);
+            lay.level[l].blocks = blocks(l);
+            lay.level[l].prefix_off = at;
+            at = up(at + lv_[l].prefix.size() * sizeof(unsigned));
+            lay.level[l].jobs_off = at;
+            at = up(at + lv_[l].jobs.size() * sizeof(PackJobRef));
+        }
+        lay.blob_off = at;
+        lay.bytes = up(at + blob_.size());
+        out.assign(lay.bytes, 0);
+        for (int l = 0; l < 2; ++l) {
+            memcpy(out.data() + lay.level[l].prefix_off, lv_[l].prefix.data(), lv_[l].prefix.size() * sizeof(unsigned));
+            if (!lv_[l].jobs.empty()) memcpy(out.data() + lay.level[l].jobs_off, lv_[l].jobs.data(), lv_[l].jobs.size() * sizeof(PackJobRef));
+        }
+        if (!blob_.empty()) memcpy(out.data() + lay.blob_off, blob_.data(), blob_.size());
+        return lay;
+    }
+
+private:
+    static size_t up(size_t v) { return (v + ALIGN - 1) / ALIGN * ALIGN; }
+    struct Level {
+        std::vector<unsigned> prefix{0u};
+        std::vector<PackJobRef> jobs;
+    };
+    Level lv_[2];
+    std::vector<unsigned char> blob_;
+};
+
+}
diff --git a/pc-gan_amd/csrc/pack_plan.hip b/pc-gan_amd/csrc/pack_plan.hip
--- /dev/null
+++ b/pc-gan_amd/csrc/pack_plan.hip
@@ -0,0 +1,121 @@
+#include "pack_kernels.h"
+#include "pack_plan.h"
+#include <new>
+
+namespace pcgan {
+
+namespace {
+thread_local PackPlanBuilder* g_recorder = nullptr;
+}
+
+bool pack_recording() { return g_recorder != nullptr; }
+
+int pack_record(int kind, unsigned blocks, bool has_rowmax, const void* args, size_t nbytes) {
+    PCGAN_CHECK(g_recorder != nullptr, "pack plan: no plan is being recorded");
+    PCGAN_CHECK(g_recorder->add(kind, blocks, has_rowmax, args, nbytes), "pack plan: job of kind %d with %u workgroups refused", kind, blocks);
+    return 0;
+}
+
+__global__ void __launch_bounds__(256) pack_plan_kernel(const unsigned* __restrict__ prefix, const PackJobRef* __restrict__ jobs, int n,
+                                                        const unsigned char* __restrict__ blob) {
+    const int j = pack_find_job(prefix, n, blockIdx.x);
+    const unsigned first = prefix[j], vb = blockIdx.x - first, vgrid = prefix[j + 1] - first;
+    const unsigned char* a = blob + jobs[j].arg_off;
+    switch (jobs[j].kind) {
+        case PK_ROW_ABSMAX: weight_row_absmax_body(*reinterpret_cast<const RowAbsmaxArgs*>(a), vb, vgrid); break;
+        case PK_REPACK_FWD: repack_fwd_body(*reinterpret_cast<const RepackFwdArgs*>(a), vb, vgrid); break;
+        case PK_REPACK_BWD: repack_bwd_body(*reinterpret_cast<const RepackBwdArgs*>(a), vb, vgrid); break;
+        case PK_REPACK_BWD_MULTI: repack_bwd_multi_body(*reinterpret_cast<const PackBwdArgs*>(a), vb, vgrid); break;
+        case PK_BSPLIT: bsplit_pack_body(*reinterpret_cast<const BsplitPackArgs*>(a), vb, vgrid); break;
+        case PK_BSPLIT_DGRAD: bsplit_pack_dgrad_body(*reinterpret_cast<const BsplitPackDgradArgs*>(a), vb, vgrid); break;
+        case PK_PRESPLIT: hgemm_presplit_body(*reinterpret_cast<const PresplitArgs*>(a), vb, vgrid); break;
+        case PK_TRANSPOSE4: transpose4_body(*reinterpret_cast<const Transpose4Args*>(a), vb, vgrid); break;
+        case PK_PACK_STRIP: pack_strip_body(*reinterpret_cast<const PackStripArgs*>(a), vb, vgrid); break;
+        case PK_THIN: thin_pack_body(*reinterpret_cast<const ThinPackArgs*>(a), vb, vgrid); break;
+        default: break;
+    }
+}
+
+struct PackPlan {
+    PackPlanLayout lay;
+    unsigned char* dev = nullptr;
+};
+
+}
+
+using namespace pcgan;
+
+static int record_item(const pcgan_pack_item& it) {
+    const pcgan_conv_desc* d = &it.desc;
+    switch (it.form) {
+        case PCGAN_PACK_WEIGHTS: return pcgan_conv2d_pack_weights(d, it.pass, it.w, (float*)it.packed, nullptr);
+        case PCGAN_PACK_HGEMM: return pcgan_conv2d_hgemm_pack(d, it.pass, it.w, it.rowmax, (float*)it.packed, nullptr);
+        case PCGAN_PACK_BSPLIT: return pcgan_conv2d_bsplit_pack(d, it.w, it.packed, nullptr);
+        case PCGAN_PACK_BSPLIT_DGRAD: return pcgan_conv2d_bsplit_dgrad_pack(d, it.w, it.packed, nullptr);
+        case PCGAN_PACK_HSPLIT: return pcgan_conv2d_hsplit_pack(d, it.pass, it.w, it.packed, nullptr);
+        case PCGAN_PACK_THIN: return pcgan_conv2d_thin_pack(d, it.pass, it.w, it.packed, nullptr);
+        default: PCGAN_CHECK(false, "pack_plan_create: unknown form %d", it.form);
+    }
+}
+
+extern "C" int pcgan_pack_plan_create(const pcgan_pack_item* items, int n, void** plan) {
+    PCGAN_CHECK(plan != nullptr && n >= 0 && (items != nullptr || n == 0), "pack_plan_create: null pointer or negative count");
+    PCGAN_CHECK(!pack_recording(), "pack_plan_create: a plan is already being recorded on this thread");
+    *plan = nullptr;
+    PackPlanBuilder b;
+    g_recorder = &b;
+    int err = 0;
+    for (int i = 0; i < n && !err; ++i) err = record_item(items[i]);
+    g_recorder = nullptr;
+    if (err) return err;
+    std::vector<unsigned char> img;
+    PackPlan* p = new (std::nothrow) PackPlan;
+    PCGAN_CHECK(p != nullptr, "pack_plan_create: out of memory");
+    p->lay = b.image(img);
+    if (p->lay.level[0].n + p->lay.level[1].n > 0) {
+        hipError_t e = hipMalloc((void**)&p->dev, img.size());
+        if (e == hipSuccess) e = hipMemcpy(p->dev, img.data(), img.size(), hipMemcpyHostToDevice);
+        if (e != hipSuccess) {
+            if (p->dev) (void)hipFree(p->dev);
+            delete p;
+            PCGAN_CHECK(false, "pack_plan_create: upload of %zu bytes failed: %s", img.size(), hipGetErrorString(e));
+        }
+    }
+    *plan = p;
+    return 0;
+}
+
+extern "C" int pcgan_pack_plan_run(void* plan, pcgan_stream_t s) {
+    PCGAN_CHECK(plan != nullptr, "pack_plan_run: null plan");
+    const PackPlan* p = (const PackPlan*)plan;
+    for (int l = 0; l < 2; ++l) {
+        const PackLevelLayout& L = p->lay.level[l];
+        if (L.n == 0) continue;
+        hipLaunchKernelGGL(pack_plan_kernel, dim3(L.blocks), dim3(256), 0, (hipStream_t)s, (const unsigned*)(p->dev + L.prefix_off),
+                           (const PackJobRef*)(p->dev + L.jobs_off), L.n, (const unsigned char*)(p->dev + p->lay.blob_off));
+        PCGAN_LAUNCH_CHECK();
+    }
+    return 0;
+}
+
+extern "C" int pcgan_pack_plan_launches(void* plan) {
+    if (!plan) return 0;
+    const PackPlan* p = (const PackPlan*)plan;
+    return (p->lay.level[0].n > 0) + (p->lay.level[1].n > 0);
+}
+
+extern "C" int pcgan_pack_plan_jobs(void* plan, int level) {
+    if (!plan || level < 0 || level > 1) return 0;
+    return ((const PackPlan*)plan)->lay.level[level].n;
+}
+
+extern "C" int pcgan_pack_plan_destroy(void* plan) {
+    if (!plan) return 0;
+    PackPlan* p = (PackPlan*)plan;
+    if (p->dev) {
+        hipError_t e = hipFree(p->dev);
+        PCGAN_CHECK(e == hipSuccess, "pack_plan_destroy: %s", hipGetErrorString(e));
+    }
+    delete p;
+    return 0;
+}
diff --git a/pc-gan_amd/csrc/pack_plan_selftest.cpp b/pc-gan_amd/csrc/pack_plan_selftest.cpp
--- /dev/null
+++ b/pc-gan_amd/csrc/pack_plan_selftest.cpp
@@ -0,0 +1,125 @@
+#include "pack_plan.h"
+#include <stdio.h>
+#include <stdlib.h>
+
+using namespace pcgan;
+
+static int g_fail = 0;
+#define EXPECT(cond)                                                   \
+    do {                                                               \
+        if (!(cond)) {                                                 \
+            fprintf(stderr, "%s:%d: %s\n", __FILE__, __LINE__, #cond); \
+            ++g_fail;                                                  \
+        }                                                              \
+    } while (0)
+
+struct Args {
+    uint64_t tag;
+    int job, blocks;
+};
+
+static void check_image(const PackPlanBuilder& b, const std::vector<Args> (&want)[2]) {
+    std::vector<unsigned char> img;
+    const PackPlanLayout lay = b.image(img);
+    EXPECT(lay.bytes == img.size() && lay.bytes % PackPlanBuilder::ALIGN == 0);
+    size_t prev_end = 0;
+    for (int l = 0; l < 2; ++l) {
+        const PackLevelLayout& L = lay.level[l];
+        const int n = (int)want[l].size();
+        EXPECT(L.n == n && b.jobs(l) == n);
+        EXPECT(L.prefix_off % PackPlanBuilder::ALIGN == 0 && L.jobs_off % PackPlanBuilder::ALIGN == 0);
+        EXPECT(L.prefix_off >= prev_end && L.jobs_off >= L.prefix_off + (size_t)(n + 1) * sizeof(unsigned));
+        prev_end = L.jobs_off + (size_t)n * sizeof(PackJobRef);
+        EXPECT(prev_end <= lay.blob_off);
+        const unsigned* prefix = reinterpret_cast<const unsigned*>(img.data() + L.prefix_off);
+        const PackJobRef* jobs = reinterpret_cast<const PackJobRef*>(img.data() + L.jobs_off);
+        EXPECT(prefix[0] == 0);
+        unsigned sum = 0;
+        for (int j = 0; j < n; ++j) {
+            EXPECT(prefix[j] == sum);
+            sum += (unsigned)want[l][j].blocks;
+            EXPECT(prefix[j + 1] == sum);
+            EXPECT(jobs[j].arg_off % PackPlanBuilder::ALIGN == 0 && lay.blob_off + jobs[j].arg_off + sizeof(Args) <= lay.bytes);
+            Args a;
+            memcpy(&a, img.data() + lay.blob_off + jobs[j].arg_off, sizeof(a));
+            EXPECT(a.tag == want[l][j].tag && a.job == want[l][j].job && a.blocks == want[l][j].blocks);
+            EXPECT(pack_level(jobs[j].kind, false) == l || jobs[j].kind == PK_BSPLIT || jobs[j].kind == PK_BSPLIT_DGRAD);
+            const unsigned probes[4] = {prefix[j], prefix[j + 1] - 1, prefix[j] + (want[l][j].blocks > 1), prefix[j + 1] - 1 - (want[l][j].blocks > 1)};
+            for (unsigned blk : probes) EXPECT(pack_find_job(prefix, n, blk) == j);
+        }
+        EXPECT(L.blocks == sum && b.blocks(l) == sum);
+        if (n > 0) {
+            EXPECT(pack_find_job(prefix, n, 0) == 0);
+            EXPECT(pack_find_job(prefix, n, sum - 1) == n - 1);
+        }
+        if (sum <= 200000)
+            for (unsigned blk = 0, j = 0; blk < sum; ++blk) {
+                while (blk >= prefix[j + 1]) ++j;
+                EXPECT(pack_find_job(prefix, n, blk) == (int)j);
+            }
+    }
+}
+
+int main() {
+    for (int k = 0; k < PK_KINDS; ++k) {
+        const bool second = k == PK_PRESPLIT || k == PK_TRANSPOSE4 || k == PK_PACK_STRIP || k == PK_THIN;
+        if (k == PK_BSPLIT || k == PK_BSPLIT_DGRAD) {
+            EXPECT(pack_level(k, false) == 0 && pack_level(k, true) == 1);
+        } else {
+            EXPECT(pack_level(k, false) == (second ? 1 : 0) && pack_level(k, true) == (second ? 1 : 0));
+        }
+    }
+    {
+        PackPlanBuilder b;
+        std::vector<Args> want[2];
+        check_image(b, want);
+        EXPECT(b.blocks(0) == 0 && b.blocks(1) == 0);
+        std::vector<unsigned char> img;
+        EXPECT(b.image(img).bytes >= 2 * sizeof(unsigned));
+    }
+    {
+        PackPlanBuilder b;
+        std::vector<Args> want[2];
+        const Args a = {0xabcdef0123456789ull, 0, 1};
+        EXPECT(b.add(PK_REPACK_FWD, 1, false, &a, sizeof(a)));
+        want[0].push_back(a);
+        EXPECT(!b.add(PK_REPACK_FWD, 0, false, &a, sizeof(a)));
+        EXPECT(!b.add(PK_KINDS, 1, false, &a, sizeof(a)));
+        EXPECT(!b.add(-1, 1, false, &a, sizeof(a)));
+        EXPECT(!b.add(PK_THIN, 1, true, nullptr, sizeof(a)));
+        EXPECT(!b.add(PK_REPACK_FWD, PackPlanBuilder::MAX_BLOCKS, false, &a, sizeof(a)));
+        check_image(b, want);
+    }
+    {
+        PackPlanBuilder b;
+        std::vector<Args> want[2];
+        const int sizes[] = {1, 2, 3, 255, 256, 257, 1, 4096, 7, 1, 1, 512};
+        for (int i = 0; i < 300; ++i) {
+            const int kind = i % PK_KINDS;
+            const bool rm = (i / PK_KINDS) % 2 == 1;
+            const int blocks = sizes[i % (int)(sizeof(sizes) / sizeof(sizes[0]))];
+            const Args a = {0x1000000ull * (uint64_t)i + 7, i, blocks};
+            EXPECT(b.add(kind, (unsigned)blocks, rm, &a, sizeof(a)));
+            want[pack_level(kind, rm)].push_back(a);
+        }
+        EXPECT(want[0].size() + want[1].size() == 300 && !want[0].empty() && !want[1].empty());
+        check_image(b, want);
+    }
+    {
+        PackPlanBuilder b;
+        const Args a = {1, 0, 0};
+        EXPECT(b.add(PK_BSPLIT, 0x40000000u, true, &a, sizeof(a)));
+        EXPECT(b.add(PK_THIN, 0x3ffffffeu, true, &a, sizeof(a)));
+        EXPECT(b.add(PK_THIN, 1, true, &a, sizeof(a)));
+        EXPECT(!b.add(PK_THIN, 1, true, &a, sizeof(a)));
+        EXPECT(b.jobs(1) == 3 && b.blocks(1) == PackPlanBuilder::MAX_BLOCKS);
+        EXPECT(pack_find_job(b.prefix(1), 3, 0x3fffffffu) == 0 && pack_find_job(b.prefix(1), 3, 0x40000000u) == 1);
+        EXPECT(pack_find_job(b.prefix(1), 3, 0x7ffffffdu) == 1 && pack_find_job(b.prefix(1), 3, 0x7ffffffeu) == 2);
+    }
+    if (g_fail) {
+        fprintf(stderr, "pack_plan_selftest: %d check(s) failed\n", g_fail);
+        return 1;
+    }
+    printf("pack_plan_selftest: ok\n");
+    return 0;
+}
diff --git a/pc-gan_amd/csrc/smallm_conv.hip b/pc-gan_amd/csrc/smallm_conv.hip
--- a/pc-gan_amd/csrc/smallm_conv.hip
+++ b/pc-gan_amd/csrc/smallm_conv.hip
@@ -1,24 +1,11 @@
 #include "igemm.h"
+#include "pack_kernels.h"
+#include "pack_plan.h"
 
 namespace pcgan {
 
-__global__ void transpose4_kernel(const float* __restrict__ A, float* __restrict__ At, int M, int Kp) {
-    const int total = Kp * 4;
-    for (int i = blockIdx.x * blockDim.x + threadIdx.x; i < total; i += gridDim.x * blockDim.x) {
-        const int k = i >> 2, m = i & 3;
-        At[i] = m < M ? A[(size_t)m * Kp + k] : 0.f;
-    }
-}
-
-__global__ void pack_strip_kernel(const float* __restrict__ A, float* __restrict__ Ws, int M, int Cg, int Cgp, int nR, int nS) {
-    const int total = Cg * nS * 32;
-    const int Kp = nR * nS * Cgp;
-    for (int i = blockIdx.x * blockDim.x + threadIdx.x; i < total; i += gridDim.x * blockDim.x) {
-        const int m = i & 3, ri = (i >> 2) & 7, cs = i >> 5;
-        const int c = cs / nS, sj = cs - c * nS;
-        Ws[i] = (m < M && ri < nR) ? A[(size_t)m * Kp + (ri * nS + sj) * Cgp + c] : 0.f;
-    }
-}
+__global__ void transpose4_kernel(Transpose4Args a) { transpose4_body(a, blockIdx.x, gridDim.x); }
+__global__ void pack_strip_kernel(PackStripArgs a) { pack_strip_body(a, blockIdx.x, gridDim.x); }
 
 template <int MODE, typename TA>
 __global__ void __launch_bounds__(256) smallm_conv_kernel(IgemmArgs a) {
@@ -335,12 +322,18 @@
 }
 
 int launch_transpose4(const float* A, float* At, int M, int Kp, hipStream_t st) {
-    hipLaunchKernelGGL(transpose4_kernel, dim3((Kp * 4 + 255) / 256), dim3(256), 0, st, A, At, M, Kp);
+    const Transpose4Args a = {A, At, M, Kp};
+    const unsigned blocks = (unsigned)((Kp * 4 + 255) / 256);
+    if (pack_recording()) return pack_record(PK_TRANSPOSE4, blocks, false, &a, sizeof(a));
+    hipLaunchKernelGGL(transpose4_kernel, dim3(blocks), dim3(256), 0, st, a);
     PCGAN_LAUNCH_CHECK();
     return 0;
 }
 int launch_pack_strip(const float* A, float* Ws, int M, int Cg, int Cgp, int nR, int nS, hipStream_t st) {
-    hipLaunchKernelGGL(pack_strip_kernel, dim3((Cg * nS * 32 + 255) / 256), dim3(256), 0, st, A, Ws, M, Cg, Cgp, nR, nS);
+    const PackStripArgs a = {A, Ws, M, Cg, Cgp, nR, nS};
+    const unsigned blocks = (unsigned)((Cg * nS * 32 + 255) / 256);
+    if (pack_recording()) return pack_record(PK_PACK_STRIP, blocks, false, &a, sizeof(a));
+    hipLaunchKernelGGL(pack_strip_kernel, dim3(blocks), dim3(256), 0, st, a);
     PCGAN_LAUNCH_CHECK();
     return 0;
 }
diff --git a/pc-gan_amd/csrc/thin_conv.hip b/pc-gan_amd/csrc/thin_conv.hip
--- a/pc-gan_amd/csrc/thin_conv.hip
+++ b/pc-gan_amd/csrc/thin_conv.hip
@@ -1,12 +1,10 @@
-#include "common.h"
+#include "pack_kernels.h"
+#include "pack_plan.h"
 
 namespace pcgan {
 namespace {
 
-typedef _Float16 f16x8 __attribute__((ext_vector_type(8)));
-typedef _Float16 f16x4 __attribute__((ext_vector_type(4)));
 typedef float f32x16 __attribute__((ext_vector_type(16)));
-typedef unsigned u32x4 __attribute__((ext_vector_type(4)));
 typedef unsigned u32x2 __attribute__((ext_vector_type(2)));
 
 constexpr unsigned THIN_OOB = 0x80000000u;
@@ -146,26 +144,7 @@
     report_nonfinite(a.ovf, bad);
 }
 
-__global__ void thin_pack_kernel(const float* __restrict__ w, const float* __restrict__ rowmax, u32x4* __restrict__ out, int M, int G, int T,
-                                 int nst, int transposed, int Kout, int Cin, int total) {
-    const int e = blockIdx.x * blockDim.x + threadIdx.x;
-    if (e >= total) return;
-    const int ln = e & 63, piece = (e >> 6) & 1, st = (e >> 7) % nst, mb = (e >> 7) / nst;
-    const int lo = ln & 31, hi = ln >> 5, m = mb * 32 + lo;
-    const float s = m < M ? pow2_scale(rowmax[m]) : 1.f;
-    f16x8 v;
-#pragma unroll
-    for (int i = 0; i < 8; ++i) {
-        const int k = st * 16 + hi * 8 + i, tap = k >> 2, g = k & 3;
-        float x = 0.f;
-        if (m < M && tap < T && g < G) x = transposed ? w[((size_t)g * Cin + m) * T + (T - 1 - tap)] : w[((size_t)m * Cin + g) * T + tap];
-        _Float16 h, l;
-        split2h(x * s, h, l);
-        v[i] = piece ? l : h;
-    }
-    (void)Kout;
-    out[e] = __builtin_bit_cast(u32x4, v);
-}
+__global__ void thin_pack_kernel(ThinPackArgs a) { thin_pack_body(a, blockIdx.x, gridDim.x); }
 
 struct Geo {
     int G, M, Hin, Win, Hout, Wout, pad, reflect, R, S, ST, nst, transposed;
@@ -255,8 +234,10 @@
     float* rowmax = (float*)((char*)packed + thin_body_bytes(g));
     if (launch_weight_row_absmax(w, d->K, d->C, d->R * d->S, g.transposed, rowmax, st)) return 2;
     const int total = (g.M / 32) * g.nst * 2 * 64;
-    hipLaunchKernelGGL(thin_pack_kernel, dim3((unsigned)((total + 255) / 256)), dim3(256), 0, st, w, (const float*)rowmax, (u32x4*)packed, g.M,
-                       g.G, g.R * g.S, g.nst, g.transposed, d->K, d->C, total);
+    const ThinPackArgs a = {w, rowmax, (u32x4*)packed, g.M, g.G, g.R * g.S, g.nst, g.transposed, d->C, total};
+    const unsigned blocks = (unsigned)((total + 255) / 256);
+    if (pack_recording()) return pack_record(PK_THIN, blocks, true, &a, sizeof(a));
+    hipLaunchKernelGGL(thin_pack_kernel, dim3(blocks), dim3(256), 0, st, a);
     PCGAN_LAUNCH_CHECK();
     return 0;
 }
diff --git a/pc-gan_amd/hip/lib.py b/pc-gan_amd/hip/lib.py
--- a/pc-gan_amd/hip/lib.py
+++ b/pc-gan_amd/hip/lib.py
@@ -27,6 +27,14 @@
     _fields_ = [(n, ctypes.c_int) for n in
                 ('N', 'C', 'H', 'W', 'K', 'R', 'S', 'stride', 'pad_h', 'pad_w', 'P', 'Q', 'k_off', 'K_total', 'dtype')]
 
+
+class PackItem(ctypes.Structure):
+    _fields_ = [('desc', ConvDesc), ('form', ctypes.c_int), ('pass_', ctypes.c_int), ('w', ctypes.c_void_p), ('rowmax', ctypes.c_void_p),
+                ('packed', ctypes.c_void_p)]
+
+
+PACK_FORM_IDS = {'pcgan_conv2d_pack_weights': 0, 'pcgan_conv2d_hgemm_pack': 1, 'pcgan_conv2d_bsplit_pack': 2,
+                 'pcgan_conv2d_bsplit_dgrad_pack': 3, 'pcgan_conv2d_hsplit_pack': 4, 'pcgan_conv2d_thin_pack': 5}
 
 _vp, _i, _f, _sz = ctypes.c_void_p, ctypes.c_int, ctypes.c_float, ctypes.c_size_t
 _dp = ctypes.POINTER(ConvDesc)
@@ -158,6 +166,11 @@
     'pcgan_pool_mse_fwd': (_i, [_vp] * 8 + [_sz] + [_i] * 4 + [_f, _f, _i, _vp]),
     'pcgan_skip_join_fwd': (_i, [_vp] * 3 + [_i] * 7 + [_vp]),
     'pcgan_skip_join_bwd': (_i, [_vp] * 5 + [_i] * 7 + [_vp]),
+    'pcgan_pack_plan_create': (_i, [ctypes.POINTER(PackItem), _i, ctypes.POINTER(_vp)]),
+    'pcgan_pack_plan_run': (_i, [_vp, _vp]),
+    'pcgan_pack_plan_launches': (_i, [_vp]),
+    'pcgan_pack_plan_jobs': (_i, [_vp, _i]),
+    'pcgan_pack_plan_destroy': (_i, [_vp]),
 }
 
 _lib = None
@@ -197,8 +210,12 @@
             set_option(key, conv(v), lib)
 
 
+OPTION_GEN = [0]
+
+
 def set_option(key, value, lib=None):
     lib = lib or load()
+    OPTION_GEN[0] += 1
     if lib.pcgan_set_option(key.encode(), int(value)) != 0:
         msg = lib.pcgan_last_error()
         raise RuntimeError('pcgan_hip set_option failed: %s' % (msg.decode() if msg else '?'))
diff --git a/pc-gan_amd/hip/ops.py b/pc-gan_amd/hip/ops.py
--- a/pc-gan_amd/hip/ops.py
+++ b/pc-gan_amd/hip/ops.py
@@ -343,8 +343,11 @@
     stamp = _weight_stamp(w)
     ent = cache.get(key)
     if ent is not None and ent[0] == stamp:
-        if ent[3] != _raw_stream():
-            torch.cuda.current_stream().wait_event(ent[2])
+        raw = _raw_stream()
+        if ent[3] != raw:
+            owner = w.__dict__.get('_pcgan_pack_owner')
+            if owner is None or not owner.already_waited(ent[2], raw):
+                torch.cuda.current_stream().wait_event(ent[2])
         return (ent[1], ent[4]) if want_rowmax else ent[1]
     cur = torch.cuda.current_stream()
     form = _PACK_FORMS[pass_]
@@ -367,7 +370,106 @@
     ev = torch.cuda.Event()
     ev.record(cur)
     cache[key] = (stamp, buf, ev, cur.cuda_stream, rowmax)
+    PACK_STATS['lazy'] += 1
+    owner = w.__dict__.get('_pcgan_pack_owner')
+    if owner is not None:
+        PACK_STATS['lazy_owned'] += 1
+        if PACK_PLAN:
+            owner.register(cache, key, d, pass_, w, buf, rowmax)
     return (buf, rowmax) if want_rowmax else buf
+
+
+PACK_PLAN = os.environ.get('PCGAN_PACK_PLAN', '1') != '0'
+PACK_STATS = {'lazy': 0, 'lazy_owned': 0, 'plan_builds': 0, 'plan_runs': 0, 'plan_launches': 0}
+_PLAN_GEN = [0]
+
+
+class _PackItem(object):
+    __slots__ = ('cache', 'key', 'd', 'pass_', 'w', 'wptr', 'buf', 'rowmax')
+
+
+class PackSet(object):
+
+    def __init__(self):
+        self.items = {}
+        self.handle = None
+        self.dirty = True
+        self.gen = (_PLAN_GEN[0], _L.OPTION_GEN[0])
+        self.event, self.waited = None, set()
+
+    def already_waited(self, ev, raw_stream):
+        if ev is not self.event:
+            return False
+        if raw_stream in self.waited:
+            return True
+        self.waited.add(raw_stream)
+        return False
+
+    def register(self, cache, key, d, pass_, w, buf, rowmax):
+        it = self.items.get((id(cache), key))
+        if it is not None and it.cache is cache and it.w is w and it.wptr == w.data_ptr() and it.buf is buf and it.rowmax is rowmax \
+                and it.pass_ == pass_ and bytes(it.d) == bytes(d):
+            return
+        it = _PackItem()
+        it.cache, it.key, it.d, it.pass_, it.w, it.wptr, it.buf, it.rowmax = cache, key, _L.ConvDesc.from_buffer_copy(d), pass_, w, w.data_ptr(), buf, rowmax
+        self.items[(id(cache), key)] = it
+        self.dirty = True
+
+    def _drop_plan(self):
+        if self.handle is not None:
+            h, self.handle = self.handle, None
+            _L.check(_L.load().pcgan_pack_plan_destroy(h), 'pack_plan_destroy')
+
+    def _build(self, lib):
+        self.items = {k: it for k, it in self.items.items() if (it.cache.get(it.key) or (None, None))[1] is it.buf}
+        self._drop_plan()
+        items = list(self.items.values())
+        arr = (_L.PackItem * max(len(items), 1))()
+        for a, it in zip(arr, items):
+            form = _PACK_FORMS[it.pass_]
+            a.desc, a.form, a.pass_ = it.d, _L.PACK_FORM_IDS[form.pack], form.lib_pass or 0
+            a.w, a.packed, a.rowmax = it.w.data_ptr(), it.buf.data_ptr(), it.rowmax.data_ptr() if it.rowmax is not None else None
+            it.wptr = a.w
+        h = ctypes.c_void_p()
+        _L.check(lib.pcgan_pack_plan_create(arr, len(items), ctypes.byref(h)), 'pack_plan_create')
+        self.handle = h
+        self.dirty = False
+        PACK_STATS['plan_builds'] += 1
+
+    def run(self):
+        if not PACK_PLAN:
+            return
+        gen = (_PLAN_GEN[0], _L.OPTION_GEN[0])
+        if gen != self.gen:
+            self.items.clear()
+            self.gen, self.dirty = gen, True
+        if not self.items:
+            return
+        lib = _L.load()
+        if self.dirty or any(it.w.data_ptr() != it.wptr for it in self.items.values()):
+            if torch.cuda.is_current_stream_capturing():
+                return
+            self._build(lib)
+            if not self.items:
+                return
+        cur = torch.cuda.current_stream(next(iter(self.items.values())).w.device)
+        for st in list(_side.values()) + list(_branch.values()):
+            if st.device == cur.device and st.cuda_stream != cur.cuda_stream:
+                cur.wait_stream(st)
+        _L.check(lib.pcgan_pack_plan_run(self.handle, _vp(cur.cuda_stream)), 'pack_plan_run')
+        PACK_STATS['plan_runs'] += 1
+        PACK_STATS['plan_launches'] += int(lib.pcgan_pack_plan_launches(self.handle))
+        ev = torch.cuda.Event()
+        self.event, self.waited = ev, set()
+        ev.record(cur)
+        for it in self.items.values():
+            it.cache[it.key] = (_weight_stamp(it.w), it.buf, ev, cur.cuda_stream, it.rowmax)
+
+    def __del__(self):
+        try:
+            self._drop_plan()
+        except Exception:
+            pass
 
 
 _PLANS = {}
@@ -376,6 +478,7 @@
 def clear_plans():
     _PLANS.clear()
     _RB_PLANS.clear()
+    _PLAN_GEN[0] += 1
 
 
 class _Plan(object):
diff --git a/pc-gan_amd/hip/optim.py b/pc-gan_amd/hip/optim.py
--- a/pc-gan_amd/hip/optim.py
+++ b/pc-gan_amd/hip/optim.py
@@ -25,6 +25,7 @@
         self.exp_avg = torch.zeros(total, dtype=torch.float32, device=dev)
         self.exp_avg_sq = torch.zeros(total, dtype=torch.float32, device=dev)
         self._views = []
+        self.packs = ops.PackSet()
         with torch.no_grad():
             for p, o in zip(ps, offs):
                 n = p.numel()
@@ -33,6 +34,7 @@
                 gv = self.gflat[o:o + n].view(p.shape)
                 p.grad = gv
                 p._pcgan_fused_grad = True
+                p._pcgan_pack_owner = self.packs
                 self._views.append((p, gv))
         self.numel = sum(p.numel() for p in ps)
         self.step_dev = torch.zeros(1, dtype=torch.int32, device=dev)
@@ -93,6 +95,7 @@
         if self.flat.is_cuda:
             ops.adam_step_dev(self.flat, self.gflat, self.exp_avg, self.exp_avg_sq, self.lr_dev, self.step_dev,
                               g['betas'][0], g['betas'][1], g['eps'], params=[p for p, _ in self._views])
+            self.packs.run()
         else:
             raise RuntimeError('FusedAdam: parameters are on %s; the HIP path needs a GPU (no CPU fallback)'
                                % self.flat.device)
```

After: 1198 images/sec. No clear change (-0.1%).
